# giuliojiang/pbrt-v3-IILE

Hardware: AMD Instinct MI355X
Metric: Mray/s on killeroo-simple 1080p (path integrator, rays = Scene::Intersect + IntersectP calls) (higher is better)
Workload: dtype f32

## Files before the change

include/iile_gpu.h:

```cpp
#ifndef IILE_GPU_H
#define IILE_GPU_H

#include "iile_scene.h"

#ifdef __cplusplus
extern "C" {
#endif

typedef struct iile_scene iile_scene;

enum {
    IILE_OK = 0,
    IILE_ERR_ARG = 1,
    IILE_ERR_NO_DEVICE = 2,
    IILE_ERR_HIP = 3,
    IILE_ERR_UNSUPPORTED = 4,
    IILE_ERR_TIMEOUT = 5
};

typedef struct iile_render_params {
    int32_t k_begin, k_end;
    int32_t tile_rank, tile_nranks;
    int32_t spp_per_pass;
    int32_t collect_stats;
// ... 5 lines not shown
typedef struct iile_stats {
    uint64_t camera_rays, closest_rays, shadow_rays;
    uint64_t nodes_closest, nodes_any, tri_tests, tri_hits;
    uint64_t sphere_tests;
    uint64_t nee_evals, zero_radiance;
    uint64_t path_length[8];
    double ms_total;
    double ms_generate, ms_extend, ms_shade, ms_connect, ms_film;
    int32_t n_extend_launches, n_connect_launches , n_shade_launches, n_passes;
    uint64_t n_paths;
    uint64_t workspace_bytes;
    uint64_t ext_rays, ext_nodes, ext_tri_tests, ext_sphere_tests;
    uint64_t any_tri_tests;
    double ms_shadow, ms_mis, ms_resolve;
    uint64_t mis_rays_traced;
    uint64_t ext_rays_traced;
} iile_stats;

int iile_device_count(void);
const char *iile_last_error(void);

int iile_device_select(int32_t device);
int iile_device_alloc(uint64_t bytes, void **out_dev);
void iile_device_free(void *dev);
int iile_device_download(void *dst_host, const void *src_dev, uint64_t bytes, void *stream);
int iile_device_upload(void *dst_dev, const void *src_host, uint64_t bytes, void *stream);
int iile_device_zero(void *dev, uint64_t bytes, void *stream);
int iile_stream_create(void **out_stream);
int iile_stream_wait(void *stream);
void iile_stream_destroy(void *stream);

int iile_scene_create(const iile_scene_desc *desc, iile_scene **out);
void iile_scene_destroy(iile_scene *scene);
int iile_scene_set_camera_motion(iile_scene *scene, const iile_camera_motion *motion);

int iile_render(iile_scene *scene, const iile_render_params *params, float *film_xyzw, iile_stats *stats);
int iile_render_status(iile_scene *scene, void *stream);
int iile_render_ao(iile_scene *scene, const iile_ao_params *params, const iile_render_params *render, float *film_xyzw, iile_stats *stats);
int iile_test_patch_capacity(iile_scene *scene, uint32_t capacity);

int iile_trace_closest(iile_scene *scene, int32_t n, const float *o3, const float *d3, const float *tmax,
                       int32_t *prim, float *tb, iile_stats *stats);
#define IILE_SHAPE_HIT_FLOATS 28
int iile_shape_hit_attributes(iile_scene *scene, int32_t n, const float *o3, const float *d3, const int32_t *prim, float *out);
int iile_trace_any(iile_scene *scene, int32_t n, const float *o3, const float *d3, const float *tmax,
                   int32_t *hit, iile_stats *stats);
int iile_halton_samples(iile_scene *scene, int32_t n, const int32_t *px, const int32_t *py, const int32_t *k,
                        int32_t dim0, int32_t ndims, float *out, uint32_t *index_out);
int iile_sample_table_records(iile_scene *scene, int32_t n, const int32_t *px, const int32_t *py, const int32_t *k, const int32_t *bounce,
                              float *out8);
uint64_t iile_sample_table_budget(void);
void iile_test_sample_table_budget(uint64_t bytes);
uint64_t iile_sample_table_bytes(const iile_scene *scene);
int iile_camera_rays(iile_scene *scene, int32_t n, const float *pfilm2, const float *plens2, float *o3, float *d3);
int iile_camera_rays_at(iile_scene *scene, int32_t n, const float *pfilm2, const float *plens2, float time, float *o3, float *d3);
int iile_li_samples(iile_scene *scene, int32_t n, const int32_t *px, const int32_t *py, const int32_t *k,
                    float *L3, int32_t *nrays2);
int iile_ao_array_samples(iile_scene *scene, int32_t n_samples, int32_t n, const int32_t *px, const int32_t *py, const int32_t *k,
                          const int32_t *j, float *out2);
int iile_ao_li_samples(iile_scene *scene, const iile_ao_params *params, int32_t n, const int32_t *px, const int32_t *py, const int32_t *k,
                       float *L1, int32_t *nrays2);
int iile_bsdf_eval(iile_scene *scene, int32_t n, int32_t mat, const float *wo3, const float *wi3, float *out4);
int iile_bsdf_sample(iile_scene *scene, int32_t n, int32_t mat, const float *wo3, const float *u2, float *out7);
int iile_bsdf_eval_ng(iile_scene *scene, int32_t n, int32_t mat, const float *ng3, const float *wo3, const float *wi3, float *out4);
int iile_bsdf_sample_ng(iile_scene *scene, int32_t n, int32_t mat, const float *ng3, const float *wo3, const float *u2, float *out7);
int iile_bsdf_sample_specular(iile_scene *scene, int32_t n, int32_t mat, const float *wo3, const float *u2, float *out9);
int iile_render_probes(iile_scene *scene, int32_t n_probes, const float *pos3, const float *dir3, float *intensity_rgb,
                       float *normals_xyz, float *distance, int32_t outputs_on_device, iile_stats *stats, void *stream);
typedef struct iile_probe_ref_params {
    int32_t max_depth;
    int32_t first_sample;
    int32_t n_samples;
    int32_t spp_total;
    int32_t outputs_on_device;
    void *stream;
} iile_probe_ref_params;
int iile_render_probes_reference(iile_scene *scene, int32_t n_probes, const float *pos3, const float *dir3, const iile_probe_ref_params *params,
                                 float *intensity_rgb, float *weight_sum, float *normals_xyz, float *distance, iile_stats *stats);
int iile_test_probe_ref_group(iile_scene *scene, uint32_t samples_per_group);
int iile_reference_points(iile_scene *scene, int32_t n, const float *pfilm2, uint8_t *valid, float *pos3, float *dir3);
typedef struct iile_direct_params {
    int32_t n_passes, first_pass;
    int32_t accumulate;
    int32_t film_on_device;
    void *stream;
} iile_direct_params;
int iile_render_direct(iile_scene *scene, const iile_direct_params *params, double *film_rgbw);
int iile_iispt_hemi_points(iile_scene *scene, const iile_iispt_task *task, uint8_t *valid, float *pos3, float *dir3);
int iile_iispt_gather(iile_scene *scene, const iile_iispt_task *task, const uint8_t *valid, const float *pos3, const float *dir3,
                      const float *nn_films, int32_t nn_on_device, float *out_rgbw, int32_t out_on_device);
int iile_iispt_hemi_points_batch(iile_scene *scene, const iile_iispt_task *tasks, int32_t n_tasks, uint8_t *valid, float *pos3, float *dir3,
                                 void *stream);
int iile_iispt_gather_batch(iile_scene *scene, const iile_iispt_task *tasks, int32_t n_tasks, const uint8_t *valid, const float *pos3,
                            const float *dir3, const float *nn_films, int32_t nn_on_device, float *out_rgbw, int32_t out_on_device, void *stream);
int iile_iispt_film_add(iile_scene *scene, const iile_iispt_task *tasks, int32_t n_tasks, const float *out_rgbw_dev, double *film_rgbw_dev,
                        int32_t film_w, int32_t film_h, void *stream);
int iile_iispt_film_merge(const double *direct_rgbw_dev, const double *indirect_rgbw_dev, int64_t n_pixels, float *rgb_dev, void *stream);
typedef struct iile_iispt_net iile_iispt_net;
typedef struct iile_iispt_net_weights {
    const float *conv_weight[15], *conv_bias[15];
    const float *bn_weight[5], *bn_bias[5], *bn_mean[5], *bn_var[5];
    float bn_eps;
} iile_iispt_net_weights;
int iile_iispt_net_create(const iile_iispt_net_weights *weights, iile_iispt_net **out);
int iile_iispt_net_load(const char *path, iile_iispt_net **out);
int iile_iispt_net_forward(iile_iispt_net *net, const float *in_dev, float *out_dev, int32_t n, int32_t max_batch, void *stream,
// ... 28 lines not shown
```

pbrt-v3-iile_amd/binding.py:

```python
import ctypes
import os

import numpy as np

_HERE = os.path.dirname(os.path.abspath(__file__))
LIB_DIR = os.path.join(_HERE, "lib")
REPO_ROOT = os.path.dirname(_HERE)
DEFAULT_SCENE = os.path.join(REPO_ROOT, "scenes", "killeroo-simple.pbrt")

c_i32, c_u32, c_u64, c_f32, c_f64 = (ctypes.c_int32, ctypes.c_uint32, ctypes.c_uint64, ctypes.c_float,
                                     ctypes.c_double)
c_vp = ctypes.c_void_p


class HostOverrides(ctypes.Structure):
    _fields_ = [("xres", c_i32), ("yres", c_i32), ("spp", c_i32), ("max_depth", c_i32), ("sampler", c_i32),
                ("accel_split", c_i32), ("bvh_build", c_vp), ("quick_render", c_i32)]


SAMPLERS = {None: 0, "": 0, "halton": 1, "sobol": 2}
SPLITS = {None: 0, "": 0, "sah": 1, "hlbvh": 2, "middle": 3, "equal": 4}


class HostSceneInfo(ctypes.Structure):
# ... 142 lines not shown

class Disney(ctypes.Structure):
    _fields_ = [(n, c_f32) for n in ("metallic specular_tint anisotropic sheen sheen_tint clearcoat clearcoat_gloss spec_trans "
                                     "flatness diff_trans").split()] + [("thin", c_i32), ("pad_", c_i32)]
QUADRIC_DISK, QUADRIC_CYLINDER = 0, 1
PRIM_SPHERE, PRIM_FLIP, PRIM_QUADRIC = 1, 8, 32
LIGHT_AREA_QUADRIC = 6


class GpuStats(ctypes.Structure):
    _fields_ = [(n, c_u64) for n in ("camera_rays closest_rays shadow_rays nodes_closest nodes_any tri_tests "
                                     "tri_hits sphere_tests nee_evals zero_radiance").split()] + [
        ("path_length", c_u64 * 8),
        ("ms_total", c_f64), ("ms_generate", c_f64), ("ms_extend", c_f64), ("ms_shade", c_f64),
        ("ms_connect", c_f64), ("ms_film", c_f64),
        ("n_extend_launches", c_i32), ("n_connect_launches", c_i32), ("n_shade_launches", c_i32),
        ("n_passes", c_i32), ("n_paths", c_u64), ("workspace_bytes", c_u64),
        ("ext_rays", c_u64), ("ext_nodes", c_u64), ("ext_tri_tests", c_u64), ("ext_sphere_tests", c_u64),
        ("any_tri_tests", c_u64), ("ms_shadow", c_f64), ("ms_mis", c_f64), ("ms_resolve", c_f64),
        ("mis_rays_traced", c_u64), ("ext_rays_traced", c_u64)]

    def as_dict(self):
        d = {}
        for name, _ in self._fields_:
            v = getattr(self, name)
            d[name] = list(v) if name == "path_length" else v
        return d


HOST_SYMBOLS = ["iile_host_load_pbrt", "iile_host_scene_desc", "iile_host_scene_film", "iile_host_scene_get_info",
                "iile_host_scene_free", "iile_host_film_to_rgb", "iile_host_write_pfm", "iile_host_last_error", "iile_host_read_image",
                "iile_host_scene_texture", "iile_host_scene_texture_level", "iile_host_scene_filter_table",
                "iile_host_sobol_matrices", "iile_host_sobol_vdc", "iile_host_write_exr", "iile_host_write_image",
                "iile_host_scene_film_filename", "iile_host_scene_light", "iile_host_scene_quadric_count", "iile_host_scene_quadric",
                "iile_host_scene_material", "iile_host_scene_camera", "iile_host_scene_ao", "iile_host_scene_camera_motion"]
class NetWeights(ctypes.Structure):
    _fields_ = [("conv_weight", c_vp * 15), ("conv_bias", c_vp * 15), ("bn_weight", c_vp * 5), ("bn_bias", c_vp * 5),
                ("bn_mean", c_vp * 5), ("bn_var", c_vp * 5), ("bn_eps", c_f32)]


class ProbeRefParams(ctypes.Structure):
    _fields_ = [("max_depth", c_i32), ("first_sample", c_i32), ("n_samples", c_i32), ("spp_total", c_i32), ("outputs_on_device", c_i32),
                ("stream", c_vp)]


class DirectParams(ctypes.Structure):
    _fields_ = [("n_passes", ctypes.c_int32), ("first_pass", ctypes.c_int32), ("accumulate", ctypes.c_int32), ("film_on_device", ctypes.c_int32),
                ("stream", ctypes.c_void_p)]


GPU_SYMBOLS = ["iile_device_count", "iile_last_error", "iile_scene_create", "iile_scene_destroy", "iile_render",
               "iile_scene_set_camera_motion", "iile_camera_rays_at",
               "iile_render_ao", "iile_ao_array_samples", "iile_ao_li_samples",
               "iile_trace_closest", "iile_trace_any", "iile_shape_hit_attributes", "iile_halton_samples", "iile_sample_table_records", "iile_sample_table_budget", "iile_test_sample_table_budget", "iile_sample_table_bytes", "iile_camera_rays", "iile_li_samples",
               "iile_bsdf_eval", "iile_bsdf_sample", "iile_bsdf_eval_ng", "iile_bsdf_sample_ng", "iile_bsdf_sample_specular", "iile_trig_probe", "iile_texture_eval", "iile_texture_eval_p", "iile_light_sample_li", "iile_light_sample_at", "iile_light_pdf_at", "iile_light_le", "iile_light_choose", "iile_render_probes",
               "iile_render_probes_reference", "iile_test_probe_ref_group", "iile_reference_points",
               "iile_device_select", "iile_device_alloc", "iile_device_free", "iile_device_download", "iile_device_upload", "iile_device_zero",
               "iile_stream_create", "iile_stream_wait", "iile_stream_destroy",
               "iile_iispt_film_add", "iile_iispt_film_merge",
               "iile_iispt_hemi_points", "iile_iispt_gather", "iile_iispt_hemi_points_batch", "iile_iispt_gather_batch", "iile_bvh_build_hlbvh", "iile_bvh_pack_probe", "iile_render_direct",
               "iile_wide_ref_shift", "iile_traversal_limits", "iile_render_status", "iile_test_patch_capacity", "iile_iispt_net_create", "iile_iispt_net_load", "iile_iispt_net_forward", "iile_iispt_net_predict", "iile_iispt_net_destroy"]
DIST_SYMBOLS = ["iile_dist_unique_id", "iile_dist_create", "iile_dist_create_deadline", "iile_dist_abort", "iile_dist_wait", "iile_dist_destroy", "iile_dist_rank", "iile_dist_size", "iile_dist_ranks_seen",
                "iile_dist_film_reduce", "iile_dist_monitor_reduce", "iile_dist_barrier", "iile_dist_sum_u64", "iile_dist_max_f64",
                "iile_dist_rendezvous_file", "iile_dist_rendezvous_file_token", "iile_dist_rendezvous_done", "iile_dist_all_ok",
                "iile_dist_last_error"]
DIST_ID_BYTES = 128

_host = None
_gpu = None
_dist = None


def host_lib():
    global _host
    if _host is None:
        path = os.path.join(LIB_DIR, "libiile_host.so")
        if not os.path.exists(path):
            raise RuntimeError(f"{path} is missing: run __graft_entry__.build() (make -C pbrt-v3-iile_amd/csrc host)")
        lib = ctypes.CDLL(path)
        lib.iile_host_last_error.restype = ctypes.c_char_p
        lib.iile_host_load_pbrt.argtypes = [ctypes.c_char_p, ctypes.POINTER(HostOverrides), ctypes.POINTER(c_vp)]
        lib.iile_host_scene_desc.restype = c_vp
        lib.iile_host_scene_desc.argtypes = [c_vp]
        lib.iile_host_scene_film.restype = ctypes.POINTER(FilmDesc)
        lib.iile_host_scene_film.argtypes = [c_vp]
        lib.iile_host_scene_get_info.argtypes = [c_vp, ctypes.POINTER(HostSceneInfo)]
        lib.iile_host_scene_ao.argtypes = [c_vp, ctypes.POINTER(AoParams)]
        lib.iile_host_scene_free.argtypes = [c_vp]
        lib.iile_host_scene_free.restype = None
        lib.iile_host_scene_quadric_count.argtypes = [c_vp]
        lib.iile_host_scene_quadric_count.restype = c_i32
        lib.iile_host_scene_quadric.argtypes = [c_vp, c_i32, ctypes.POINTER(Quadric)]
        lib.iile_host_scene_material.argtypes = [c_vp, c_i32, ctypes.POINTER(Material)]
        lib.iile_host_scene_camera.argtypes = [c_vp, ctypes.POINTER(Camera)]
        lib.iile_host_scene_camera_motion.argtypes = [c_vp, ctypes.POINTER(CameraMotion)]
        lib.iile_host_film_to_rgb.argtypes = [ctypes.POINTER(FilmDesc), c_vp, c_vp]
        lib.iile_host_write_pfm.argtypes = [ctypes.c_char_p, c_vp, c_i32, c_i32]
        lib.iile_host_read_image.argtypes = [ctypes.c_char_p, ctypes.POINTER(c_i32), ctypes.POINTER(c_i32), c_vp]
        lib.iile_host_write_exr.argtypes = [ctypes.c_char_p, c_vp, c_i32, c_i32, c_i32, c_i32, c_i32, c_i32]
        lib.iile_host_write_image.argtypes = [ctypes.c_char_p, ctypes.POINTER(FilmDesc), c_vp]
        lib.iile_host_scene_film_filename.argtypes = [c_vp]
        lib.iile_host_scene_film_filename.restype = ctypes.c_char_p
        lib.iile_host_scene_texture.argtypes = [c_vp, c_i32, ctypes.POINTER(Texture)]
        lib.iile_host_scene_texture_level.argtypes = [c_vp, c_i32, c_i32, c_vp]
        lib.iile_host_scene_filter_table.argtypes = [c_vp, c_vp]
        lib.iile_host_sobol_matrices.argtypes = [c_i32, c_vp, c_vp]
        lib.iile_host_sobol_vdc.argtypes = [c_i32, c_vp, c_vp]
# ... 44 lines not shown
        if not os.path.exists(path):
            raise RuntimeError(f"{path} is missing: the HIP extension was not built; there is no CPU fallback "
                               "(run __graft_entry__.build())")
        lib = ctypes.CDLL(path)
        lib.iile_last_error.restype = ctypes.c_char_p
        lib.iile_scene_create.argtypes = [c_vp, ctypes.POINTER(c_vp)]
        lib.iile_scene_destroy.argtypes = [c_vp]
        lib.iile_scene_destroy.restype = None
        lib.iile_render.argtypes = [c_vp, ctypes.POINTER(RenderParams), c_vp, ctypes.POINTER(GpuStats)]
        lib.iile_render_ao.argtypes = [c_vp, ctypes.POINTER(AoParams), ctypes.POINTER(RenderParams), c_vp, ctypes.POINTER(GpuStats)]
        lib.iile_ao_array_samples.argtypes = [c_vp, c_i32, c_i32, c_vp, c_vp, c_vp, c_vp, c_vp]
        lib.iile_ao_li_samples.argtypes = [c_vp, ctypes.POINTER(AoParams), c_i32, c_vp, c_vp, c_vp, c_vp, c_vp]
        lib.iile_trace_closest.argtypes = [c_vp, c_i32, c_vp, c_vp, c_vp, c_vp, c_vp, ctypes.POINTER(GpuStats)]
        lib.iile_trace_any.argtypes = [c_vp, c_i32, c_vp, c_vp, c_vp, c_vp, ctypes.POINTER(GpuStats)]
        lib.iile_halton_samples.argtypes = [c_vp, c_i32, c_vp, c_vp, c_vp, c_i32, c_i32, c_vp, c_vp]
        lib.iile_camera_rays.argtypes = [c_vp, c_i32, c_vp, c_vp, c_vp, c_vp]
        lib.iile_camera_rays_at.argtypes = [c_vp, c_i32, c_vp, c_vp, c_f32, c_vp, c_vp]
        lib.iile_scene_set_camera_motion.argtypes = [c_vp, ctypes.POINTER(CameraMotion)]
        lib.iile_li_samples.argtypes = [c_vp, c_i32, c_vp, c_vp, c_vp, c_vp, c_vp]
        lib.iile_bsdf_eval.argtypes = [c_vp, c_i32, c_i32, c_vp, c_vp, c_vp]
        lib.iile_texture_eval.argtypes = [c_vp, c_i32, c_i32, c_vp, c_vp, c_vp]
        lib.iile_light_sample_li.argtypes = [c_vp, c_i32, c_i32, c_vp, c_vp]
        lib.iile_light_sample_at.argtypes = [c_vp, c_i32, c_i32, c_vp, c_vp, c_vp, c_vp]
        lib.iile_light_pdf_at.argtypes = [c_vp, c_i32, c_i32, c_vp, c_vp, c_vp, c_vp]
        lib.iile_light_le.argtypes = [c_vp, c_i32, c_i32, c_vp, c_vp]
        lib.iile_light_choose.argtypes = [c_vp, c_i32, c_vp, c_vp, c_vp, c_vp, c_vp]
        lib.iile_texture_eval_p.argtypes = [c_vp, c_i32, c_i32, c_vp, c_vp, c_vp, c_vp]
        lib.iile_render_probes.argtypes = [c_vp, c_i32, c_vp, c_vp, c_vp, c_vp, c_vp, c_i32, ctypes.POINTER(GpuStats), c_vp]
        lib.iile_render_probes_reference.argtypes = [c_vp, c_i32, c_vp, c_vp, ctypes.POINTER(ProbeRefParams), c_vp, c_vp, c_vp, c_vp,
                                                     ctypes.POINTER(GpuStats)]
        lib.iile_test_probe_ref_group.argtypes = [c_vp, c_u32]
        lib.iile_reference_points.argtypes = [c_vp, c_i32, c_vp, c_vp, c_vp, c_vp]
        lib.iile_bsdf_sample.argtypes = [c_vp, c_i32, c_i32, c_vp, c_vp, c_vp]
        lib.iile_bsdf_eval_ng.argtypes = [c_vp, c_i32, c_i32, c_vp, c_vp, c_vp, c_vp]
        lib.iile_bsdf_sample_ng.argtypes = [c_vp, c_i32, c_i32, c_vp, c_vp, c_vp, c_vp]
        lib.iile_bsdf_sample_specular.argtypes = [c_vp, c_i32, c_i32, c_vp, c_vp, c_vp]
        lib.iile_trig_probe.argtypes = [c_i32, c_vp, c_vp]
        lib.iile_iispt_hemi_points.argtypes = [c_vp, ctypes.POINTER(IisptTask), c_vp, c_vp, c_vp]
        lib.iile_iispt_gather.argtypes = [c_vp, ctypes.POINTER(IisptTask), c_vp, c_vp, c_vp, c_vp, c_i32, c_vp, c_i32]
        lib.iile_iispt_hemi_points_batch.argtypes = [c_vp, ctypes.POINTER(IisptTask), c_i32, c_vp, c_vp, c_vp, c_vp]
        lib.iile_iispt_gather_batch.argtypes = [c_vp, ctypes.POINTER(IisptTask), c_i32, c_vp, c_vp, c_vp, c_vp, c_i32, c_vp, c_i32, c_vp]
        lib.iile_bvh_build_hlbvh.argtypes = [c_i32, c_vp, c_i32, c_vp, ctypes.POINTER(c_i32), c_vp, ctypes.POINTER(BvhBuildStats)]
        lib.iile_bvh_pack_probe.argtypes = [c_i32, c_vp, c_i32, c_vp, c_vp, ctypes.POINTER(c_i32)]
        lib.iile_render_status.argtypes = [c_vp, c_vp]
        lib.iile_traversal_limits.argtypes = [ctypes.POINTER(c_i32)]
        lib.iile_traversal_limits.restype = None
        lib.iile_test_patch_capacity.argtypes = [c_vp, c_u32]
        lib.iile_sample_table_budget.argtypes = []
        lib.iile_sample_table_budget.restype = c_u64
        lib.iile_test_sample_table_budget.argtypes = [c_u64]
        lib.iile_test_sample_table_budget.restype = None
        lib.iile_sample_table_bytes.argtypes = [c_vp]
        lib.iile_sample_table_bytes.restype = c_u64
        lib.iile_iispt_net_create.argtypes = [ctypes.POINTER(NetWeights), ctypes.POINTER(c_vp)]
        lib.iile_iispt_net_load.argtypes = [ctypes.c_char_p, ctypes.POINTER(c_vp)]
        lib.iile_iispt_net_forward.argtypes = [c_vp, c_vp, c_vp, c_i32, c_i32, c_vp, c_vp, c_i32]
        lib.iile_iispt_net_predict.argtypes = [c_vp, c_vp, c_vp, c_vp, c_vp, c_vp, c_i32, c_i32, c_i32, c_vp]
        lib.iile_iispt_film_add.argtypes = [c_vp, ctypes.POINTER(IisptTask), c_i32, c_vp, c_vp, c_i32, c_i32, c_vp]
        lib.iile_iispt_film_merge.argtypes = [c_vp, c_vp, ctypes.c_int64, c_vp, c_vp]
        lib.iile_device_upload.argtypes = [c_vp, c_vp, ctypes.c_uint64, c_vp]
        lib.iile_device_zero.argtypes = [c_vp, ctypes.c_uint64, c_vp]
        lib.iile_iispt_net_destroy.argtypes = [c_vp]
        lib.iile_iispt_net_destroy.restype = None
        _gpu = lib
    return _gpu


def dist_lib():
    global _dist
    if _dist is None:
        path = os.path.join(LIB_DIR, "libiile_dist.so")
        if not os.path.exists(path):
            raise RuntimeError(f"{path} is missing: run __graft_entry__.build() (make -C pbrt-v3-iile_amd/csrc dist)")
        lib = ctypes.CDLL(path)
        lib.iile_dist_last_error.restype = ctypes.c_char_p
        lib.iile_dist_unique_id.argtypes = [c_vp]
        lib.iile_dist_create.argtypes = [c_vp, c_i32, c_i32, ctypes.POINTER(c_vp)]
        lib.iile_dist_create_deadline.argtypes = [c_vp, c_i32, c_i32, ctypes.c_double, ctypes.POINTER(c_vp)]
        lib.iile_dist_wait.argtypes = [c_vp, c_vp]
        lib.iile_dist_abort.argtypes = [c_vp]
        lib.iile_dist_abort.restype = None
        lib.iile_dist_destroy.argtypes = [c_vp]
        lib.iile_dist_destroy.restype = None
        lib.iile_dist_rank.argtypes = [c_vp]
        lib.iile_dist_size.argtypes = [c_vp]
        lib.iile_dist_film_reduce.argtypes = [c_vp, c_vp, ctypes.c_int64, c_i32, c_vp]
        lib.iile_dist_barrier.argtypes = [c_vp, c_vp]
        lib.iile_dist_sum_u64.argtypes = [c_vp, c_vp, c_i32]
        lib.iile_dist_max_f64.argtypes = [c_vp, c_vp, c_i32]
        lib.iile_dist_rendezvous_file.argtypes = [ctypes.c_char_p, c_i32, c_vp, c_i32]
        lib.iile_dist_rendezvous_file_token.argtypes = [ctypes.c_char_p, c_i32, ctypes.c_uint64, c_vp, c_i32]
        lib.iile_dist_rendezvous_done.argtypes = [c_vp, ctypes.c_char_p]
        lib.iile_dist_all_ok.argtypes = [c_vp, c_i32, ctypes.POINTER(c_i32)]
        _dist = lib
    return _dist


class Dist:

    @staticmethod
    def unique_id():
        buf = (ctypes.c_uint8 * DIST_ID_BYTES)()
        lib = dist_lib()
        if lib.iile_dist_unique_id(buf) != 0:
            raise RuntimeError(f"iile_dist_unique_id failed: {lib.iile_dist_last_error().decode()}")
        return bytes(buf)
# ... 239 lines not shown
            self.close()
        except Exception:
            pass


def sample_table_budget():
    return int(gpu_lib().iile_sample_table_budget())


def set_test_sample_table_budget(nbytes):
    gpu_lib().iile_test_sample_table_budget(int(nbytes))


class GpuScene:

    def __init__(self, host_scene):
        lib = gpu_lib()
        self.host = host_scene
        self._s = c_vp()
        rc = lib.iile_scene_create(host_scene.desc, ctypes.byref(self._s))
        if rc != 0:
            raise RuntimeError(f"iile_scene_create failed ({rc}): {lib.iile_last_error().decode()}")
        motion = getattr(host_scene, "camera_motion", None)
        if motion is not None:
            rc = lib.iile_scene_set_camera_motion(self._s, ctypes.byref(motion))
            if rc != 0:
                msg = lib.iile_last_error().decode()
                lib.iile_scene_destroy(self._s)
                self._s = c_vp()
                raise RuntimeError(f"iile_scene_set_camera_motion failed ({rc}): {msg}")

    def _check(self, rc, what):
        if rc != 0:
            raise RuntimeError(f"{what} failed ({rc}): {gpu_lib().iile_last_error().decode()}")

    def render(self, k_begin=0, k_end=0, tile_rank=0, tile_nranks=1, spp_per_pass=0, collect_stats=False,
               time_kernels=False, film_device_ptr=None, stream=None, want_stats=True):
        prm = RenderParams(int(k_begin), int(k_end), int(tile_rank), int(tile_nranks), int(spp_per_pass),
                           int(bool(collect_stats)), int(time_kernels), int(film_device_ptr is not None),
                           c_vp(stream) if stream else None)
        st = GpuStats()
        if film_device_ptr is not None:
            film, ptr = None, c_vp(int(film_device_ptr))
        else:
            h, w = self.host.film_shape
            film = np.zeros((h, w, 4), np.float32)
            ptr = film.ctypes.data
        rc = gpu_lib().iile_render(self._s, ctypes.byref(prm), ptr, ctypes.byref(st) if want_stats else None)
        self._check(rc, "iile_render")
        if not want_stats:
            return film, None
        d = st.as_dict()
        d["sample_table_bytes"] = int(gpu_lib().iile_sample_table_bytes(self._s))
        return film, d

    def _ao_params(self, nsamples, cossample):
        ao = self.host.ao or {"nsamples": 64, "cossample": True}
        return AoParams(int(ao["nsamples"] if nsamples is None else nsamples), int(bool(ao["cossample"] if cossample is None else cossample)))

    def render_ao(self, nsamples=None, cossample=None, k_begin=0, k_end=0, tile_rank=0, tile_nranks=1, spp_per_pass=0, collect_stats=False,
                  film_device_ptr=None, stream=None, want_stats=True):
        ao = self._ao_params(nsamples, cossample)
        prm = RenderParams(int(k_begin), int(k_end), int(tile_rank), int(tile_nranks), int(spp_per_pass), int(bool(collect_stats)), 0,
                           int(film_device_ptr is not None), c_vp(stream) if stream else None)
        st = GpuStats()
        if film_device_ptr is not None:
            film, ptr = None, c_vp(int(film_device_ptr))
        else:
            h, w = self.host.film_shape
            film = np.zeros((h, w, 4), np.float32)
            ptr = film.ctypes.data
        rc = gpu_lib().iile_render_ao(self._s, ctypes.byref(ao), ctypes.byref(prm), ptr, ctypes.byref(st) if want_stats else None)
        self._check(rc, "iile_render_ao")
        return film, (st.as_dict() if want_stats else None)

    def ao_array_samples(self, nsamples, px, py, k, j):
        px, py, k, j = _i32(px), _i32(py), _i32(k), _i32(j)
        out = np.empty((len(px), 2), np.float32)
        self._check(gpu_lib().iile_ao_array_samples(self._s, int(nsamples), len(px), px.ctypes.data, py.ctypes.data, k.ctypes.data, j.ctypes.data,
                                                    out.ctypes.data), "iile_ao_array_samples")
        return out

    def ao_li_samples(self, px, py, k, nsamples=None, cossample=None):
        ao = self._ao_params(nsamples, cossample)
        px, py, k = _i32(px), _i32(py), _i32(k)
        n = len(px)
        L = np.empty(n, np.float32)
        nr = np.empty((n, 2), np.int32)
        self._check(gpu_lib().iile_ao_li_samples(self._s, ctypes.byref(ao), n, px.ctypes.data, py.ctypes.data, k.ctypes.data, L.ctypes.data,
                                                 nr.ctypes.data), "iile_ao_li_samples")
        return L, nr

    def render_status(self, stream=None):
        self._check(gpu_lib().iile_render_status(self._s, c_vp(stream) if stream else None), "iile_render_status")

    def test_patch_capacity(self, capacity):
        self._check(gpu_lib().iile_test_patch_capacity(self._s, int(capacity)), "iile_test_patch_capacity")

    def trace_closest(self, o, d, tmax, instrumented=True):
        o, d, tmax = _f32(o), _f32(d), _f32(tmax)
        n = len(tmax)
        prim = np.empty(n, np.int32)
        tb = np.empty((n, 4), np.float32)
        st = GpuStats()
        self._check(gpu_lib().iile_trace_closest(self._s, n, o.ctypes.data, d.ctypes.data, tmax.ctypes.data,
                                                 prim.ctypes.data, tb.ctypes.data,
                                                 ctypes.byref(st) if instrumented else None), "iile_trace_closest")
        return prim, tb, st.as_dict()

    def shape_hit_attributes(self, o, d, prim):
        o, d, prim = _f32(o).reshape(-1, 3), _f32(d).reshape(-1, 3), _i32(prim)
        out = np.empty((len(prim), 28), np.float32)
        f = gpu_lib().iile_shape_hit_attributes
        f.argtypes = [c_vp, c_i32, c_vp, c_vp, c_vp, c_vp]
        self._check(f(self._s, len(prim), o.ctypes.data, d.ctypes.data, prim.ctypes.data, out.ctypes.data), "iile_shape_hit_attributes")
        r = {k: out[:, 3 * i:3 * i + 3] for i, k in enumerate(("p", "n", "sn", "dpdu", "dpdv", "dndu", "dndv", "wo"))}
        r.update(u=out[:, 24], v=out[:, 25], flip=out[:, 26] != 0)
        return r

    def trace_any(self, o, d, tmax, instrumented=True):
        o, d, tmax = _f32(o), _f32(d), _f32(tmax)
        n = len(tmax)
        hit = np.empty(n, np.int32)
        st = GpuStats()
        self._check(gpu_lib().iile_trace_any(self._s, n, o.ctypes.data, d.ctypes.data, tmax.ctypes.data,
                                             hit.ctypes.data, ctypes.byref(st) if instrumented else None),
                    "iile_trace_any")
        return hit, st.as_dict()

    def halton_samples(self, px, py, k, dim0, ndims):
        px, py, k = _i32(px), _i32(py), _i32(k)
        n = len(px)
        out = np.empty((n, ndims), np.float32)
        idx = np.empty(n, np.uint32)
        self._check(gpu_lib().iile_halton_samples(self._s, n, px.ctypes.data, py.ctypes.data, k.ctypes.data, dim0,
                                                  ndims, out.ctypes.data, idx.ctypes.data), "iile_halton_samples")
        return out, idx

    def sample_table_records(self, px, py, k, bounce):
        px, py, k, bounce = _i32(px), _i32(py), _i32(k), _i32(bounce)
        out = np.empty((len(px), 8), np.float32)
        f = gpu_lib().iile_sample_table_records
        f.argtypes = [c_vp, c_i32, c_vp, c_vp, c_vp, c_vp, c_vp]
        self._check(f(self._s, len(px), px.ctypes.data, py.ctypes.data, k.ctypes.data, bounce.ctypes.data, out.ctypes.data),
                    "iile_sample_table_records")
        return out

    def camera_rays(self, pfilm, plens=None):
        pfilm = _f32(pfilm)
        n = len(pfilm)
        o = np.empty((n, 3), np.float32)
        d = np.empty((n, 3), np.float32)
        pl = _f32(plens) if plens is not None else None
        self._check(gpu_lib().iile_camera_rays(self._s, n, pfilm.ctypes.data, pl.ctypes.data if pl is not None else None,
                                               o.ctypes.data, d.ctypes.data), "iile_camera_rays")
        return o, d

    def camera_rays_at(self, pfilm, time, plens=None):
        pfilm = _f32(pfilm)
        n = len(pfilm)
        o = np.empty((n, 3), np.float32)
        d = np.empty((n, 3), np.float32)
        pl = _f32(plens) if plens is not None else None
        self._check(gpu_lib().iile_camera_rays_at(self._s, n, pfilm.ctypes.data, pl.ctypes.data if pl is not None else None,
                                                  c_f32(time), o.ctypes.data, d.ctypes.data), "iile_camera_rays_at")
        return o, d

    def set_camera_motion(self, motion):
        return gpu_lib().iile_scene_set_camera_motion(self._s, ctypes.byref(motion) if motion is not None else None)

    def li_samples(self, px, py, k):
        px, py, k = _i32(px), _i32(py), _i32(k)
        n = len(px)
        L = np.empty((n, 3), np.float32)
        nr = np.empty((n, 2), np.int32)
        self._check(gpu_lib().iile_li_samples(self._s, n, px.ctypes.data, py.ctypes.data, k.ctypes.data, L.ctypes.data,
                                              nr.ctypes.data), "iile_li_samples")
        return L, nr

    def bsdf_eval(self, mat, wo, wi):
        wo, wi = _f32(wo), _f32(wi)
        out = np.empty((len(wo), 4), np.float32)
        self._check(gpu_lib().iile_bsdf_eval(self._s, len(wo), mat, wo.ctypes.data, wi.ctypes.data, out.ctypes.data),
                    "iile_bsdf_eval")
        return out

    def light_sample_li(self, light, p):
        p = _f32(p).reshape(-1, 3)
        out = np.empty((len(p), 7), np.float32)
        self._check(gpu_lib().iile_light_sample_li(self._s, int(light), len(p), p.ctypes.data, out.ctypes.data), "iile_light_sample_li")
        return out

    def light_sample_at(self, light, ref_p, ref_n, u):
        ref_p, ref_n, u = _f32(ref_p).reshape(-1, 3), _f32(ref_n).reshape(-1, 3), _f32(u).reshape(-1, 2)
        assert len(ref_p) == len(ref_n) == len(u)
        out = np.empty((len(ref_p), 13), np.float32)
        self._check(gpu_lib().iile_light_sample_at(self._s, int(light), len(ref_p), ref_p.ctypes.data, ref_n.ctypes.data, u.ctypes.data,
                                                   out.ctypes.data), "iile_light_sample_at")
# ... 238 lines not shown
        if rc != 0:
            raise RuntimeError(f"iile_iispt_net_forward failed ({rc}): {self._lib.iile_last_error().decode()}")

    def predict(self, intensity_ptr, normals_ptr, distance_ptr, pred_ptr, n, film_rows=False, max_batch=0, stream=None, slot_ptr=None):
        rc = self._lib.iile_iispt_net_predict(self._h, intensity_ptr, normals_ptr, distance_ptr, pred_ptr, slot_ptr, int(n), int(bool(film_rows)),
                                              int(max_batch), stream)
        if rc != 0:
            raise RuntimeError(f"iile_iispt_net_predict failed ({rc}): {self._lib.iile_last_error().decode()}")

    def close(self):
        if self._h:
            self._lib.iile_iispt_net_destroy(self._h)
            self._h = c_vp()

    def __del__(self):
        try:
            self.close()
        except Exception:
            pass


def bvh_build_hlbvh(bounds6, max_prims_in_node=4):
    b = _f32(bounds6).reshape(-1, 6)
    n = len(b)
    nodes = np.zeros(max(2 * n, 1), dtype=BVH_NODE)
    order = np.zeros(max(n, 1), dtype=np.int32)
    n_nodes = c_i32(0)
    st = BvhBuildStats()
    rc = gpu_lib().iile_bvh_build_hlbvh(n, b.ctypes.data, int(max_prims_in_node), nodes.ctypes.data, ctypes.byref(n_nodes), order.ctypes.data,
                                        ctypes.byref(st))
    if rc != 0:
        raise RuntimeError(f"iile_bvh_build_hlbvh failed ({rc}): {gpu_lib().iile_last_error().decode()}")
    return nodes[:n_nodes.value].copy(), order[:n].copy(), {k: getattr(st, k) for k, _ in BvhBuildStats._fields_}


def bvh_pack_probe(nodes):
    nodes = np.ascontiguousarray(nodes, dtype=BVH_NODE)
    ni = int((nodes["nprims"] == 0).sum())
    wide = np.zeros((max(ni, 1), 16), np.float32)
    wide4 = np.zeros((max(ni, 1), 32), np.float32)
    nested = c_i32(0)
    rc = gpu_lib().iile_bvh_pack_probe(len(nodes), nodes.ctypes.data, ni, wide.ctypes.data, wide4.ctypes.data, ctypes.byref(nested))
    if rc != 0:
        raise RuntimeError(f"iile_bvh_pack_probe failed ({rc}): {gpu_lib().iile_last_error().decode()}")
    return wide[:ni], wide4[:ni], bool(nested.value)


def traversal_limits():
    out = (c_i32 * 3)()
    gpu_lib().iile_traversal_limits(out)
    return {"lds_stack": int(out[0]), "top_records": int(out[1]), "max_bvh_depth": int(out[2])}


def trig_probe(x):
    x = _f32(x)
    out = np.empty((len(x), 3), np.float32)
    rc = gpu_lib().iile_trig_probe(len(x), x.ctypes.data, out.ctypes.data)
    if rc != 0:
        raise RuntimeError(f"iile_trig_probe failed ({rc}): {gpu_lib().iile_last_error().decode()}")
    return out


def device_count():
    return int(gpu_lib().iile_device_count())
```

pbrt-v3-iile_amd/csrc/device/api_common.h:

```cpp
#pragma once
#include <algorithm>
#include <cstdint>
#include <string>
#include <vector>

#include "../../../include/iile_gpu.h"
#include "kernels.h"

#define HIP_TRY(expr)                                                                                        \
    do {                                                                                                     \
        hipError_t e_ = (expr);                                                                              \
        if (e_ != hipSuccess)                                                                                \
            return ::iile::api_fail(IILE_ERR_HIP, std::string(#expr) + ": " + hipGetErrorString(e_));       \
    } while (0)

namespace iile {

int ensure_device();

template <typename T>
struct DevBuf {
    T *p = nullptr;
    ~DevBuf() {
        if (p) (void)hipFree(p);
// ... 34 lines not shown
        const size_t want = std::max<size_t>(std::max(bytes, grown), 1);
        const hipError_t e = hipMalloc(&p, want);
        if (e != hipSuccess) {
            p = nullptr;
            return api_fail(IILE_ERR_HIP, oom ? std::string(oom) : "hipMalloc of a device block: " + std::string(hipGetErrorString(e)));
        }
        cap = want;
        return IILE_OK;
    }
};

struct Carver {
    char *base;
    size_t used = 0;
    explicit Carver(void *block = nullptr) : base(static_cast<char *>(block)) {}
    template <typename T>
    T *take(size_t n) {
        T *r = base ? reinterpret_cast<T *>(base + used) : nullptr;
        used += (std::max<size_t>(n, 1) * sizeof(T) + 255) & ~size_t(255);
        return r;
    }
};

struct EventPair {
    hipEvent_t a, b;
    int kind;
};

constexpr uint64_t kMaxPassPaths = 200000000ull;
static_assert(kMaxPassPaths < (uint64_t(1) << kSlotBits), "queue slots must fit kSlotBits");

}

struct iile_scene {
    iile::DScene ds;
    std::vector<void *> allocs;
    std::vector<uint8_t> prim_is_shape;
    int n_cus = 256;
    int max_depth = 5;
    int spp = 1;
    std::vector<int> light_samples;
    std::vector<int> light_types;
    uint32_t ws_paths = 0;
    iile::PassBuffers pb;
    iile::DevBlock ws_block;
    uint32_t film_tiles = 0, film_pixels = 0;
    iile::FilmBuffers fb;
    iile::DevBlock film_block, wide_block;
    uint64_t film_wide = 0;
    iile_probe_setup probe;
    const uint32_t *probe_pixel_offsets = nullptr;
    const float *probe_filter_table = nullptr;
    uint64_t sample_table_bytes = 0;
    void *stab_block = nullptr;
    bool camera_moves = false;
    float shutter[2] = {0.f, 1.f};
    uint32_t *flag_count = nullptr;
    float *flag_rec = nullptr;
    iile::DevBlock probe_block;
    int *spill = nullptr;
    hipStream_t nee_stream = nullptr;
    int *spill_nee = nullptr;
    hipEvent_t ev_shade[16] = {}, ev_nee[16] = {};
    std::vector<iile::EventPair> events;
    size_t events_used = 0;
    hipEvent_t ev_begin = nullptr, ev_end = nullptr;
    std::vector<int> tile_of_slot, slot_of_tile;
    iile::DevBlock tile_tables;
    int map_key[4] = {0, 0, 0, 0};
    iile::PatchDev patch{};
    iile::DevBlock patch_block;
    iile::DevBlock film_add_block;
    uint32_t patch_cap_override = 0;
    uint32_t probe_ref_group_override = 0;
    bool overflow_unchecked = false;
    hipStream_t overflow_stream = nullptr;
    iile::DevBlock scratch;
    iile::DevBlock ao_block;
};

namespace iile {
int ensure_workspace(iile_scene *sc, uint32_t n_paths);
int ensure_film(iile_scene *sc, uint32_t n_tiles, uint32_t n_pixels, uint64_t n_wide = 0);
int frame_pass(iile_scene *sc, const DScene &S, int rank, int nranks, hipStream_t stream, PassDesc *P);
uint64_t path_budget(double bytes_per_path);
constexpr uint64_t kSampleTableBudget = uint64_t(4) << 30;
uint64_t sample_table_budget();
void set_sample_table_budget(uint64_t bytes);
int run_pass(iile_scene *sc, const DScene &S, int max_depth, const PassDesc &P_in, const LaunchCfg &cfg, bool timed, bool one_stream = false);
void copy_counters(const DCounters &c, iile_stats *st);
struct FrameIntegrator {
    double bytes_per_path;
    uint64_t max_pass_paths;
    const char *too_many;
    int (*reserve)(iile_scene *sc, uint32_t n_paths, void *ctx);
    int (*run)(iile_scene *sc, const DScene &S, const PassDesc &P, const LaunchCfg &cfg, bool timed, bool one_stream, void *ctx);
    void *ctx;
};
int render_frame(iile_scene *sc, const iile_render_params *prm, float *film_xyzw, iile_stats *stats, const FrameIntegrator &fi);
}
```

pbrt-v3-iile_amd/csrc/device/api_probes.hip:

```cpp
#include <cstring>

#include "api_common.h"

using namespace iile;

namespace {
LaunchCfg probe_cfg(const iile_scene *sc, bool count_stats = false) {
    LaunchCfg cfg{sc->n_cus, nullptr, count_stats};
    cfg.camera_moves = sc->camera_moves;
    return cfg;
}
template <typename T>
int finish(DevBuf<T> &dev, T *host, size_t n) {
    HIP_TRY(hipGetLastError());
    HIP_TRY(hipDeviceSynchronize());
    return dev.get(host, n);
}

int trace_common(iile_scene *sc, int32_t n, const float *o3, const float *d3, const float *tmax, int any,
                 std::vector<float4> *hits, iile_stats *stats) {
    if (!sc || n < 0 || !o3 || !d3 || !tmax) return api_fail(IILE_ERR_ARG, "iile_trace: bad argument");
    int rc = ensure_device();
    if (rc) return rc;
    std::vector<float4> ro(n), rd(n);
// ... 54 lines not shown
    return IILE_OK;
}

int iile_trace_any(iile_scene *sc, int32_t n, const float *o3, const float *d3, const float *tmax, int32_t *hit,
                   iile_stats *stats) {
    if (!hit) return api_fail(IILE_ERR_ARG, "iile_trace_any: null output");
    std::vector<float4> hits;
    int rc = trace_common(sc, n, o3, d3, tmax, 1, &hits, stats);
    if (rc) return rc;
    for (int i = 0; i < n; ++i) {
        uint32_t u;
        std::memcpy(&u, &hits[2 * i].x, 4);
        hit[i] = int32_t(u);
    }
    return IILE_OK;
}

int iile_halton_samples(iile_scene *sc, int32_t n, const int32_t *px, const int32_t *py, const int32_t *k,
                        int32_t dim0, int32_t ndims, float *out, uint32_t *index_out) {
    if (!sc || n < 0 || !px || !py || !k || !out || ndims <= 0 || dim0 < 0 || dim0 + ndims > (sc->ds.sobol ? sc->ds.sobol_dims : sc->ds.n_hdims))
        return api_fail(IILE_ERR_ARG, "iile_halton_samples: bad argument");
    int rc = ensure_device();
    if (rc) return rc;
    DevBuf<int> dx, dy, dk;
    DevBuf<float> dout;
    DevBuf<uint32_t> dindex;
    if ((rc = dx.put(px, n)) || (rc = dy.put(py, n)) || (rc = dk.put(k, n)) || (rc = dout.alloc(size_t(n) * ndims)) ||
        (rc = dindex.alloc(n)))
        return rc;
    if (n) launch_halton(sc->ds, n, dx.p, dy.p, dk.p, dim0, ndims, dout.p, dindex.p, probe_cfg(sc));
    if ((rc = finish(dout, out, size_t(n) * ndims))) return rc;
    if (index_out && (rc = dindex.get(index_out, n))) return rc;
    return IILE_OK;
}

int iile_sample_table_records(iile_scene *sc, int32_t n, const int32_t *px, const int32_t *py, const int32_t *k, const int32_t *bounce,
                              float *out8) {
    if (!sc || n < 0 || !px || !py || !k || !bounce || !out8) return api_fail(IILE_ERR_ARG, "iile_sample_table_records: bad argument");
    if (!sc->ds.stab_shade) return api_fail(IILE_ERR_ARG, "iile_sample_table_records: the scene has no sample table");
    for (int i = 0; i < n; ++i)
        if (k[i] < 0 || uint32_t(k[i]) >= sc->ds.stab_spp || bounce[i] >= sc->ds.max_depth)
            return api_fail(IILE_ERR_ARG, "iile_sample_table_records: sample or bounce outside the table");
    int rc = ensure_device();
    if (rc) return rc;
    DevBuf<int> dx, dy, dk, db;
    DevBuf<float> dout;
    if ((rc = dx.put(px, n)) || (rc = dy.put(py, n)) || (rc = dk.put(k, n)) || (rc = db.put(bounce, n)) || (rc = dout.alloc(size_t(n) * 8))) return rc;
    if (n) launch_sample_table_read(sc->ds, n, dx.p, dy.p, dk.p, db.p, dout.p, probe_cfg(sc));
    return finish(dout, out8, size_t(n) * 8);
}
uint64_t iile_sample_table_budget(void) { return sample_table_budget(); }
void iile_test_sample_table_budget(uint64_t bytes) { set_sample_table_budget(bytes); }
uint64_t iile_sample_table_bytes(const iile_scene *sc) { return sc ? sc->sample_table_bytes : 0; }

int iile_camera_rays(iile_scene *sc, int32_t n, const float *pfilm2, const float *plens2, float *o3, float *d3) {
    if (!sc || n < 0 || !pfilm2 || !o3 || !d3) return api_fail(IILE_ERR_ARG, "iile_camera_rays: bad argument");
    return iile_camera_rays_at(sc, n, pfilm2, plens2, 0.f, o3, d3);
}
int iile_camera_rays_at(iile_scene *sc, int32_t n, const float *pfilm2, const float *plens2, float time, float *o3, float *d3) {
    if (!sc || n < 0 || !pfilm2 || !o3 || !d3) return api_fail(IILE_ERR_ARG, "iile_camera_rays_at: bad argument");
    if (!(time == time)) return api_fail(IILE_ERR_ARG, "iile_camera_rays_at: the time is not a number");
    int rc = ensure_device();
    if (rc) return rc;
    DevBuf<float> df, dl, dox, ddx;
    if ((rc = df.put(pfilm2, 2 * size_t(n))) || (rc = dox.alloc(3 * size_t(n))) || (rc = ddx.alloc(3 * size_t(n))))
        return rc;
    if (plens2 && (rc = dl.put(plens2, 2 * size_t(n)))) return rc;
    if (n) launch_camera(sc->ds, n, df.p, plens2 ? dl.p : nullptr, time, dox.p, ddx.p, probe_cfg(sc));
    if ((rc = finish(dox, o3, 3 * size_t(n))) || (rc = ddx.get(d3, 3 * size_t(n)))) return rc;
    return IILE_OK;
}

int iile_bsdf_eval(iile_scene *sc, int32_t n, int32_t mat, const float *wo3, const float *wi3, float *out4) {
    return bsdf_probe(sc, n, mat, wo3, wi3, 3, 0, out4, 4);
}
int iile_bsdf_sample(iile_scene *sc, int32_t n, int32_t mat, const float *wo3, const float *u2, float *out7) {
    return bsdf_probe(sc, n, mat, wo3, u2, 2, 1, out7, 7);
}
int iile_bsdf_eval_ng(iile_scene *sc, int32_t n, int32_t mat, const float *ng3, const float *wo3, const float *wi3, float *out4) {
    if (!ng3) return api_fail(IILE_ERR_ARG, "iile_bsdf_eval_ng: null normal");
    return bsdf_probe(sc, n, mat, wo3, wi3, 3, 0, out4, 4, ng3);
}
int iile_bsdf_sample_ng(iile_scene *sc, int32_t n, int32_t mat, const float *ng3, const float *wo3, const float *u2, float *out7) {
    if (!ng3) return api_fail(IILE_ERR_ARG, "iile_bsdf_sample_ng: null normal");
    return bsdf_probe(sc, n, mat, wo3, u2, 2, 1, out7, 7, ng3);
}

int iile_bsdf_sample_specular(iile_scene *sc, int32_t n, int32_t mat, const float *wo3, const float *u2, float *out9) {
    return bsdf_probe(sc, n, mat, wo3, u2, 2, 2, out9, 9);
}

int iile_light_sample_li(iile_scene *sc, int32_t light, int32_t n, const float *p3, float *out7) {
    if (!sc || n < 0 || !p3 || !out7 || light < 0 || light >= sc->ds.n_lights)
        return api_fail(IILE_ERR_ARG, "iile_light_sample_li: bad argument");
    if (!iile_light_is_delta(sc->light_types[size_t(light)])) return api_fail(IILE_ERR_ARG, "iile_light_sample_li: not a delta light");
    int rc = ensure_device();
    if (rc) return rc;
    DevBuf<float> dp, dout;
    if ((rc = dp.put(p3, 3 * size_t(n))) || (rc = dout.alloc(7 * size_t(n)))) return rc;
    if (n) launch_light_probe(sc->ds, n, light, dp.p, dout.p, probe_cfg(sc));
    return finish(dout, out7, 7 * size_t(n));
}

static bool light_is_sampled(int type) {
    return type == IILE_LIGHT_DIFFUSE_AREA || type == IILE_LIGHT_AREA_TRIANGLE || type == IILE_LIGHT_AREA_QUADRIC || type == IILE_LIGHT_INFINITE;
}
// ... 114 lines not shown
```

pbrt-v3-iile_amd/csrc/device/api_render.hip:

```cpp
#include <chrono>
#include <cmath>
#include <cstdio>
#include <cstdlib>
#include <cstring>

#include "api_common.h"

using namespace iile;

namespace {

int get_events(iile_scene *sc, int kind, EventPair **out) {
    if (sc->events_used == sc->events.size()) {
        EventPair ep;
        HIP_TRY(hipEventCreate(&ep.a));
        HIP_TRY(hipEventCreate(&ep.b));
        sc->events.push_back(ep);
    }
    *out = &sc->events[sc->events_used++];
    (*out)->kind = kind;
    return IILE_OK;
}

template <typename Fn>
// ... 171 lines not shown
        sc->fb.tile_rgbw = c.take<float4>(2 * size_t(n_tiles) * 256);
        sc->fb.film_xyzw = c.take<float4>(n_pixels);
        return c.used;
    };
    if (const int rc = sc->film_block.reserve(film(Carver()))) return rc;
    film(Carver(sc->film_block.p));
    sc->fb.k0_rgbv = sc->fb.tile_rgbw + size_t(n_tiles) * 256;
    sc->film_tiles = n_tiles;
    sc->film_pixels = n_pixels;
    return IILE_OK;
}

int frame_pass(iile_scene *sc, const DScene &S, int rank, int nranks, hipStream_t stream, PassDesc *P) {
    std::memset(P, 0, sizeof(*P));
    P->n_tiles_x = (S.samp_x1 - S.samp_x0 + 15) / 16;
    P->n_tiles_y = (S.samp_y1 - S.samp_y0 + 15) / 16;
    P->tile_rank = rank, P->tile_nranks = nranks;
    return ensure_tile_map(sc, P, stream);
}

uint64_t path_budget(double bytes_per_path) {
    double budget_mb = 65536;
    if (const char *e = std::getenv("IILE_WORKSPACE_MB")) budget_mb = std::max(64.0, atof(e));
    return std::min<uint64_t>(uint64_t(budget_mb * 1048576.0 / bytes_per_path), kMaxPassPaths);
}

void copy_counters(const DCounters &c, iile_stats *st) {
    st->camera_rays = c.camera_rays;
    st->closest_rays = c.closest_rays;
    st->shadow_rays = c.shadow_rays;
    st->nodes_closest = c.nodes_closest;
    st->nodes_any = c.nodes_any;
    st->tri_tests = c.tri_tests;
    st->tri_hits = c.tri_hits;
    st->sphere_tests = c.sphere_tests;
    st->nee_evals = c.nee_evals;
    st->zero_radiance = c.zero_radiance;
    for (int i = 0; i < 8; ++i) st->path_length[i] = c.path_length[i];
    st->ext_rays = c.ext_rays;
    st->ext_nodes = c.ext_nodes;
    st->ext_tri_tests = c.ext_tri_tests;
    st->ext_sphere_tests = c.ext_sphere_tests;
    st->any_tri_tests = c.any_tri_tests;
    st->mis_rays_traced = c.mis_traced;
    st->ext_rays_traced = c.ext_traced;
}

int run_pass(iile_scene *sc, const DScene &S_in, int max_depth, const PassDesc &P_in, const LaunchCfg &cfg, bool timed, bool one_stream) {
    PassBuffers &B = sc->pb;
    PassDesc P = P_in;
    DScene S = S_in;
    if (cfg.count_stats || P.list_px || S.probe_mode || P.k0 < 0 || uint64_t(P.k0) + uint64_t(P.kc) > uint64_t(S.stab_spp) || max_depth > S.max_depth)
        clear_sample_table(&S);
    P.gen_fused = !cfg.count_stats && !P.list_px && !S.has_infinite && !S.probe_mode && !B.nray_out && !S.env_camera && !cfg.camera_moves;
    HIP_TRY(hipMemsetAsync(B.counts, 0, kCntWords * sizeof(uint32_t), cfg.stream));
    auto timed_launch_on = [&](hipStream_t stream, int kind, auto &&fn) -> int { return timed_step(sc, timed, stream, kind, fn); };
    auto timed_launch = [&](int kind, auto &&fn) -> int { return timed_launch_on(cfg.stream, kind, fn); };
    const bool two_streams = sc->nee_stream && !one_stream && !cfg.count_stats && !S.has_infinite && max_depth < 15;
    const bool nee_doubled = two_streams && !S.has_specular && B.nee_alt;
    LaunchCfg cfg_nee = cfg;
    if (two_streams) cfg_nee.stream = sc->nee_stream;
    auto buffers_of = [&](int bounce, bool nee_side) {
        PassBuffers X = B;
        if (nee_doubled && (bounce & 1)) X.nee = B.nee_alt, X.mis_hit = B.mis_hit_alt, X.nee_mis = B.nee_mis_alt;
        if (two_streams && nee_side) X.spill = sc->spill_nee;
        return X;
    };
    int rc = IILE_OK;
    if (P.gen_fused) {
        HIP_TRY(hipMemsetD32Async(reinterpret_cast<hipDeviceptr_t>(&B.counts[0]), int(P.n_paths), 1, cfg.stream));
    } else {
        rc = timed_launch(0, [&] { launch_generate(S, P, B, cfg); });
        if (rc) return rc;
    }
    P.skip_last_bounce = 0;
    if (!cfg.count_stats && max_depth >= 1 && !S.probe_mode && !B.nray_out)
        P.skip_last_bounce = S.has_specular ? 1 : 2;
    const int last_bounce = (P.skip_last_bounce == 2) ? max_depth - 1 : max_depth;
    for (int b = 0; b <= last_bounce; ++b) {
        rc = timed_launch(1, [&] { launch_extend(S, P, B, b, B.queue_cap, cfg); });
        if (rc) return rc;
        if (S.has_infinite) {
            rc = timed_launch(6, [&] { launch_miss(S, B, b, B.queue_cap, cfg); });
            if (rc) return rc;
        }
        if (two_streams && !nee_doubled && b > 0) HIP_TRY(hipStreamWaitEvent(cfg.stream, sc->ev_nee[b - 1], 0));
        if (nee_doubled && b > 1) HIP_TRY(hipStreamWaitEvent(cfg.stream, sc->ev_nee[b - 2], 0));
        const PassBuffers B_shade = buffers_of(b, false), B_nee = buffers_of(b, true);
        rc = timed_launch(2, [&] { launch_shade(S, P, B_shade, b, B.queue_cap, cfg); });
        if (rc) return rc;
        if (b < max_depth) {
            if (two_streams) {
                HIP_TRY(hipEventRecord(sc->ev_shade[b], cfg.stream));
                HIP_TRY(hipStreamWaitEvent(cfg_nee.stream, sc->ev_shade[b], 0));
            }
            rc = timed_launch_on(cfg_nee.stream, 5, [&] { launch_mis(S, B_nee, b, B.queue_cap, cfg_nee); });
            if (rc) return rc;
            rc = timed_launch_on(cfg_nee.stream, 6, [&] { launch_mis_lit(S, B_nee, b, B.queue_cap, cfg_nee); });
            if (rc) return rc;
            rc = timed_launch_on(cfg_nee.stream, 3, [&] { launch_shadow(S, B_nee, b, B.queue_cap, cfg_nee); });
            if (rc) return rc;
            if (two_streams) HIP_TRY(hipEventRecord(sc->ev_nee[b], cfg_nee.stream));
        }
    }
    if (two_streams && max_depth > 0) HIP_TRY(hipStreamWaitEvent(cfg.stream, sc->ev_nee[max_depth - 1], 0));
    HIP_TRY(hipGetLastError());
    return IILE_OK;
}

int render_frame(iile_scene *sc, const iile_render_params *prm, float *film_xyzw, iile_stats *stats, const FrameIntegrator &fi) {
    int rc = check_pending_overflow(sc);
    if (rc) return rc;
    const DScene &S = sc->ds;
    int k_begin = prm->k_begin, k_end = prm->k_end;
    if (k_end <= 0) {
        k_begin = 0;
        k_end = sc->spp;
    }
    if (k_begin < 0 || k_begin >= k_end) return api_fail(IILE_ERR_ARG, "iile_render: empty sample range");
    int rank = prm->tile_rank, nranks = prm->tile_nranks;
    if (nranks <= 0) {
        rank = 0;
        nranks = 1;
    }
    if (rank < 0 || rank >= nranks) return api_fail(IILE_ERR_ARG, "iile_render: tile_rank out of range");
    hipStream_t stream = static_cast<hipStream_t>(prm->stream);
    LaunchCfg cfg{sc->n_cus, stream, prm->collect_stats != 0};
    cfg.camera_moves = sc->camera_moves;
    const bool timed = prm->time_kernels != 0;

    PassDesc P;
    rc = frame_pass(sc, S, rank, nranks, stream, &P);
    if (rc) return rc;
    const uint64_t pix_slots = uint64_t(P.n_owned_tiles) * 256;
    const int n_samples = k_end - k_begin;
    uint64_t max_paths = std::min<uint64_t>(path_budget(fi.bytes_per_path), fi.max_pass_paths);
    if (prm->spp_per_pass > 0) max_paths = std::min<uint64_t>(max_paths, std::max<uint64_t>(1, pix_slots * uint64_t(prm->spp_per_pass)));
    const uint64_t paths_per_tile = uint64_t(256) * uint64_t(n_samples);
    if (paths_per_tile > kMaxPassPaths) return api_fail(IILE_ERR_UNSUPPORTED, "more than 781 250 samples per pixel in one render: split the sample range");
    if (paths_per_tile > fi.max_pass_paths) return api_fail(IILE_ERR_UNSUPPORTED, fi.too_many);
    const int tiles_per_pass = int(std::max<uint64_t>(1, std::min<uint64_t>(uint64_t(std::max(P.n_owned_tiles, 1)), max_paths / paths_per_tile)));
    const uint32_t fw = uint32_t(S.crop_x1 - S.crop_x0), fh = uint32_t(S.crop_y1 - S.crop_y0);
// ... 186 lines not shown
```

pbrt-v3-iile_amd/csrc/device/api_scene.hip:

```cpp
#include <array>
#include <chrono>
#include <cmath>
#include <cstddef>
#include <cstdio>
#include <cstdlib>
#include <cstring>
#include <limits>
#include <map>

#include "api_common.h"

using namespace iile;

namespace {
thread_local std::string g_err;
}
namespace iile {
int api_fail(int code, const std::string &msg) {
    g_err = msg;
    return code;
}
int ensure_device() {
    int n = 0;
    hipError_t e = hipGetDeviceCount(&n);
// ... 635 lines not shown
    const int n = d.n_lights;
    const size_t stride = light_record_floats(n);
    if (n > 1 && d.integrator.light_strategy != IILE_LIGHTS_SPATIAL) {
        std::vector<float> tab(stride, 0.f);
        const float *power = n > IILE_MAX_LIGHTS ? d.light_power_all : d.integrator.light_power;
        float *func = tab.data(), *cdf = tab.data() + n;
        for (int i = 0; i < n; ++i) func[i] = d.integrator.light_strategy == IILE_LIGHTS_UNIFORM ? 1.f : power[i];
        cdf[0] = 0;
        for (int i = 1; i < n + 1; ++i) cdf[i] = cdf[i - 1] + func[i - 1] / n;
        const float func_int = cdf[n];
        if (func_int == 0)
            for (int i = 1; i < n + 1; ++i) cdf[i] = float(i) / float(n);
        else
            for (int i = 1; i < n + 1; ++i) cdf[i] /= func_int;
        tab[2 * size_t(n) + 1] = func_int;
        return upload(sc, tab.data(), tab.size(), &S.light_dist);
    }
    if (!spatial_table(d)) return IILE_OK;
    light_grid(d, S.light_nv);
    std::vector<float> samples(128 * 5);
    const int bases[5] = {2, 3, 5, 7, 11};
    for (int i = 0; i < 128; ++i)
        for (int b = 0; b < 5; ++b) {
            if (b == 0) {
                uint64_t v = uint64_t(i), r = 0;
                for (int k = 0; k < 64; ++k) r |= ((v >> k) & 1ull) << (63 - k);
                samples[5 * i] = float(double(r) * 0x1p-64);
                continue;
            }
            const float inv_base = 1.f / float(bases[b]);
            uint64_t a = uint64_t(i), rev = 0;
            float inv_base_n = 1;
            while (a) {
                const uint64_t next = a / uint64_t(bases[b]);
                rev = rev * uint64_t(bases[b]) + (a - next * uint64_t(bases[b]));
                inv_base_n *= inv_base;
                a = next;
            }
            samples[5 * i + b] = std::min(float(rev) * inv_base_n, 0x1.fffffep-1f);
        }
    const float *dsamples = nullptr;
    float *dist = nullptr;
    const size_t n_vox = size_t(S.light_nv[0]) * S.light_nv[1] * S.light_nv[2];
    int rc = upload(sc, samples.data(), samples.size(), &dsamples);
    if (!rc) rc = scene_alloc(sc, n_vox * stride * sizeof(float), &dist, "hipMalloc(light distributions) failed");
    if (rc) return rc;
    S.light_dist = dist;
    LaunchCfg cfg{sc->n_cus, nullptr, false};
    launch_light_distributions(S, dsamples, dist, cfg);
    if (hipDeviceSynchronize() != hipSuccess || hipGetLastError() != hipSuccess) return api_fail(IILE_ERR_HIP, "light distribution kernel failed");
    return IILE_OK;
}

int build_sample_table(iile_scene *sc, const iile_scene_desc &d) {
    DScene &S = sc->ds;
    clear_sample_table(&S);
    sc->sample_table_bytes = 0;
    const int64_t spp = d.halton.spp;
    if (S.sobol || S.max_depth <= 0 || spp <= 0 || S.sample_stride <= 0 || std::getenv("IILE_NO_SAMPLE_TABLE")) return IILE_OK;
    if (5 + 7 * int64_t(S.max_depth) >= int64_t(S.n_hdims)) return IILE_OK;
    const bool lens = S.lens_radius > 0;
    const uint64_t per_slot = uint64_t(32) * uint64_t(S.max_depth) + (lens ? 16 : 8);
    if (uint64_t(spp) > sample_table_budget() / (uint64_t(16384) * per_slot)) return IILE_OK;
    const uint64_t slots = uint64_t(16384) * uint64_t(spp);
    if (slots >= (uint64_t(1) << 32)) return IILE_OK;
    const auto t0 = std::chrono::steady_clock::now();
    S.stab_slots = uint32_t(slots), S.stab_spp = uint32_t(spp);
    if (spp > 1) {
        int l = 0;
        while ((uint64_t(1) << l) < uint64_t(spp)) ++l;
        S.stab_spp_magic = uint32_t((((uint64_t(1) << l) - uint64_t(spp)) << 32) / uint64_t(spp) + 1);
        S.stab_spp_shift = uint32_t(l - 1);
    }
    float2 *cam = nullptr, *lens_part = nullptr;
    float4 *shade = nullptr;
    auto layout = [&](Carver c) {
        cam = c.take<float2>(slots);
        if (lens) lens_part = c.take<float2>(slots);
        shade = c.take<float4>(slots * uint64_t(S.max_depth) * 2);
        return c.used;
    };
    void *block = nullptr;
    if (hipMalloc(&block, layout(Carver())) != hipSuccess) {
        (void)hipGetLastError();
        clear_sample_table(&S);
        return IILE_OK;
    }
    sc->allocs.push_back(block);
    sc->stab_block = block;
    layout(Carver(block));
    launch_sample_table(S, cam, lens_part, shade, LaunchCfg{sc->n_cus, nullptr, false});
    if (hipDeviceSynchronize() != hipSuccess || hipGetLastError() != hipSuccess) return api_fail(IILE_ERR_HIP, "sample table kernel failed");
    S.stab_cam = cam, S.stab_lens = lens_part, S.stab_shade = shade;
    sc->sample_table_bytes = slots * per_slot;
    if (std::getenv("IILE_TIMING"))
        fprintf(stderr, "iile timing: sample table of %.1f MiB built in %.3f s\n", double(sc->sample_table_bytes) / 1048576.0,
                std::chrono::duration<double>(std::chrono::steady_clock::now() - t0).count());
    return IILE_OK;
}

}

namespace iile {
namespace {
uint64_t g_table_budget_override = 0;
}
uint64_t sample_table_budget() { return g_table_budget_override ? g_table_budget_override : kSampleTableBudget; }
void set_sample_table_budget(uint64_t bytes) { g_table_budget_override = bytes; }
}

extern "C" {

const char *iile_last_error(void) { return g_err.c_str(); }

int iile_device_count(void) {
    int n = 0;
    if (hipGetDeviceCount(&n) != hipSuccess) return 0;
    return n;
}

int iile_device_select(int32_t device) {
    int rc = ensure_device();
    if (rc) return rc;
    HIP_TRY(hipSetDevice(device));
    return IILE_OK;
}
int iile_device_alloc(uint64_t bytes, void **out_dev) {
    if (!out_dev) return api_fail(IILE_ERR_ARG, "iile_device_alloc: null argument");
    int rc = ensure_device();
    if (rc) return rc;
    HIP_TRY(hipMalloc(out_dev, std::max<size_t>(size_t(bytes), 1)));
    return IILE_OK;
}
void iile_device_free(void *dev) {
    if (dev) (void)hipFree(dev);
}
int iile_device_download(void *dst_host, const void *src_dev, uint64_t bytes, void *stream) {
    if (!dst_host || !src_dev) return api_fail(IILE_ERR_ARG, "iile_device_download: null argument");
    hipStream_t s = static_cast<hipStream_t>(stream);
    HIP_TRY(hipMemcpyAsync(dst_host, src_dev, size_t(bytes), hipMemcpyDeviceToHost, s));
    HIP_TRY(hipStreamSynchronize(s));
    return IILE_OK;
}

int iile_device_upload(void *dst_dev, const void *src_host, uint64_t bytes, void *stream) {
    if (!dst_dev || !src_host) return api_fail(IILE_ERR_ARG, "iile_device_upload: null argument");
    hipStream_t s = static_cast<hipStream_t>(stream);
    HIP_TRY(hipMemcpyAsync(dst_dev, src_host, size_t(bytes), hipMemcpyHostToDevice, s));
    HIP_TRY(hipStreamSynchronize(s));
    return IILE_OK;
// ... 39 lines not shown
              "texture kinds");
int iile_scene_create(const iile_scene_desc *d, iile_scene **out) {
    if (!d || !out) return api_fail(IILE_ERR_ARG, "iile_scene_create: null argument");
    int rc = check_scene_desc(*d);
    if (!rc) rc = ensure_device();
    if (rc) return rc;
    iile_scene *sc = new iile_scene;
    std::memset(&sc->ds, 0, sizeof(sc->ds));
    std::memset(&sc->pb, 0, sizeof(sc->pb));
    std::memset(&sc->fb, 0, sizeof(sc->fb));
    hipDeviceProp_t prop;
    int dev = 0;
    if (hipGetDevice(&dev) == hipSuccess && hipGetDeviceProperties(&prop, dev) == hipSuccess)
        sc->n_cus = prop.multiProcessorCount;
    set_kernel_flags(*d, sc->ds);
    for (auto build : {build_bvh, build_top4, build_prims, build_shapes, build_materials, build_textures, build_lights, build_halton,
                       build_sobol, build_camera_film, build_runtime, build_light_distribution, build_sample_table}) {
        rc = build(sc, *d);
        if (rc) {
            iile_scene_destroy(sc);
            return rc;
        }
    }
    *out = sc;
    return IILE_OK;
}

int iile_scene_set_camera_motion(iile_scene *sc, const iile_camera_motion *mo) {
    if (!sc || !mo) return api_fail(IILE_ERR_ARG, "iile_scene_set_camera_motion: null argument");
    if (sc->camera_moves) return api_fail(IILE_ERR_ARG, "iile_scene_set_camera_motion: the scene's camera has a motion already");
    auto finite = [](const float *v, size_t n) {
        for (size_t i = 0; i < n; ++i)
            if (!std::isfinite(v[i])) return false;
        return true;
    };
    if (!finite(&mo->start_time, 1) || !finite(&mo->end_time, 1) || !finite(mo->camera_to_world_end, 16) || !finite(&mo->T[0][0], 6) ||
        !finite(&mo->R[0][0], 8) || !finite(&mo->S[0][0], 32))
        return api_fail(IILE_ERR_ARG, "iile_scene_set_camera_motion: a non-finite entry in the camera motion");
    if (mo->end_time < mo->start_time) return api_fail(IILE_ERR_ARG, "iile_scene_set_camera_motion: the motion ends before it starts (TransformTimes)");
    int rc = ensure_device();
    if (rc) return rc;
    DScene &S = sc->ds;
    DCameraMotion dm;
    std::memset(&dm, 0, sizeof(dm));
    dm.c2w_start = S.camera_to_world;
    std::memcpy(dm.c2w_end.m, mo->camera_to_world_end, 64);
    dm.start_time = mo->start_time, dm.end_time = mo->end_time;
    dm.shutter_open = sc->shutter[0], dm.shutter_close = sc->shutter[1];
    std::memcpy(dm.T, mo->T, sizeof(dm.T));
    std::memcpy(dm.R, mo->R, sizeof(dm.R));
    for (int k = 0; k < 2; ++k)
        for (int i = 0; i < 3; ++i)
            for (int j = 0; j < 3; ++j) dm.S[k][3 * i + j] = mo->S[k][4 * i + j];
    if (S.stab_cam) {
        const uint64_t slots = S.stab_slots;
        void *time = nullptr;
        if (sc->sample_table_bytes + 4 * slots <= sample_table_budget() && hipMalloc(&time, size_t(slots) * sizeof(float)) != hipSuccess) {
            (void)hipGetLastError();
            time = nullptr;
        }
        if (!time) {
            for (void *&p : sc->allocs)
                if (p == sc->stab_block) p = nullptr;
            HIP_TRY(hipFree(sc->stab_block));
            sc->stab_block = nullptr;
            clear_sample_table(&S);
            sc->sample_table_bytes = 0;
        } else {
            sc->allocs.push_back(time);
            launch_sample_table_time(S, static_cast<float *>(time), LaunchCfg{sc->n_cus, nullptr, false});
            if (hipDeviceSynchronize() != hipSuccess || hipGetLastError() != hipSuccess) return api_fail(IILE_ERR_HIP, "sample table time kernel failed");
            dm.stab_time = static_cast<float *>(time);
            sc->sample_table_bytes += 4 * slots;
        }
    }
    HIP_TRY(hipMemcpy(const_cast<DCameraMotion *>(camera_motion(S)), &dm, sizeof(dm), hipMemcpyHostToDevice));
    sc->camera_moves = true;
    return IILE_OK;
}

void iile_scene_destroy(iile_scene *sc) {
    if (!sc) return;
    for (void *p : sc->allocs) (void)hipFree(p);
    if (sc->nee_stream) (void)hipStreamDestroy(sc->nee_stream);
    for (int i = 0; i < 16; ++i) {
        if (sc->ev_shade[i]) (void)hipEventDestroy(sc->ev_shade[i]);
        if (sc->ev_nee[i]) (void)hipEventDestroy(sc->ev_nee[i]);
    }
    for (EventPair &e : sc->events) {
        (void)hipEventDestroy(e.a);
        (void)hipEventDestroy(e.b);
    }
    if (sc->ev_begin) (void)hipEventDestroy(sc->ev_begin);
    if (sc->ev_end) (void)hipEventDestroy(sc->ev_end);
    delete sc;
}
}
```

pbrt-v3-iile_amd/csrc/device/dbsdf.h:

```cpp
#pragma once
enum Lobe : int { kLobePassThrough, kLobeLambert, kLobeLambertTrans, kLobeMicro, kLobeMicroTrans, kLobeBlend, kLobeSpecular, kLobeSpecTrans };
DEV bool lobe_is_specular(Lobe l) { return l == kLobePassThrough || l == kLobeSpecular || l == kLobeSpecTrans; }
struct Bsdf {
    F3 ns, ng, ss, ts;
    F3 kd;
    union { F3 micro_r, ks; };
    union { F3 kr, ltrans_t, cond_eta; };
    union { F3 kt, mtrans_t, cond_k; };
    float alpha, eta;
    float alpha_y;
    F3 t0;
    bool has_t0, has_t1;
    float path_eta;
    bool has_mtrans;
    int n_lobes;
    float on_a, on_b;
    bool oren_nayar;
    int mtype;
    bool has_lambert, has_micro, has_spec;
    bool has_blend;
    bool has_ltrans;
};
DEV int n_nonspec(const Bsdf &b) {
    return (b.has_lambert ? 1 : 0) + (b.has_ltrans ? 1 : 0) + (b.has_micro ? 1 : 0) + (b.has_mtrans ? 1 : 0) + (b.has_blend ? 1 : 0);
// ... 314 lines not shown
    const float eta = wo.z > 0 ? (eta_b / eta_a) : (eta_a / eta_b);
    F3 wh = normalize(wo + wi * eta);
    if (wh.z < 0) wh = -wh;
    const float F = fr_dielectric(dot(wo, wh), eta_a, eta_b);
    const float sqrt_denom = dot(wo, wh) + eta * dot(wi, wh);
    const float factor = 1 / eta;
    const float omf = 1.f - F;
    return F3{omf, omf, omf} * b.mtrans_t *
           fabsf(tr_d(wh, b.alpha, b.alpha_y) * tr_g(wo, wi, b.alpha, b.alpha_y) * eta * eta * absdot(wi, wh) * absdot(wo, wh) * factor * factor /
                 (cos_i * cos_o * sqrt_denom * sqrt_denom));
}
DEV float mtrans_pdf(const Bsdf &b, F3 wo, F3 wi) {
    if (same_hemisphere(wo, wi)) return 0;
    const float eta_a = 1.f, eta_b = b.eta;
    const float eta = wo.z > 0 ? (eta_b / eta_a) : (eta_a / eta_b);
    const F3 wh = normalize(wo + wi * eta);
    const float sqrt_denom = dot(wo, wh) + eta * dot(wi, wh);
    const float dwh_dwi = fabsf((eta * eta * dot(wi, wh)) / (sqrt_denom * sqrt_denom));
    return tr_pdf(wo, wh, b.alpha, b.alpha_y) * dwh_dwi;
}
DEV F3 lobes_f(const Bsdf &b, F3 wo, F3 wi) {
    F3 f = F3{0, 0, 0};
    if (b.has_lambert) f = f + diffuse_f(b, wo, wi);
    if (b.has_micro) f = f + micro_f(b, wo, wi);
    if (b.has_blend) f = f + blend_f(b, wo, wi);
    return f;
}
DEV F3 trans_lobes_f(const Bsdf &b, F3 wo, F3 wi) {
    F3 f = F3{0, 0, 0};
    if (b.has_ltrans) f = f + ltrans_f(b);
    if (b.has_mtrans) f = f + mtrans_f(b, wo, wi);
    return f;
}
DEV F3 bsdf_f(const Bsdf &b, F3 woW, F3 wiW) {
    F3 wi = to_local(b, wiW), wo = to_local(b, woW);
    if (wo.z == 0) return F3{0, 0, 0};
    bool reflect = dot(wiW, b.ng) * dot(woW, b.ng) > 0;
    if (reflect) return lobes_f(b, wo, wi);
    return trans_lobes_f(b, wo, wi);
}
DEV float bsdf_pdf(const Bsdf &b, F3 woW, F3 wiW) {
    if (b.n_lobes == 0) return 0.f;
    F3 wo = to_local(b, woW), wi = to_local(b, wiW);
    if (wo.z == 0) return 0.f;
    float pdf = 0.f;
    if (b.has_lambert) pdf += lambert_pdf(wo, wi);
    if (b.has_ltrans) pdf += ltrans_pdf(wo, wi);
    if (b.has_micro) pdf += micro_pdf(b, wo, wi);
    if (b.has_mtrans) pdf += mtrans_pdf(b, wo, wi);
    if (b.has_blend) pdf += blend_pdf(b, wo, wi);
    const int matching = n_nonspec(b);
    return matching > 0 ? pdf / matching : 0.f;
}
DEV F3 bsdf_sample_f(const Bsdf &b, F3 woW, F3 *wiW, float u0, float u1, float *pdf, const bool allow_specular = false,
                     bool *sampled_specular = nullptr, bool *sampled_transmission = nullptr) {
    if (sampled_specular) *sampled_specular = false;
    if (sampled_transmission) *sampled_transmission = false;
    const int matching = allow_specular ? b.n_lobes : n_nonspec(b);
    if (matching == 0) {
        *pdf = 0;
        return F3{0, 0, 0};
    }
    int comp = int(floorf(u0 * matching));
    if (comp > matching - 1) comp = matching - 1;
    Lobe pick;
    int count = comp;
    if (allow_specular && b.has_t0 && count-- == 0)
        pick = kLobePassThrough;
    else if (b.has_lambert && count-- == 0)
        pick = kLobeLambert;
    else if (b.has_ltrans && count-- == 0)
        pick = kLobeLambertTrans;
    else if (b.has_micro && count-- == 0)
        pick = kLobeMicro;
    else if (b.has_mtrans && count-- == 0)
        pick = kLobeMicroTrans;
    else if (b.has_blend && count-- == 0)
        pick = kLobeBlend;
    else if (!(allow_specular && b.has_t1) || (b.has_spec && count-- == 0))
        pick = kLobeSpecular;
    else
        pick = kLobeSpecTrans;
    if (pick == kLobeSpecular && !b.has_spec) __builtin_unreachable();
    const float ur0 = mn(u0 * matching - comp, kOneMinusEpsilon);
    F3 wo = to_local(b, woW);
    if (wo.z == 0) return F3{0, 0, 0};
    *pdf = 0;
    F3 wi = F3{0, 0, 0}, f;
    if (pick == kLobeLambert) {
        wi = cosine_sample_hemisphere(ur0, u1);
        if (wo.z < 0) wi.z *= -1;
        *pdf = lambert_pdf(wo, wi);
        f = diffuse_f(b, wo, wi);
    } else if (pick == kLobeLambertTrans) {
        wi = cosine_sample_hemisphere(ur0, u1);
        if (wo.z > 0) wi.z *= -1;
        *pdf = ltrans_pdf(wo, wi);
        f = ltrans_f(b);
    } else if (pick == kLobeMicro) {
        F3 wh = tr_sample_wh(wo, ur0, u1, b.alpha, b.alpha_y);
        wi = -wo + 2 * dot(wo, wh) * wh;
        if (!same_hemisphere(wo, wi))
            f = F3{0, 0, 0};
        else {
            *pdf = tr_pdf(wo, wh, b.alpha, b.alpha_y) / (4 * dot(wo, wh));
            f = micro_f(b, wo, wi);
        }
    } else if (pick == kLobeBlend) {
        float ua = ur0;
        if (ua < .5f) {
            ua = mn(2 * ua, kOneMinusEpsilon);
            wi = cosine_sample_hemisphere(ua, u1);
            if (wo.z < 0) wi.z *= -1;
        } else {
            ua = mn(2 * (ua - .5f), kOneMinusEpsilon);
            const F3 wh = tr_sample_wh(wo, ua, u1, b.alpha, b.alpha_y);
            wi = -wo + 2 * dot(wo, wh) * wh;
            if (!same_hemisphere(wo, wi)) return F3{0, 0, 0};
        }
        *pdf = blend_pdf(b, wo, wi);
        f = blend_f(b, wo, wi);
    } else if (pick == kLobeMicroTrans) {
        const F3 wh = tr_sample_wh(wo, ur0, u1, b.alpha, b.alpha_y);
        const float eta_a = 1.f, eta_b = b.eta;
        const float eta = wo.z > 0 ? (eta_a / eta_b) : (eta_b / eta_a);
        if (!refract_dir(wo, wh, eta, &wi)) return F3{0, 0, 0};
        *pdf = mtrans_pdf(b, wo, wi);
        f = mtrans_f(b, wo, wi);
    } else if (pick == kLobePassThrough || pick == kLobeSpecTrans) {
        const float eta_a = 1.f, eta_b = pick == kLobePassThrough ? 1.f : b.eta;
        float scale;
        if (!specular_refract(wo, eta_a, eta_b, &wi, &scale)) return F3{0, 0, 0};
        *pdf = 1;
        const F3 ft = (pick == kLobePassThrough ? b.t0 : b.kt) * (1.f - fr_dielectric(wi.z, eta_a, eta_b));
        f = sdiv(ft * scale, fabsf(wi.z));
        if (sampled_specular) *sampled_specular = true;
        if (sampled_transmission) *sampled_transmission = true;
    } else if (b.mtype == kMatGlass) {
        const float eta_a = 1.f, eta_b = b.eta;
        const float F = fr_dielectric(wo.z, eta_a, eta_b);
        if (ur0 < F) {
            wi = F3{-wo.x, -wo.y, wo.z};
            *pdf = F;
// ... 272 lines not shown
    switch (l) {
    case kDzDiffuse:
    case kDzRetro: return b.dz_diffuse;
    case kDzFakeSS: return b.dz_diffuse && b.dz_thin;
    case kDzSheen: return b.dz_sheen;
    case kDzMicro: return true;
    case kDzCoat: return b.dz_coat;
    case kDzMicroTrans: return b.has_mtrans;
    default: return b.has_ltrans;
    }
}
DEV F3 dz_lobes_f(const DisneyBsdf &b, bool reflect, F3 wo, F3 wi) {
    F3 f = F3{0, 0, 0};
    if (reflect) {
        if (b.dz_diffuse) {
            f = f + dz_diffuse_f(b.r_diffuse, wo, wi);
            if (b.dz_thin) f = f + dz_fakess_f(b.r_ss, b.rough, wo, wi);
            f = f + dz_retro_f(b.r_retro, b.rough, wo, wi);
            if (b.dz_sheen) f = f + dz_sheen_f(b.r_sheen, wo, wi);
        }
        f = f + dz_micro_f(b, wo, wi);
        if (b.dz_coat) f = f + dz_coat_f(b, wo, wi);
    } else {
        if (b.has_mtrans) f = f + dz_mtrans_f(b, wo, wi);
        if (b.has_ltrans) f = f + ltrans_f(b);
    }
    return f;
}
DEV float dz_lobes_pdf(const DisneyBsdf &b, int skip, F3 wo, F3 wi, float pdf) {
    const float cosine = lambert_pdf(wo, wi);
#pragma unroll
    for (int l = kDzDiffuse; l <= kDzSheen; ++l)
        if (l != skip && dz_has(b, DisneyLobe(l))) pdf += cosine;
    if (skip != kDzMicro) pdf += micro_pdf(b, wo, wi);
    if (skip != kDzCoat && b.dz_coat) pdf += dz_coat_pdf(b, wo, wi);
    if (skip != kDzMicroTrans && b.has_mtrans) pdf += dz_mtrans_pdf(b, wo, wi);
    if (skip != kDzLambertTrans && b.has_ltrans) pdf += ltrans_pdf(wo, wi);
    return pdf;
}
DEV F3 bsdf_f(const DisneyBsdf &b, F3 woW, F3 wiW) {
    if (!b.disney) return bsdf_f(static_cast<const Bsdf &>(b), woW, wiW);
    const F3 wi = to_local(b, wiW), wo = to_local(b, woW);
    if (wo.z == 0) return F3{0, 0, 0};
    const bool reflect = dot(wiW, b.ng) * dot(woW, b.ng) > 0;
    return dz_lobes_f(b, reflect, wo, wi);
}
DEV float bsdf_pdf(const DisneyBsdf &b, F3 woW, F3 wiW) {
    if (!b.disney) return bsdf_pdf(static_cast<const Bsdf &>(b), woW, wiW);
    const F3 wo = to_local(b, woW), wi = to_local(b, wiW);
    if (wo.z == 0) return 0.f;
    return dz_lobes_pdf(b, -1, wo, wi, 0.f) / b.n_lobes;
}
DEV F3 bsdf_sample_f(const DisneyBsdf &b, F3 woW, F3 *wiW, float u0, float u1, float *pdf, const bool allow_specular = false,
                     bool *sampled_specular = nullptr, bool *sampled_transmission = nullptr) {
    if (!b.disney) return bsdf_sample_f(static_cast<const Bsdf &>(b), woW, wiW, u0, u1, pdf, allow_specular, sampled_specular, sampled_transmission);
    if (sampled_specular) *sampled_specular = false;
    if (sampled_transmission) *sampled_transmission = false;
    const int matching = b.n_lobes;
    int comp = int(floorf(u0 * matching));
    if (comp > matching - 1) comp = matching - 1;
    int pick = kDzLambertTrans, count = comp;
    bool found = false;
#pragma unroll
    for (int l = kDzDiffuse; l <= kDzLambertTrans; ++l)
        if (!found && dz_has(b, DisneyLobe(l)) && count-- == 0) pick = l, found = true;
    const float ur0 = mn(u0 * matching - comp, kOneMinusEpsilon);
    const F3 wo = to_local(b, woW);
    if (wo.z == 0) return F3{0, 0, 0};
    *pdf = 0;
    F3 wi = F3{0, 0, 0}, f;
    if (pick <= kDzSheen) {
        wi = cosine_sample_hemisphere(ur0, u1);
        if (wo.z < 0) wi.z *= -1;
        *pdf = lambert_pdf(wo, wi);
        f = dz_lobe_f(b, DisneyLobe(pick), wo, wi);
    } else if (pick == kDzMicro) {
        const F3 wh = tr_sample_wh(wo, ur0, u1, b.alpha, b.alpha_y);
        wi = -wo + 2 * dot(wo, wh) * wh;
        if (!same_hemisphere(wo, wi))
            f = F3{0, 0, 0};
        else {
            *pdf = tr_pdf(wo, wh, b.alpha, b.alpha_y) / (4 * dot(wo, wh));
            f = dz_micro_f(b, wo, wi);
        }
    } else if (pick == kDzCoat) {
        const float alpha2 = .25f * .25f;
        const float cos_t = sqrtf(mx(0.f, (1 - powf(alpha2, 1 - ur0)) / (1 - alpha2)));
        const float sin_t = sqrtf(mx(0.f, 1 - cos_t * cos_t));
        const float phi = 2 * kPi * u1;
        float sp, cp;
        sincos_f(phi, &sp, &cp);
        F3 wh = F3{sin_t * cp, sin_t * sp, cos_t};
        if (!same_hemisphere(wo, wh)) wh = -wh;
        wi = -wo + 2 * dot(wo, wh) * wh;
        if (!same_hemisphere(wo, wi))
            f = F3{0, 0, 0};
        else {
            *pdf = dz_coat_pdf(b, wo, wi);
            f = dz_coat_f(b, wo, wi);
        }
    } else if (pick == kDzMicroTrans) {
        const F3 wh = tr_sample_wh(wo, ur0, u1, b.t_ax, b.t_ay);
        const float eta_a = 1.f, eta_b = b.eta;
        const float eta = wo.z > 0 ? (eta_a / eta_b) : (eta_b / eta_a);
        if (!refract_dir(wo, wh, eta, &wi)) return F3{0, 0, 0};
        *pdf = dz_mtrans_pdf(b, wo, wi);
        f = dz_mtrans_f(b, wo, wi);
// ... 18 lines not shown
```

pbrt-v3-iile_amd/csrc/device/dlight.h:

```cpp
#pragma once
#include "dtex.h"
struct LightSample {
    F3 p, perr, n;
};
DEV float sphere_area(const DSphere &sp) { return sp.phi_max * sp.radius * (sp.zmax - sp.zmin); }
DEV LightSample sphere_sample_area(const DSphere &sp, float u0, float u1, float *pdf) {
    float z = 1 - 2 * u0;
    float r = sqrtf(mx(0.f, 1.f - z * z));
    float phi = 2 * kPi * u1;
    float s, c;
    sincos_f(phi, &s, &c);
    F3 us = F3{r * c, r * s, z};
    F3 pobj = F3{0, 0, 0} + sp.radius * us;
    LightSample it;
    it.n = normalize(xf_normal(sp.o2w_inv, pobj));
    if (sp.reverse_orientation) it.n = it.n * -1.f;
    float scale = sp.radius / length(pobj);
    pobj = F3{pobj.x * scale, pobj.y * scale, pobj.z * scale};
    F3 pobj_err = kGamma5 * vabs(pobj);
    it.p = xf_point_err2(sp.o2w, pobj, pobj_err, &it.perr);
    *pdf = 1 / sphere_area(sp);
    return it;
}
DEV LightSample sphere_sample(const DSphere &sp, const Isect &ref, float u0, float u1, float *pdf) {
    const F3 pc = F3{sp.center[0], sp.center[1], sp.center[2]};
    F3 porigin = offset_ray_origin(ref.p, ref.perr, ref.n, pc - ref.p);
    if (length_sq(porigin - pc) <= sp.radius * sp.radius) {
        LightSample intr = sphere_sample_area(sp, u0, u1, pdf);
        F3 wi = intr.p - ref.p;
        if (length_sq(wi) == 0)
            *pdf = 0;
        else {
            wi = normalize(wi);
            *pdf *= length_sq(ref.p - intr.p) / absdot(intr.n, -wi);
        }
        if (is_inf(*pdf)) *pdf = 0.f;
        return intr;
    }
    F3 wc = normalize(pc - ref.p);
    F3 wcx, wcy;
    coordinate_system(wc, &wcx, &wcy);
    float sin_tmax2 = sp.radius * sp.radius / length_sq(ref.p - pc);
    float cos_tmax = sqrtf(mx(0.f, 1 - sin_tmax2));
    float cos_t = (1 - u0) + u0 * cos_tmax;
    float sin_t = sqrtf(mx(0.f, 1 - cos_t * cos_t));
    float phi = u1 * 2 * kPi;
    float dc = length(ref.p - pc);
    float ds = dc * cos_t - sqrtf(mx(0.f, sp.radius * sp.radius - dc * dc * sin_t * sin_t));
    float cos_a = (dc * dc + sp.radius * sp.radius - ds * ds) / (2 * dc * sp.radius);
    float sin_a = sqrtf(mx(0.f, 1 - cos_a * cos_a));
    float sphi, cphi;
    sincos_f(phi, &sphi, &cphi);
    F3 nw = sin_a * cphi * (-wcx) + sin_a * sphi * (-wcy) + cos_a * (-wc);
    F3 pw = pc + sp.radius * nw;
    LightSample it;
    it.p = pw;
    it.perr = kGamma5 * vabs(pw);
    it.n = nw;
    if (sp.reverse_orientation) it.n = it.n * -1.f;
    *pdf = 1 / (2 * kPi * (1 - cos_tmax));
    return it;
}
DEV float sphere_pdf(const DSphere &sp, const Isect &ref, F3 wi) {
    const F3 pc = F3{sp.center[0], sp.center[1], sp.center[2]};
    F3 porigin = offset_ray_origin(ref.p, ref.perr, ref.n, pc - ref.p);
    if (length_sq(porigin - pc) <= sp.radius * sp.radius) {
        F3 ro = offset_ray_origin(ref.p, ref.perr, ref.n, wi);
        float t;
        F3 od, ph;
        if (!sphere_test(sp, ro, wi, IILE_INF, &t, &od, &ph)) return 0;
        Isect li;
        sphere_interaction(sp, od, ph, &li);
        float pdf = length_sq(ref.p - li.p) / (absdot(li.n, -wi) * sphere_area(sp));
        if (is_inf(pdf)) pdf = 0.f;
        return pdf;
    }
    float sin_tmax2 = sp.radius * sp.radius / length_sq(ref.p - pc);
    float cos_tmax = sqrtf(mx(0.f, 1 - sin_tmax2));
    return 1 / (2 * kPi * (1 - cos_tmax));
}
DEV float quadric_area(const DQuadric &q) {
    if (q.kind == kQuadricDisk) return float(double(q.phi_max) * 0.5 * double(q.radius * q.radius - q.inner_radius * q.inner_radius));
    return (q.zmax - q.zmin) * q.radius * q.phi_max;
}
DEV LightSample quadric_sample_area(const DQuadric &q, float u0, float u1, float *pdf) {
    LightSample it;
    if (q.kind == kQuadricDisk) {
        float px, py;
        concentric_sample_disk(u0, u1, &px, &py);
        const F3 pobj = F3{px * q.radius, py * q.radius, q.height};
        it.n = normalize(xf_normal(q.o2w_inv, F3{0, 0, 1}));
        if (q.reverse_orientation) it.n = it.n * -1.f;
        it.p = xf_point_err2(q.o2w, pobj, F3{0, 0, 0}, &it.perr);
    } else {
        const float z = (1 - u0) * q.zmin + u0 * q.zmax;
        const float phi = u1 * q.phi_max;
        float s, c;
        sincos_f(phi, &s, &c);
        F3 pobj = F3{q.radius * c, q.radius * s, z};
        it.n = normalize(xf_normal(q.o2w_inv, F3{pobj.x, pobj.y, 0}));
        if (q.reverse_orientation) it.n = it.n * -1.f;
        const float hit_rad = sqrtf(pobj.x * pobj.x + pobj.y * pobj.y);
        pobj.x *= q.radius / hit_rad;
        pobj.y *= q.radius / hit_rad;
        const F3 pobj_err = kGamma3 * vabs(F3{pobj.x, pobj.y, 0});
// ... 77 lines not shown
    sincos_f(phi, &sin_phi, &cos_phi);
    const F3 wl = F3{sin_theta * cos_phi, sin_theta * sin_phi, cos_theta};
    *wi = F3{lt.l2w[0] * wl.x + lt.l2w[1] * wl.y + lt.l2w[2] * wl.z, lt.l2w[3] * wl.x + lt.l2w[4] * wl.y + lt.l2w[5] * wl.z,
             lt.l2w[6] * wl.x + lt.l2w[7] * wl.y + lt.l2w[8] * wl.z};
    *pdf = map_pdf / (2 * kPi * kPi * sin_theta);
    if (sin_theta == 0) *pdf = 0;
    *target = ref_p + *wi * (2 * lt.world_radius);
    return inf_lookup(S, lt, d0, d1);
}
DEV float inf_pdf_li(const DScene &S, const DLight &lt, F3 w) {
    const F3 wi = inf_w2l(lt, w);
    const float theta = spherical_theta(wi), phi = spherical_phi(wi);
    float sin_theta, cos_theta;
    sincos_f(theta, &sin_theta, &cos_theta);
    if (sin_theta <= 0) return 0;
    const float func_int = inf_cond(S, lt, lt.dist_h)[2 * lt.dist_h + 1];
    if (!(func_int > 0)) return 0;
    const float p0 = phi * kInv2Pi, p1 = theta * kInvPi;
    int iu = int(p0 * float(lt.dist_w)), iv = int(p1 * float(lt.dist_h));
    iu = iu < 0 ? 0 : (iu > lt.dist_w - 1 ? lt.dist_w - 1 : iu);
    iv = iv < 0 ? 0 : (iv > lt.dist_h - 1 ? lt.dist_h - 1 : iv);
    const float func = inf_cond(S, lt, iv)[iu];
    return (func / func_int) / (2 * kPi * kPi * sin_theta);
}

DEV float triangle_area(const DScene &S, int prim) {
    const float4 v0 = S.tri_verts[3 * size_t(prim)], v1 = S.tri_verts[3 * size_t(prim) + 1],
                 v2 = S.tri_verts[3 * size_t(prim) + 2];
    const F3 p0 = F3{v0.x, v0.y, v0.z}, p1 = F3{v1.x, v1.y, v1.z}, p2 = F3{v2.x, v2.y, v2.z};
    return float(0.5 * double(length(cross(p1 - p0, p2 - p0))));
}
DEV LightSample triangle_sample_area(const DScene &S, int prim, float u0, float u1, float *pdf) {
    const float su0 = sqrtf(u0);
    const float b0 = 1 - su0, b1 = u1 * su0;
    const float4 v0 = S.tri_verts[3 * size_t(prim)], v1 = S.tri_verts[3 * size_t(prim) + 1],
                 v2 = S.tri_verts[3 * size_t(prim) + 2];
    const F3 p0 = F3{v0.x, v0.y, v0.z}, p1 = F3{v1.x, v1.y, v1.z}, p2 = F3{v2.x, v2.y, v2.z};
    const uint32_t flags = f2b(v0.w);
    LightSample it;
    it.p = b0 * p0 + b1 * p1 + (1 - b0 - b1) * p2;
    it.n = normalize(cross(p1 - p0, p2 - p0));
    if (flags & 2u) {
        const float4 a = S.tri_norms[3 * size_t(prim)], b = S.tri_norms[3 * size_t(prim) + 1],
                     c = S.tri_norms[3 * size_t(prim) + 2];
        const F3 ns = b0 * F3{a.x, a.y, a.z} + b1 * F3{b.x, b.y, b.z} + (1 - b0 - b1) * F3{c.x, c.y, c.z};
        it.n = faceforward(it.n, ns);
    } else if (flags & 8u)
        it.n = it.n * -1.f;
    const F3 abs_sum = vabs(b0 * p0) + vabs(b1 * p1) + vabs((1 - b0 - b1) * p2);
    it.perr = kGamma6 * abs_sum;
    *pdf = 1 / triangle_area(S, prim);
    return it;
}
DEV LightSample shape_sample(const DScene &S, const DLight &lt, const Isect &ref, float u0, float u1, float *pdf) {
    if (lt.type == kLightDiffuseArea) return sphere_sample(S.spheres[lt.sphere], ref, u0, u1, pdf);
    if (lt.type == kLightAreaQuadric) return quadric_sample(S.quadrics[lt.quadric], ref, u0, u1, pdf);
    LightSample intr = triangle_sample_area(S, lt.prim, u0, u1, pdf);
    F3 wi = intr.p - ref.p;
    if (length_sq(wi) == 0)
        *pdf = 0;
    else {
        wi = normalize(wi);
        *pdf *= length_sq(ref.p - intr.p) / absdot(intr.n, -wi);
        if (is_inf(*pdf)) *pdf = 0.f;
    }
    return intr;
}
DEV float shape_pdf(const DScene &S, const DLight &lt, const Isect &ref, F3 wi, unsigned long long *n_tests,
                    unsigned long long *n_hits) {
    if (lt.type == kLightDiffuseArea) return sphere_pdf(S.spheres[lt.sphere], ref, wi);
    if (lt.type == kLightAreaQuadric) return quadric_pdf(S.quadrics[lt.quadric], ref, wi);
    const F3 o = offset_ray_origin(ref.p, ref.perr, ref.n, wi);
    const RayCtx rc = make_ray_ctx(o, wi);
    const int prim = lt.prim;
    const float4 v0 = S.tri_verts[3 * size_t(prim)], v1 = S.tri_verts[3 * size_t(prim) + 1],
                 v2 = S.tri_verts[3 * size_t(prim) + 2];
    const F3 p0 = F3{v0.x, v0.y, v0.z}, p1 = F3{v1.x, v1.y, v1.z}, p2 = F3{v2.x, v2.y, v2.z};
    float t, b0, b1, b2;
    ++*n_tests;
    if (!triangle_test(rc, IILE_INF, p0, p1, p2, &t, &b0, &b1, &b2)) return 0;
    ++*n_hits;
    Isect li;
    triangle_interaction(S, prim, f2b(v0.w), p0, p1, p2, wi, b0, b1, b2, &li);
    float pdf = length_sq(ref.p - li.p) / (absdot(li.n, -wi) * triangle_area(S, prim));
    if (is_inf(pdf)) pdf = 0.f;
    return pdf;
}
DEV float power_heuristic(float fpdf, float gpdf) {
    float f = 1 * fpdf, g = 1 * gpdf;
    return (f * f) / (f * f + g * g);
}

DEV F3 area_light_L(const DLight &lt, F3 n, F3 w) {
    return (lt.two_sided || dot(n, w) > 0) ? F3{lt.lemit[0], lt.lemit[1], lt.lemit[2]} : F3{0, 0, 0};
}
DEV F3 projection_light_projection(const DScene &S, const DLight &lt, F3 w) {
    const F3 wl = inf_w2l(lt, w);
    if (wl.z < lt.l2w[IILE_PROJ_HITHER]) return F3{0, 0, 0};
    float xp = lt.l2w[IILE_PROJ_M00] * wl.x;
    float yp = lt.l2w[IILE_PROJ_M11] * wl.y;
    const float wp = wl.z;
    if (wp != 1) {
        const float inv = 1.f / wp;
        xp = inv * xp;
        yp = inv * yp;
    }
    const float *sb = lt.l2w + IILE_PROJ_BOUNDS;
    const float x0 = sb[0], y0 = sb[1], x1 = sb[2], y1 = sb[3];
// ... 72 lines not shown
```

pbrt-v3-iile_amd/csrc/device/dpath.h:

```cpp
#pragma once
#include "dscene.h"

namespace iile {

DEV uint32_t div_magic(uint32_t a, uint32_t magic, uint32_t shift) {
    uint32_t t = __umulhi(magic, a);
    return (t + ((a - t) >> 1)) >> shift;
}

DEV uint32_t halton_index(const DScene &S, int px, int py, uint32_t k) {
    int pmx = px - (px / 128) * 128, pmy = py - (py / 128) * 128;
    if (pmx < 0) pmx += 128;
    if (pmy < 0) pmy += 128;
    return S.pixel_offsets[pmy * 128 + pmx] + k * uint32_t(S.sample_stride);
}

DEV float radical_inverse_base2(uint32_t a) {
    unsigned long long rev = (unsigned long long)__brev(a) << 32;
    return float(double(rev) * 0x1p-64);
}
DEV float radical_inverse_base3(uint32_t a0) {
    const float inv_base = 1.f / 3.f;
    double a = double(a0), reversed = 0;
    float inv_base_n = 1;
// ... 135 lines not shown
DEV void sample_dimensions_n(const DScene &S, PermPtr perms, int dim0, bool dim_uniform, int dim_lane, uint32_t index, float *out) {
    if (dim_lane < 2) __builtin_unreachable();
    if (S.sobol) {
#pragma unroll
        for (int i = 0; i < N; ++i) out[i] = sobol_sample_dimension(S, perms, index, dim_lane + i, 0, 0);
    } else if (dim_uniform) {
        scrambled_radical_inverse_n<N>(S, perms, dim0, index, out);
    } else {
        for (int i = 0; i < N; ++i) out[i] = sample_dimension_hi(S, perms, index, dim_lane + i);
    }
}

DEV uint32_t sample_slot(const DScene &S, int px, int py, uint32_t k) {
    int pmx = px - (px / 128) * 128, pmy = py - (py / 128) * 128;
    if (pmx < 0) pmx += 128;
    if (pmy < 0) pmy += 128;
    return uint32_t(pmy * 128 + pmx) * S.stab_spp + k;
}
DEV uint32_t slot_halton_index(const DScene &S, uint32_t slot) {
    const uint32_t cls = S.stab_spp > 1 ? div_magic(slot, S.stab_spp_magic, S.stab_spp_shift) : slot;
    return S.pixel_offsets[cls] + (slot - cls * S.stab_spp) * uint32_t(S.sample_stride);
}
DEV void record_continuation(const float4 &ra, const float4 &rb, int off, float *u0, float *u1, float *ur) {
    *u0 = off == 5 ? rb.y : (off == 1 ? ra.y : ra.x);
    *u1 = off == 5 ? rb.z : (off == 1 ? ra.z : ra.y);
    *ur = off == 5 ? rb.w : (off == 1 ? ra.w : ra.z);
}

DEV void concentric_sample_disk(float u0, float u1, float *dx, float *dy) {
    float ox = 2.f * u0 - 1, oy = 2.f * u1 - 1;
    if (ox == 0 && oy == 0) {
        *dx = 0;
        *dy = 0;
        return;
    }
    float theta, r;
    if (fabsf(ox) > fabsf(oy)) {
        r = ox;
        theta = kPiOver4 * (oy / ox);
    } else {
        r = oy;
        theta = kPiOver2 - kPiOver4 * (ox / oy);
    }
    float s, c;
    sincos_f(theta, &s, &c);
    *dx = r * c;
    *dy = r * s;
}
DEV F3 cosine_sample_hemisphere(float u0, float u1) {
    float dx, dy;
    concentric_sample_disk(u0, u1, &dx, &dy);
    float z = sqrtf(mx(0.f, 1 - dx * dx - dy * dy));
    return F3{dx, dy, z};
}

DEV float opaque_zero() {
    float z = 0.f;
    asm volatile("" : "+v"(z));
    return z;
}
static __device__ __attribute__((noinline)) F3 env_camera_direction(float pfx, float pfy, int xres, int yres) {
    const float theta = kPi * pfy / float(yres);
    const float phi = 2 * kPi * pfx / float(xres);
    float st, ct, sp, cp;
    sincos_f(theta, &st, &ct);
    sincos_f(phi, &sp, &cp);
    return F3{st * cp, ct, st * sp};
}
static __device__ __attribute__((noinline)) M44 camera_to_world_motion(const DCameraMotion *mo, float time) {
    if (time <= mo->start_time) return mo->c2w_start;
    if (time >= mo->end_time) return mo->c2w_end;
    const float dt = (time - mo->start_time) / (mo->end_time - mo->start_time);
    const float *T0 = mo->T[0], *T1 = mo->T[1], *q1 = mo->R[0], *q2 = mo->R[1];
    const float tx = (1 - dt) * T0[0] + dt * T1[0], ty = (1 - dt) * T0[1] + dt * T1[1], tz = (1 - dt) * T0[2] + dt * T1[2];
    float q[4];
    const float cos_theta = (q1[0] * q2[0] + q1[1] * q2[1] + q1[2] * q2[2]) + q1[3] * q2[3];
    if (cos_theta > .9995f) {
        for (int i = 0; i < 4; ++i) q[i] = (1 - dt) * q1[i] + dt * q2[i];
        const float len = sqrtf((q[0] * q[0] + q[1] * q[1] + q[2] * q[2]) + q[3] * q[3]), inv = 1.f / len;
        q[0] *= inv, q[1] *= inv, q[2] *= inv, q[3] = q[3] / len;
    } else {
        const float theta = acos_f(mn(mx(cos_theta, -1.f), 1.f));
        const float thetap = theta * dt;
        float qp[4];
        for (int i = 0; i < 4; ++i) qp[i] = q2[i] - q1[i] * cos_theta;
        const float len = sqrtf((qp[0] * qp[0] + qp[1] * qp[1] + qp[2] * qp[2]) + qp[3] * qp[3]), inv = 1.f / len;
        qp[0] *= inv, qp[1] *= inv, qp[2] *= inv, qp[3] = qp[3] / len;
        float st, ct;
        sincos_f(thetap, &st, &ct);
        for (int i = 0; i < 4; ++i) q[i] = q1[i] * ct + qp[i] * st;
    }
    const float xx = q[0] * q[0], yy = q[1] * q[1], zz = q[2] * q[2];
    const float xy = q[0] * q[1], xz = q[0] * q[2], yz = q[1] * q[2];
    const float wx = q[0] * q[3], wy = q[1] * q[3], wz = q[2] * q[3];
    float R[16] = {1 - 2 * (yy + zz), 2 * (xy - wz), 2 * (xz + wy), 0,
                   2 * (xy + wz), 1 - 2 * (xx + zz), 2 * (yz - wx), 0,
                   2 * (xz - wy), 2 * (yz + wx), 1 - 2 * (xx + yy), 0,
                   0, 0, 0, 1};
    float Tm[16] = {1, 0, 0, tx, 0, 1, 0, ty, 0, 0, 1, tz, 0, 0, 0, 1};
    float Sm[16] = {0, 0, 0, 0, 0, 0, 0, 0, 0, 0, 0, 0, 0, 0, 0, 1};
    for (int i = 0; i < 3; ++i)
        for (int j = 0; j < 3; ++j) Sm[4 * i + j] = (1 - dt) * mo->S[0][3 * i + j] + dt * mo->S[1][3 * i + j];
    float TR[16];
    M44 out;
    for (int i = 0; i < 4; ++i)
        for (int j = 0; j < 4; ++j)
// ... 536 lines not shown
    is->u = b0 * uv00 + b1 * uv10 + b2 * uv20;
    is->v = b0 * uv01 + b1 * uv11 + b2 * uv21;
    is->dpdu = dpdu;
    is->dpdv = dpdv;
    is->wo = normalize(-ray_d);
    F3 n = normalize(cross(dp02, dp12));
    const bool flip = (flags & 8u) != 0;
    if (flags & 2u) {
        const float4 *nn = S.tri_norms + 3 * size_t(prim);
        float4 a = nn[0], b = nn[1], c = nn[2];
        F3 n0 = F3{a.x, a.y, a.z}, n1 = F3{b.x, b.y, b.z}, n2 = F3{c.x, c.y, c.z};
        F3 ns = (b0 * n0 + b1 * n1 + b2 * n2);
        if (length_sq(ns) > 0)
            ns = normalize(ns);
        else
            ns = n;
        F3 ss = normalize(dpdu);
        F3 ts = cross(ss, ns);
        if (length_sq(ts) > 0.f) {
            ts = normalize(ts);
            ss = cross(ts, ns);
        } else
            coordinate_system(ns, &ss, &ts);
        const F3 dn1 = n0 - n2, dn2 = n1 - n2;
        if (double(fabsf(determinant)) < 1e-8) {
            is->dndu = is->dndv = F3{0, 0, 0};
        } else {
            const float inv_det = 1 / determinant;
            is->dndu = (duv12y * dn1 - duv02y * dn2) * inv_det;
            is->dndv = (-duv12x * dn1 + duv02x * dn2) * inv_det;
        }
        F3 sn = normalize(cross(ss, ts));
        if (flip) sn = -sn;
        n = faceforward(n, sn);
        is->sn = sn;
        is->sdpdu = ss;
        is->sdpdv = ts;
    } else {
        if (flip) n = -n;
        is->sn = n;
        is->sdpdu = dpdu;
        is->sdpdv = dpdv;
        is->dndu = is->dndv = F3{0, 0, 0};
    }
    is->flip = flip;
    is->n = n;
}

#include "dtrav.h"
#include "dtex.h"
#include "dbsdf.h"
#include "dlight.h"

template <bool EXT, bool COUNT, class BSDF>
DEV uint32_t estimate_direct_request(const DScene &S, const DLight &lt, const DSphere *lsp, const Isect &is, const BSDF &bsdf, float ul0,
                                     float ul1, float us0, float us1, F3 &so, F3 &sd, F3 &A, F3 &mo, F3 &md, F3 &Bc,
                                     unsigned long long *n_pdf_tests, unsigned long long *n_pdf_hits) {
    uint32_t nee_flags = 0;
    if (EXT && lt.type == kLightInfinite) {
        float light_pdf = 0, scattering_pdf = 0;
        F3 wi = F3{0, 0, 0}, target = F3{0, 0, 0};
        const F3 Li = inf_sample_li(S, lt, is.p, ul0, ul1, &wi, &light_pdf, &target);
        if (light_pdf > 0 && !is_black(Li)) {
            const F3 f = bsdf_f(bsdf, is.wo, wi) * absdot(wi, is.sn);
            scattering_pdf = bsdf_pdf(bsdf, is.wo, wi);
            if (!is_black(f)) {
                so = offset_ray_origin(is.p, is.perr, is.n, target - is.p);
                sd = target - so;
                A = sdiv(f * Li * power_heuristic(light_pdf, scattering_pdf), light_pdf);
                nee_flags |= NEE_HAS_SHADOW;
            }
        }
        F3 f2 = bsdf_sample_f(bsdf, is.wo, &wi, us0, us1, &scattering_pdf);
        f2 = f2 * absdot(wi, is.sn);
        if (!is_black(f2) && scattering_pdf > 0) {
            const float lp = inf_pdf_li(S, lt, wi);
            if (lp != 0) {
                mo = offset_ray_origin(is.p, is.perr, is.n, wi);
                md = wi;
                Bc = sdiv(f2 * inf_le(S, lt, wi) * power_heuristic(scattering_pdf, lp), scattering_pdf);
                nee_flags |= NEE_HAS_MIS;
            }
        }
    } else if (EXT && iile_light_is_delta(lt.type)) {
        F3 wi, target;
        const F3 Li = delta_light_li(S, lt, is.p, &wi, &target);
        if (!is_black(Li)) {
            const F3 f = bsdf_f(bsdf, is.wo, wi) * absdot(wi, is.sn);
            if (!is_black(f)) {
                so = offset_ray_origin(is.p, is.perr, is.n, target - is.p);
                sd = target - so;
                A = sdiv(f * Li, 1.f);
                nee_flags |= NEE_HAS_SHADOW;
            }
        }
    } else {
        float light_pdf = 0, scattering_pdf = 0;
        F3 wi = F3{0, 0, 0}, Li = F3{0, 0, 0};
        const LightSample ps = EXT ? shape_sample(S, lt, is, ul0, ul1, &light_pdf) : sphere_sample(*lsp, is, ul0, ul1, &light_pdf);
        if (light_pdf == 0 || length_sq(ps.p - is.p) == 0) {
            light_pdf = 0;
        } else {
            wi = normalize(ps.p - is.p);
            Li = area_light_L(lt, ps.n, -wi);
        }
        if (light_pdf > 0 && !is_black(Li)) {
            const F3 f = bsdf_f(bsdf, is.wo, wi) * absdot(wi, is.sn);
            scattering_pdf = bsdf_pdf(bsdf, is.wo, wi);
            if (!is_black(f)) {
                so = offset_ray_origin(is.p, is.perr, is.n, ps.p - is.p);
                const F3 target = offset_ray_origin(ps.p, ps.perr, ps.n, so - ps.p);
                sd = target - so;
                A = sdiv(f * Li * power_heuristic(light_pdf, scattering_pdf), light_pdf);
                nee_flags |= NEE_HAS_SHADOW;
            }
        }
        F3 f2 = bsdf_sample_f(bsdf, is.wo, &wi, us0, us1, &scattering_pdf);
        f2 = f2 * absdot(wi, is.sn);
        if (!is_black(f2) && scattering_pdf > 0) {
            const F3 m_o = offset_ray_origin(is.p, is.perr, is.n, wi);
            bool can_reach = true;
            if (!COUNT && lt.type == kLightDiffuseArea) {
                float t_l;
                F3 od_l, ph_l;
                can_reach = sphere_test(lsp ? *lsp : S.spheres[lt.sphere], m_o, wi, IILE_INF, &t_l, &od_l, &ph_l);
            } else if (EXT && !COUNT && lt.type == kLightAreaQuadric) {
                float t_l;
                F3 od_l, ph_l;
                can_reach = quadric_test(S.quadrics[lt.quadric], m_o, wi, IILE_INF, &t_l, &od_l, &ph_l);
            }
            if (can_reach) {
                const float lp = EXT ? shape_pdf(S, lt, is, wi, n_pdf_tests, n_pdf_hits) : sphere_pdf(*lsp, is, wi);
                if (lp != 0) {
                    mo = m_o;
                    md = wi;
                    Bc = sdiv(f2 * F3{lt.lemit[0], lt.lemit[1], lt.lemit[2]} * power_heuristic(scattering_pdf, lp), scattering_pdf);
                    nee_flags |= NEE_HAS_MIS;
                }
            }
        }
    }
    return nee_flags;
}

DEV bool mis_ray_lit(const DScene &S, int li, int prim, float b0, float b1, float b2, F3 mo, F3 md) {
    const DLight &lt = S.lights[li];
    Isect lis;
    if (lt.type == kLightAreaTriangle) {
        const float4 v0 = S.tri_verts[3 * size_t(prim)], v1 = S.tri_verts[3 * size_t(prim) + 1], v2 = S.tri_verts[3 * size_t(prim) + 2];
        triangle_interaction(S, prim, f2b(v0.w), F3{v0.x, v0.y, v0.z}, F3{v1.x, v1.y, v1.z}, F3{v2.x, v2.y, v2.z}, md, b0, b1, b2, &lis);
    } else {
        shape_hit_interaction(S, lt.type == kLightAreaQuadric ? ~lt.quadric : lt.sphere, mo, md, &lis);
    }
    return lt.two_sided || dot(lis.n, -md) > 0;
}

}
```

pbrt-v3-iile_amd/csrc/device/dscene.h:

```cpp
#pragma once
#include "../../../include/iile_scene.h"
#include "dmath.h"

namespace iile {

struct DSphere {
    M44 o2w, o2w_inv;
    float radius, zmin, zmax, theta_min, theta_max, phi_max;
    int reverse_orientation, swaps_handedness;
    float center[3];
    float pad_;
};
enum { kQuadricDisk = 0, kQuadricCylinder = 1 };
struct DQuadric {
    M44 o2w, o2w_inv;
    int kind;
    float radius, inner_radius, height, zmin, zmax, phi_max;
    int reverse_orientation, swaps_handedness;
};
enum { kMatMatte = 0, kMatPlastic = 1, kMatUber = 2, kMatMirror = 3, kMatGlass = 4, kMatMetal = 5, kMatSubstrate = 6,
       kMatTranslucent = 8, kMatDisney = 10 };
struct alignas(16) DMaterial {
    int type;
    float kd[3];
// ... 113 lines not shown
    int light_nv[3];
    int has_infinite;
    int extended_features;
    int all_lights_infinite;
    int has_glass;
    int has_uber_trans;
    int has_specular;
    int has_alpha;
    int rare_prims;
    int boxes_nested;
    M44 raster_to_camera, camera_to_world;
    float lens_radius, focal_distance;
    float dx_camera[3], dy_camera[3];
    int env_camera;
    float diff_scale;
    int xres, yres;
    int crop_x0, crop_y0, crop_x1, crop_y1;
    int samp_x0, samp_y0, samp_x1, samp_y1;
    int pb_x0, pb_y0, pb_x1, pb_y1;
    int pb_set;
    float filter_rx, filter_ry, max_sample_luminance;
    int probe_mode;
    int filter_wide;
    const float *filter_table;
    int base_scale0, base_scale1, base_exp0, base_exp1, sample_stride, mult_inv0, mult_inv1;
    int sample_center;
    const float2 *stab_cam;
    const float2 *stab_lens;
    const float4 *stab_shade;
    uint32_t stab_slots;
    uint32_t stab_spp;
    uint32_t stab_spp_magic, stab_spp_shift;
    int sobol, sobol_log2res, sobol_res, sobol_dims;
    const uint32_t *sobol_mat;
    const uint32_t *sobol_vdc;
    const uint32_t *sobol_bt;
    const uint32_t *sobol_vdc_bt;
    int max_depth;
    float rr_threshold;
};
static_assert(sizeof(DScene) == 672, "DScene keeps its size: the kernels take it by value, and their register allocation follows its layout");
constexpr int kPixelOffsets = 128 * 128;
inline __host__ __device__ const DCameraMotion *camera_motion(const DScene &S) {
    return reinterpret_cast<const DCameraMotion *>(S.pixel_offsets + kPixelOffsets);
}
inline __host__ __device__ const iile_disney *disney_table(const DScene &S) {
    return reinterpret_cast<const iile_disney *>(S.materials + S.n_materials);
}
inline void clear_sample_table(DScene *S) {
    S->stab_cam = S->stab_lens = nullptr;
    S->stab_shade = nullptr;
    S->stab_slots = S->stab_spp = S->stab_spp_magic = S->stab_spp_shift = 0;
}

enum { NEE_HAS_SHADOW = 1, NEE_HAS_MIS = 2 };

struct DCounters {
    unsigned long long camera_rays, closest_rays, shadow_rays;
    unsigned long long nodes_closest, nodes_any, tri_tests, tri_hits, sphere_tests;
    unsigned long long nee_evals, zero_radiance;
    unsigned long long path_length[8];
    unsigned long long ext_rays, ext_nodes, ext_tri_tests, ext_sphere_tests;
    unsigned long long any_tri_tests;
    unsigned long long mis_traced;
    unsigned long long ext_traced;
};

}
```

pbrt-v3-iile_amd/csrc/device/kernels.h:

```cpp
#pragma once
#include <string>

#include "../../../include/iile_scene.h"
#include "dscene.h"

namespace iile {

struct PassDesc {
    int n_tiles_x, n_tiles_y, tile_rank, tile_nranks, n_owned_tiles;
    const int *tile_of_slot, *slot_of_tile;
    int slot0, n_pass_tiles;
    int k0, kc;
    uint32_t n_paths;
    const int *list_px, *list_py, *list_k;
    int probe_mode, probe_tiles, probe_stx;
    const DProbeCam *probe_cams;
    int gen_fused;
    int skip_last_bounce;
    uint32_t direct_seed;
    int direct_arrays;
    const unsigned long long *direct_jump;
    const int *direct_nsamples;
    int direct_total_samples;
    int direct_levels;
// ... 6 lines not shown
    float4 *L;
    float4 *beta;
    uint32_t *hindex;
    float *eta_scale;
    float4 *ray_o[2];
    float4 *ray_d[2];
    float4 *ray_s[2];
    float4 *hits;
    float4 *mis_hit;
    float4 *nee_alt, *mis_hit_alt;
    uint8_t *nee_mis_alt;
    float4 *nee;
    uint8_t *nee_mis;
    uint32_t *shade_q;
    uint32_t *counts;
    DCounters *counters;
    uint32_t *nray_out;
    int *spill;
    float4 *aux;
    uint32_t *flag_count;
    float *flag_rec;
    float4 *dir_E, *dir_F;
    float4 *dir_RD;
    uint32_t dir_paths;
};
constexpr uint32_t kMaxFlagged = 1u << 20;

struct FilmBuffers {
    float4 *tile_rgbw;
    float4 *k0_rgbv;
    float4 *film_xyzw;
    float4 *wide_L;
    float2 *wide_pf;
};

struct PatchDev {
    uint32_t *counters;
    uint4 *hits;
    uint32_t *keys;
    uint32_t *heads;
    uint32_t table_mask;
    uint4 *ent_a;
    float4 *ent_b;
    uint32_t cap_hits, cap_entries;
};
constexpr uint32_t kPatchNil = 0xffffffffu;

struct LaunchCfg {
    int n_cus;
    hipStream_t stream;
    bool count_stats;
    int trav_blocks_per_cu = 0;
    bool camera_moves = false;
};

int api_fail(int code, const std::string &msg);
int check_bvh_nodes(const iile_bvh_node *nodes, int n_nodes, int64_t max_prims, const char *prefix, int *n_interior);
int pack_wide_records(const iile_bvh_node *d_nodes, int n_nodes, int n_interior, float4 *d_wide, float4 *d_wide4, int *nested_out,
                      const int *d_remap = nullptr);

uint32_t queue_capacity(uint32_t n_paths, int n_cus);
void launch_generate(const DScene &S, const PassDesc &P, const PassBuffers &B, const LaunchCfg &cfg);
void launch_extend(const DScene &S, const PassDesc &P, const PassBuffers &B, int bounce, uint32_t max_rays, const LaunchCfg &cfg);
void launch_shade(const DScene &S, const PassDesc &P, const PassBuffers &B, int bounce, uint32_t max_rays, const LaunchCfg &cfg);
void launch_shade_motion(const DScene &S, const PassDesc &P, const PassBuffers &B, int bounce, uint32_t max_rays, const LaunchCfg &cfg);
void launch_shadow(const DScene &S, const PassBuffers &B, int bounce, uint32_t max_rays, const LaunchCfg &cfg);
void launch_mis(const DScene &S, const PassBuffers &B, int bounce, uint32_t max_rays, const LaunchCfg &cfg);
void launch_light_distributions(const DScene &S, const float *samples, float *out, const LaunchCfg &cfg);
void launch_sample_table(const DScene &S, float2 *cam, float2 *lens, float4 *shade, const LaunchCfg &cfg);
void launch_sample_table_time(const DScene &S, float *time, const LaunchCfg &cfg);
void launch_sample_table_read(const DScene &S, int n, const int *px, const int *py, const int *k, const int *bounce, float *out, const LaunchCfg &cfg);
void launch_miss(const DScene &S, const PassBuffers &B, int bounce, uint32_t max_rays, const LaunchCfg &cfg);
void launch_mis_lit(const DScene &S, const PassBuffers &B, int bounce, uint32_t max_rays, const LaunchCfg &cfg);
void launch_direct_generate(const DScene &S, const PassDesc &P, const PassBuffers &B, const LaunchCfg &cfg);
void launch_direct_shade(const DScene &S, const PassDesc &P, const PassBuffers &B, int depth, uint32_t max_rays, const LaunchCfg &cfg);
void launch_direct_tree(const DScene &S, const PassDesc &P, const PassBuffers &B, double *film_rgbw, const LaunchCfg &cfg);
void launch_direct_miss(const DScene &S, const PassBuffers &B, int depth, uint32_t max_rays, const LaunchCfg &cfg);
void launch_direct_fold(const DScene &S, const PassDesc &P, const PassBuffers &B, double *film_rgbw, const LaunchCfg &cfg);

void launch_film_accumulate(const DScene &S, const PassDesc &P, const PassBuffers &B, const FilmBuffers &F, const LaunchCfg &cfg);
void launch_film_resolve(const DScene &S, const PassDesc &P, const FilmBuffers &F, const LaunchCfg &cfg);
void launch_patch_pass(const DScene &S, const PassDesc &P, const PassBuffers &B, const FilmBuffers &F, const PatchDev &D, const LaunchCfg &cfg);
void launch_patch_merge(const DScene &S, const PassDesc &P, const FilmBuffers &F, const PatchDev &D, const LaunchCfg &cfg);
void launch_film_store(const DScene &S, const PassDesc &P, const PassBuffers &B, const FilmBuffers &F, int k_begin, int n_samples, const LaunchCfg &cfg);
void launch_film_gather(const DScene &S, const PassDesc &P, const FilmBuffers &F, int n_samples, const LaunchCfg &cfg);
void launch_probe_finish(const DScene &S, const PassDesc &P, const PassBuffers &B, const FilmBuffers &F, int n_probes, float *intensity, float *normals,
                         float *distance, const LaunchCfg &cfg);
bool launch_probe_film(const DScene &S, const PassDesc &P, const PassBuffers &B, int n_probes, float *intensity, float *normals, float *distance,
                       const LaunchCfg &cfg);
int probe_film_tiles(const DScene &S);
void launch_probe_film_add(const DScene &S, const PassDesc &P, const PassBuffers &B, int n_probes, float4 *acc, int n_ord, float *normals, float *distance,
                           const LaunchCfg &cfg);
void launch_probe_film_resolve(const DScene &S, const PassDesc &P, int n_probes, float4 *acc, int n_ord, float *intensity, float *weight_sum, const LaunchCfg &cfg);

struct AoBuffers {
    float4 *ray_o, *ray_d;
    float *term;
    uint8_t *vis;
    uint32_t *hit_pid;
    int n_samples, cos_sample;
};
constexpr int kCntAoHits = 16, kCntAoHead = 64;
void launch_ao_rays(const DScene &S, const PassDesc &P, const PassBuffers &B, const AoBuffers &A, const LaunchCfg &cfg);
void launch_ao_occlude(const DScene &S, const PassBuffers &B, const AoBuffers &A, uint32_t max_rays, const LaunchCfg &cfg);
void launch_ao_fold(const PassDesc &P, const PassBuffers &B, const AoBuffers &A, const LaunchCfg &cfg);
void launch_ao_array_probe(const DScene &S, int n_samples, int n, const int *px, const int *py, const int *k, const int *j, float *out2, const LaunchCfg &cfg);

struct DHemiCam {
    M44 c2w;
    float w2c[9];
    float look[3], origin[3];
    int valid;
};
struct IisptItems {
    float4 *ro, *rd, *beta, *hit, *pf;
    uint32_t *idx;
    uint32_t *n_active;
    int n_items, n_hemi, nx;
};
struct IisptJob {
    iile_iispt_task T;
    IisptItems I;
    int ny;
    uint8_t *valid;
// ... 42 lines not shown
```

pbrt-v3-iile_amd/csrc/device/kernels_shade.hip:

```cpp
#include <cstdlib>
#include <type_traits>

#include "kcommon.h"

namespace iile {

DEV F3 sample_li_plain(const DScene &S, const DLight &lt, F3 po, float u0, float u1, float *pdf) {
    *pdf = 1;
    if (lt.type == kLightInfinite) {
        F3 wi, target;
        return inf_sample_li(S, lt, po, u0, u1, &wi, pdf, &target);
    }
    if (iile_light_is_delta(lt.type)) {
        F3 wi, target;
        return delta_light_li(S, lt, po, &wi, &target);
    }
    Isect ref;
    ref.p = po;
    ref.perr = F3{0, 0, 0};
    ref.n = F3{0, 0, 0};
    const LightSample ps = shape_sample(S, lt, ref, u0, u1, pdf);
    if (*pdf == 0 || length_sq(ps.p - po) == 0) {
        *pdf = 0;
        return F3{0, 0, 0};
// ... 38 lines not shown
    for (int j = 0; j < n; ++j) {
        const float f = mx(d[j], min_contrib);
        d[j] = f;
        cdf = cdf + f / float(n);
        d[n + 1 + j] = cdf;
    }
    const float func_int = cdf;
    d[2 * n + 1] = func_int;
    for (int i = 1; i < n + 1; ++i) {
        if (func_int == 0)
            d[n + i] = float(i) / float(n);
        else
            d[n + i] = d[n + i] / func_int;
    }
}

__global__ __launch_bounds__(256) void k_sample_table(DScene S, float2 *cam, float2 *lens, float4 *shade) {
    const uint32_t slot = blockIdx.x * blockDim.x + threadIdx.x;
    if (slot >= S.stab_slots) return;
    const uint32_t idx = slot_halton_index(S, slot);
    if (blockIdx.y == 0) {
        cam[slot] = make_float2(sample_dimension(S, idx, 0), sample_dimension(S, idx, 1));
        if (lens) lens[slot] = make_float2(sample_dimension(S, idx, 3), sample_dimension(S, idx, 4));
        return;
    }
    const int b = int(blockIdx.y) - 1, d0 = 5 + 7 * b;
    float r[8];
    for (int i = 0; i < 8; ++i) r[i] = sample_dimension_hi(S, S.perms, idx, d0 + i);
    float4 *rec = shade + (size_t(b) * S.stab_slots + slot) * 2;
    rec[0] = make_float4(r[0], r[1], r[2], r[3]);
    rec[1] = make_float4(r[4], r[5], r[6], r[7]);
}
__global__ __launch_bounds__(256) void k_sample_table_time(DScene S, float *time) {
    const uint32_t slot = blockIdx.x * blockDim.x + threadIdx.x;
    if (slot >= S.stab_slots) return;
    time[slot] = sample_dimension(S, slot_halton_index(S, slot), 2);
}
__global__ void k_sample_table_read(DScene S, int n, const int *px, const int *py, const int *k, const int *bounce, float *out) {
    const int i = blockIdx.x * blockDim.x + threadIdx.x;
    if (i >= n) return;
    const uint32_t slot = sample_slot(S, px[i], py[i], uint32_t(k[i]));
    float4 a = make_float4(0, 0, 0, 0), b = make_float4(0, 0, 0, 0);
    if (bounce[i] < 0) {
        const float2 c = S.stab_cam[slot];
        a.x = c.x, a.y = c.y;
        if (S.stab_lens) a.z = S.stab_lens[slot].x, a.w = S.stab_lens[slot].y;
    } else {
        const float4 *rec = S.stab_shade + (size_t(bounce[i]) * S.stab_slots + slot) * 2;
        a = rec[0], b = rec[1];
    }
    reinterpret_cast<float4 *>(out)[2 * size_t(i)] = a;
    reinterpret_cast<float4 *>(out)[2 * size_t(i) + 1] = b;
}
#endif

#ifndef IILE_SHADE_WAVES
#define IILE_SHADE_WAVES 4
#endif
#ifndef IILE_SHADE_WAVES_TEX
#define IILE_SHADE_WAVES_TEX 3
#endif
#ifndef IILE_SHADE_WAVES_DISNEY
#define IILE_SHADE_WAVES_DISNEY 2
#endif
constexpr int shade_waves(bool tex, bool disney = false) { return disney ? IILE_SHADE_WAVES_DISNEY : (tex ? IILE_SHADE_WAVES_TEX : IILE_SHADE_WAVES); }
#ifndef IILE_SHADE_TAB_REREAD
#define IILE_SHADE_TAB_REREAD 0
#endif
template <bool COUNT, bool EXT, bool TEX, bool TAB = false, bool DIS = false, bool MOT = false>
__global__ __launch_bounds__(kBlock, shade_waves(TEX, DIS)) void k_shade(DScene S, PassDesc P, PassBuffers B, int bounce, uint32_t plane) {
    static_assert(!(TAB && COUNT), "the instrumented build keeps the digit chains");
    static_assert(!DIS || (EXT && TEX && !COUNT), "the Disney builds are textured ones");
    static_assert(!MOT || (TEX && (DIS || COUNT)), "the moving camera's builds are the instrumented one and the Disney builds");
    constexpr bool DZ = DIS || COUNT;
    typename std::conditional<TAB, const uint16_t *, lds_u16 *>::type s_perms;
    if constexpr (TAB) {
        s_perms = S.perms;
    } else {
        extern __shared__ __attribute__((aligned(16))) uint16_t s_perms_raw[];
        if (S.sobol) {
        } else {
            for (int i = threadIdx.x; i < S.n_perms; i += kBlock) s_perms_raw[i] = S.perms[i];
        }
        __syncthreads();
        s_perms = (lds_u16 *)s_perms_raw;
    }
    const uint32_t count = B.counts[kCntShade + bounce];
    const float4 *ro = B.ray_o[bounce & 1], *rd = B.ray_d[bounce & 1];
    float4 *no = B.ray_o[(bounce + 1) & 1], *nd = B.ray_d[(bounce + 1) & 1];
    const float4 *rs = B.ray_s[bounce & 1];
    float4 *ns = B.ray_s[(bounce + 1) & 1];
    unsigned long long n_nee = 0, n_term = 0, n_pdf_tests = 0, n_pdf_hits = 0;
    DiagSums<IILE_SWITCH(IILE_SHADE_STAMPS) && !COUNT, 8> stamps;
    WaveOut ray_out{0, 0}, nee_out{0, 0}, mis_out{0, 0};
    auto pad_ray = [&](uint32_t sl) { no[sl] = make_float4(0, 0, 0, b2f(kInvalid)); };
    auto pad_nee = [&](uint32_t sl) { B.nee[plane + sl] = B.nee[4 * plane + sl] = make_float4(0, 0, 0, b2f(kInvalid)); };
    auto pad_mis = [&](uint32_t sl) { B.nee[2 * plane + sl] = make_float4(0, 0, 0, b2f(kInvalid)); };
    __shared__ uint32_t s_entry[kWavesPerBlock][kShadeChunk];
    const int lane = threadIdx.x & 63, wave = threadIdx.x >> 6;
    uint32_t *const head = &B.counts[kCntShdHead + bounce];
    for (;;) {
        uint32_t base = 0;
        if (lane == 0) base = atomicAdd(head, uint32_t(kShadeChunk));
        base = __builtin_amdgcn_readfirstlane(base);
        if (base >= count) break;
        uint32_t ent[kShadeChunk / 64];
#pragma unroll
        for (int j = 0; j < kShadeChunk / 64; ++j) {
            const uint32_t qi = base + uint32_t(j) * 64u + uint32_t(lane);
            ent[j] = qi < count ? B.shade_q[qi] : kInvalid;
        }
        uint32_t run = 0;
        for (uint32_t c = 0; c < 8; ++c) {
#pragma unroll
            for (int j = 0; j < kShadeChunk / 64; ++j) {
                const bool is_c = (ent[j] == kInvalid ? 7u : ent[j] >> kSlotBits) == c;
                const uint64_t m = __ballot(is_c);
                if (is_c)
                    s_entry[wave][run + __builtin_amdgcn_mbcnt_hi(uint32_t(m >> 32), __builtin_amdgcn_mbcnt_lo(uint32_t(m), 0u))] = ent[j];
                run += uint32_t(__popcll(m));
            }
        }
        __builtin_amdgcn_fence(__ATOMIC_ACQ_REL, "wavefront");
        __builtin_amdgcn_wave_barrier();
        stamps.mark(0);
      for (int round = 0; round < kShadeChunk / 64; ++round) {
        const uint32_t mine = s_entry[wave][round * 64 + lane];
        const bool valid = mine != kInvalid;
        if (__ballot(valid) == 0) break;
        const uint32_t slot = mine & ((1u << kSlotBits) - 1u);
        bool surface = false;
        bool alive = false, returned_early = false;
        uint32_t pid = 0, hidx = 0;
        int dim = 0;
        bool tab_wave = false;
        float4 rec_a = make_float4(0, 0, 0, 0), rec_b = make_float4(0, 0, 0, 0);
        auto chain_index = [&]() { return TAB ? slot_halton_index(S, hidx) : hidx; };
        Isect is;
        typename bsdf_of<DZ>::type bsdf;
        F3 beta = F3{0, 0, 0}, ray_d = F3{0, 0, 1};
        uint32_t state_next = 0;
        {
            bool emit_nee = false;
            F3 so = F3{0, 0, 0}, sd = F3{0, 0, 1}, mo = F3{0, 0, 0}, md = F3{0, 0, 1};
            F3 A = F3{0, 0, 0}, Bc = F3{0, 0, 0};
            uint32_t nee_flags = 0, nee_light = 0;
            float light_sel_pdf = 1.f;
            if (valid) {
                float4 o4, d4;
                uint32_t fused_hidx = 0;
                const float4 h4 = B.hits[slot];
                if (bounce == 0 && P.gen_fused) {
                    const float4 cpf = B.beta[slot];
                    fused_hidx = f2b(cpf.z);
                    float cl0 = 0, cl1 = 0;
                    if (S.lens_radius > 0) {
                        if (TAB) {
                            const float2 cl = S.stab_lens[fused_hidx];
                            cl0 = cl.x, cl1 = cl.y;
                        } else {
                            cl0 = sample_dimension(S, s_perms, fused_hidx, 3);
                            cl1 = sample_dimension(S, s_perms, fused_hidx, 4);
                        }
                    }
                    F3 co, cd;
                    float ctm;
                    camera_ray<false>(S, cpf.x, cpf.y, cl0, cl1, &co, &cd, &ctm, opaque_zero());
                    o4 = make_float4(co.x, co.y, co.z, b2f(slot));
                    d4 = make_float4(cd.x, cd.y, cd.z, ctm);
                } else {
                    o4 = ro[slot];
                    d4 = rd[slot];
                }
                pid = f2b(o4.w);
                const float4 beta4 = bounce == 0 ? make_float4(1, 1, 1, 0) : rs[slot];
                const uint32_t state_w = bounce == 0 ? 5u : f2b(d4.w);
                beta = F3{beta4.x, beta4.y, beta4.z};
                dim = int(state_w & 0xffffu);
                const bool prev_specular = EXT && (state_w >> 16) != 0;
                hidx = bounce == 0 ? ((P.gen_fused) ? fused_hidx : B.hindex[pid]) : f2b(beta4.w);
                float u_nee[4] = {0, 0, 0, 0};
                if (bounce < S.max_depth) {
                    const int dim_u = __builtin_amdgcn_readfirstlane(dim);
                    const bool dim_uniform = __ballot(dim != dim_u) == 0;
                    if (TAB) {
                        tab_wave = dim_uniform && dim_u == 5 + 7 * bounce;
                        if (tab_wave) {
                            const float4 *rec = S.stab_shade + (size_t(bounce) * S.stab_slots + hidx) * 2;
                            rec_a = rec[0];
                            rec_b = rec[1];
                            u_nee[0] = rec_a.y, u_nee[1] = rec_a.z, u_nee[2] = rec_a.w, u_nee[3] = rec_b.x;
                        } else {
                            sample_dimensions_n<4>(S, s_perms, dim_u + 1, false, dim + 1, chain_index(), u_nee);
                        }
                    } else {
                        sample_dimensions_n<4>(S, s_perms, dim_u + 1, dim_uniform, dim + 1, hidx, u_nee);
                    }
                }
                stamps.mark(1);
                const int prim = int(f2b(h4.x));
                const F3 ray_o = F3{o4.x, o4.y, o4.z};
                ray_d = F3{d4.x, d4.y, d4.z};
                float4 v0 = S.tri_verts[3 * size_t(prim)];
                float4 v1 = S.tri_verts[3 * size_t(prim) + 1];
                float4 v2 = S.tri_verts[3 * size_t(prim) + 2];
                keep_whole(v0, v1, v2);
                const uint32_t flags = f2b(v0.w);
                const int material = int(f2b(v1.w)), light = int(f2b(v2.w));
                if (flags & 1u) {
                    shape_hit_interaction<TEX, EXT>(S, S.prim_shape[prim], ray_o, ray_d, &is);
                } else {
                    triangle_interaction(S, prim, flags, F3{v0.x, v0.y, v0.z}, F3{v1.x, v1.y, v1.z},
                                         F3{v2.x, v2.y, v2.z}, ray_d, h4.y, h4.z, h4.w, &is);
                }
                if (EXT && S.probe_mode && bounce == 0) {
                    const F3 cv = is.p - ray_o;
                    const DProbeCam &cam = P.probe_cams[(pid / uint32_t(P.kc)) / (256u * uint32_t(P.probe_tiles))];
                    B.aux[pid] = make_float4(cam.nrm[0] * is.n.x + cam.nrm[1] * is.n.y + cam.nrm[2] * is.n.z,
                                             cam.nrm[3] * is.n.x + cam.nrm[4] * is.n.y + cam.nrm[5] * is.n.z,
                                             cam.nrm[6] * is.n.x + cam.nrm[7] * is.n.y + cam.nrm[8] * is.n.z, sqrtf(dot(cv, cv)));
                }
                if (((bounce == 0 && !(EXT && S.probe_mode)) || prev_specular) && light >= 0) {
                    const float4 L4 = B.L[pid];
                    const F3 L = F3{L4.x, L4.y, L4.z} + beta * area_light_L(S.lights[light], is.n, -ray_d);
                    B.L[pid] = make_float4(L.x, L.y, L.z, 0);
                }
                if (bounce < S.max_depth) {
                    surface = true;
                    if (TEX && S.textured_materials) {
                        const DMaterial &m0 = S.materials[material];
                        if (m0.kd_tex >= 0 || m0.ks_tex >= 0 || m0.kr_tex >= 0 || m0.kt_tex >= 0 || m0.bump_tex >= 0 || m0.rough_tex >= 0 || m0.sigma_tex >= 0 || m0.opacity_tex >= 0 || m0.rough_tex_v >= 0) {
                            TexDiff td = TexDiff{0, 0, 0, 0};
                            F3 dpdx = F3{0, 0, 0}, dpdy = F3{0, 0, 0};
                            if (bounce == 0) {
                                int px = 0, py = 0;
                                uint32_t kk = 0;
                                path_pixel(S, P, pid, &px, &py, &kk);
                                float u0, u1, l0 = 0, l1 = 0, time = 0;
                                if (TAB) {
                                    const float2 cu = S.stab_cam[hidx];
                                    u0 = cu.x, u1 = cu.y;
                                    if (S.lens_radius > 0) {
                                        const float2 cl = S.stab_lens[hidx];
                                        l0 = cl.x, l1 = cl.y;
                                    }
                                    if (MOT) time = camera_ray_time(S, camera_motion(S)->stab_time[hidx]);
                                } else {
                                    u0 = sample_dimension(S, s_perms, hidx, 0, px, py), u1 = sample_dimension(S, s_perms, hidx, 1, px, py);
                                    if (S.lens_radius > 0) {
                                        l0 = sample_dimension(S, s_perms, hidx, 3);
                                        l1 = sample_dimension(S, s_perms, hidx, 4);
                                    }
                                    if (MOT) time = camera_ray_time(S, sample_dimension(S, s_perms, hidx, 2));
                                }
                                const RayDiff rdiff =
                                    S.probe_mode ? probe_differentials(S, P.probe_cams[(pid / uint32_t(P.kc)) / (256u * uint32_t(P.probe_tiles))],
                                                                       float(px) + u0, float(py) + u1, ray_o, ray_d)
                                                 : camera_differentials<MOT>(S, float(px) + u0, float(py) + u1, l0, l1, ray_o, ray_d, time);
                                td = compute_differentials(is, rdiff, &dpdx, &dpdy);
                            }
                            if (m0.bump_tex >= 0) bump(S, m0.bump_tex, td, dpdx, dpdy, &is);
                            const DMaterial mm = textured_material(S, m0, is, td, dpdx, dpdy);
                            bsdf = make_bsdf_at<EXT, DZ>(S, material, mm, is);
                        } else {
                            bsdf = make_bsdf_at<EXT, DZ>(S, material, m0, is);
                        }
                    } else {
                        bsdf = make_bsdf_at<EXT, DZ>(S, material, S.materials[material], is);
                    }
                    stamps.mark(2);
                    if (n_nonspec(bsdf) > 0) {
                        ++n_nee;
                        int li = 0;
                        if (EXT && S.n_lights > 1) {
                            float ul;
                            if (TAB && tab_wave)
                                ul = rec_a.x;
                            else
                                ul = sample_dimension_hi(S, s_perms, chain_index(), dim);
                            li = sample_light(S, is.p, ul, &light_sel_pdf);
                        }
                        if (S.n_lights > 0) ++dim;
                        if (S.n_lights > 0 && light_sel_pdf != 0) {
                            DLight lt_u;
                            DSphere lsp_u;
                            if (!EXT) {
                                lt_u = uniform_entry(S.lights, 0);
                                lsp_u = uniform_entry(S.spheres, lt_u.sphere);
                            }
                            const DLight &lt = EXT ? S.lights[li] : lt_u;
                            const DSphere &lsp = EXT ? S.spheres[lt.sphere] : lsp_u;
                            dim += 4;
                            nee_flags = estimate_direct_request<EXT, COUNT>(S, lt, &lsp, is, bsdf, u_nee[0], u_nee[1], u_nee[2], u_nee[3], so, sd,
                                                                            A, mo, md, Bc, &n_pdf_tests, &n_pdf_hits);
                            stamps.mark(3);
                            nee_light = uint32_t(li);
                            emit_nee = COUNT || nee_flags != 0;
                        }
                    }
                }
            }
            stamps.mark(4);
            const uint32_t eslot = out_take(nee_out, &B.counts[kCntNee + bounce], emit_nee, pad_nee);
            const bool emit_mis = emit_nee && (nee_flags & NEE_HAS_MIS) != 0;
            const uint32_t mslot = out_take(mis_out, &B.counts[kCntMis + bounce], emit_mis, pad_mis);
            if (emit_nee) {
                B.nee[eslot] = make_float4(so.x, so.y, so.z, light_sel_pdf);
                B.nee[plane + eslot] = make_float4(sd.x, sd.y, sd.z, b2f(nee_flags));
                if (nee_flags & NEE_HAS_MIS) {
                    B.nee[4 * plane + eslot] = make_float4(A.x, A.y, A.z, b2f(pid));
                    B.nee[5 * plane + eslot] = make_float4(Bc.x, Bc.y, Bc.z, b2f(nee_light));
                    B.nee[6 * plane + eslot] = make_float4(beta.x, beta.y, beta.z, b2f(pid));
                } else {
                    const F3 Ld = F3{0, 0, 0} + A;
                    const F3 pre = (__ballot(light_sel_pdf != 1.f) == 0) ? beta * Ld : beta * sdiv(Ld, light_sel_pdf);
                    B.nee[4 * plane + eslot] = make_float4(pre.x, pre.y, pre.z, b2f(pid));
                }
            }
            if (emit_mis) {
                B.nee[2 * plane + mslot] = make_float4(mo.x, mo.y, mo.z, b2f(eslot));
                B.nee[3 * plane + mslot] = make_float4(md.x, md.y, md.z, b2f(nee_light));
            }
        }
        stamps.mark(5);
        F3 next_o = F3{0, 0, 0}, next_d = F3{0, 0, 1};
        if (P.skip_last_bounce == 2 && bounce + 1 >= S.max_depth) surface = false;
        if (surface) {
            float u_bsdf[2], ur_tab = 0;
            if (TAB && tab_wave) {
                const int off = dim - (5 + 7 * bounce);
                if (IILE_SHADE_TAB_REREAD) {
                    const float *rf = reinterpret_cast<const float *>(S.stab_shade + (size_t(bounce) * S.stab_slots + hidx) * 2) + off;
                    u_bsdf[0] = rf[0], u_bsdf[1] = rf[1];
                    if (bounce > 3) ur_tab = rf[2];
                } else {
                    record_continuation(rec_a, rec_b, off, &u_bsdf[0], &u_bsdf[1], &ur_tab);
                }
            } else {
                const int dim_u = __builtin_amdgcn_readfirstlane(dim);
                sample_dimensions_n<2>(S, s_perms, dim_u, !TAB && __ballot(dim != dim_u) == 0, dim, chain_index(), u_bsdf);
            }
            const float u0 = u_bsdf[0], u1 = u_bsdf[1];
            dim += 2;
            float pdf = 0;
            F3 wi = F3{0, 0, 0};
            bool sampled_specular = false, sampled_transmission = false;
            const F3 f = bsdf_sample_f(bsdf, -ray_d, &wi, u0, u1, &pdf, EXT, &sampled_specular, &sampled_transmission);
            float eta_scale = 1.f;
            if (EXT && S.has_glass && bounce > 0) eta_scale = B.eta_scale[pid];
            if (!(is_black(f) || pdf == 0.f)) {
                beta = beta * sdiv(f * absdot(wi, is.sn), pdf);
                const float by = lum_y(beta);
                if (by < 0.f || is_nan(by)) {
                    returned_early = true;
                } else {
                    next_o = offset_ray_origin(is.p, is.perr, is.n, wi);
                    next_d = wi;
                    alive = true;
                    if (sampled_specular && sampled_transmission) {
                        const float eta = bsdf.path_eta;
                        eta_scale *= (dot(-ray_d, is.n) > 0) ? (eta * eta) : 1 / (eta * eta);
                    }
                    const F3 rr_beta = beta * eta_scale;
                    const float mc = max3(rr_beta.x, rr_beta.y, rr_beta.z);
                    if (mc < S.rr_threshold && bounce > 3) {
                        const float q = mx(.05f, 1 - mc);
                        float ur;
                        if (TAB && tab_wave)
                            ur = ur_tab;
                        else
                            ur = sample_dimension_hi(S, s_perms, chain_index(), dim);
                        ++dim;
                        if (ur < q)
                            alive = false;
                        else
                            beta = sdiv(beta, 1 - q);
                    }
                }
            }
            if (EXT && P.skip_last_bounce == 1 && bounce + 1 >= S.max_depth && !sampled_specular) alive = false;
            if (EXT && alive && S.has_glass) B.eta_scale[pid] = eta_scale;
            state_next = uint32_t(dim) | (sampled_specular ? 0x10000u : 0u);
        }
        if (COUNT && valid && !alive && !returned_early) ++n_term;
        stamps.mark(6);
        const uint32_t nslot = out_take(ray_out, &B.counts[kCntRay + bounce + 1], alive, pad_ray);
        if (alive) {
            no[nslot] = make_float4(next_o.x, next_o.y, next_o.z, b2f(pid));
            nd[nslot] = make_float4(next_d.x, next_d.y, next_d.z, b2f(state_next));
            ns[nslot] = make_float4(beta.x, beta.y, beta.z, b2f(hidx));
        }
        stamps.mark(7);
      }
        __builtin_amdgcn_wave_barrier();
    }
    out_flush(ray_out, pad_ray);
    out_flush(nee_out, pad_nee);
    out_flush(mis_out, pad_mis);
    stamps.flush(B.counters, 0);
    if (COUNT) {
        flush_counter(&B.counters->nee_evals, n_nee);
        flush_counter(&B.counters->path_length[bounce < 7 ? bounce : 7], n_term);
        flush_counter(&B.counters->tri_tests, n_pdf_tests);
        flush_counter(&B.counters->tri_hits, n_pdf_hits);
    }
}


#ifdef IILE_SHADE_MOTION_TU
void launch_shade_motion(const DScene &S, const PassDesc &P, const PassBuffers &B, int bounce, uint32_t max_rays, const LaunchCfg &cfg) {
    const dim3 grid(grid_blocks(max_rays, cfg.n_cus, shade_waves(true, !cfg.count_stats)));
    const size_t perm_bytes = S.sobol ? size_t(16) : (size_t(S.n_perms) * sizeof(uint16_t) + 15) & ~size_t(15);
    if (cfg.count_stats)
        hipLaunchKernelGGL((k_shade<true, true, true, false, false, true>), grid, dim3(kBlock), perm_bytes, cfg.stream, S, P, B, bounce, B.queue_cap);
    else if (S.stab_shade)
        hipLaunchKernelGGL((k_shade<false, true, true, true, true, true>), grid, dim3(kBlock), 0, cfg.stream, S, P, B, bounce, B.queue_cap);
    else
        hipLaunchKernelGGL((k_shade<false, true, true, false, true, true>), grid, dim3(kBlock), perm_bytes, cfg.stream, S, P, B, bounce, B.queue_cap);
}
#else
void launch_shade(const DScene &S, const PassDesc &P, const PassBuffers &B, int bounce, uint32_t max_rays, const LaunchCfg &cfg) {
    const bool tex_build = cfg.count_stats || S.textured_materials || S.probe_mode;
    if (cfg.camera_moves && tex_build && !S.probe_mode) return launch_shade_motion(S, P, B, bounce, max_rays, cfg);
    const bool dis_build = S.disney_build && !cfg.count_stats;
    const dim3 grid(grid_blocks(max_rays, cfg.n_cus, shade_waves(tex_build, dis_build)));
    const size_t perm_bytes = S.sobol ? size_t(16) : (size_t(S.n_perms) * sizeof(uint16_t) + 15) & ~size_t(15);
    if (dis_build) {
        if (S.stab_shade)
            hipLaunchKernelGGL((k_shade<false, true, true, true, true>), grid, dim3(kBlock), 0, cfg.stream, S, P, B, bounce, B.queue_cap);
        else
            hipLaunchKernelGGL((k_shade<false, true, true, false, true>), grid, dim3(kBlock), perm_bytes, cfg.stream, S, P, B, bounce, B.queue_cap);
    } else if (S.stab_shade && !cfg.count_stats) {
        if (S.textured_materials)
            hipLaunchKernelGGL((k_shade<false, true, true, true>), grid, dim3(kBlock), 0, cfg.stream, S, P, B, bounce, B.queue_cap);
        else if (S.extended_features)
            hipLaunchKernelGGL((k_shade<false, true, false, true>), grid, dim3(kBlock), 0, cfg.stream, S, P, B, bounce, B.queue_cap);
        else
            hipLaunchKernelGGL((k_shade<false, false, false, true>), grid, dim3(kBlock), 0, cfg.stream, S, P, B, bounce, B.queue_cap);
    } else if (cfg.count_stats)
        hipLaunchKernelGGL((k_shade<true, true, true>), grid, dim3(kBlock), perm_bytes, cfg.stream, S, P, B, bounce, B.queue_cap);
    else
        if (S.textured_materials || S.probe_mode)
            hipLaunchKernelGGL((k_shade<false, true, true>), grid, dim3(kBlock), perm_bytes, cfg.stream, S, P, B, bounce, B.queue_cap);
        else if (S.extended_features)
            hipLaunchKernelGGL((k_shade<false, true, false>), grid, dim3(kBlock), perm_bytes, cfg.stream, S, P, B, bounce, B.queue_cap);
        else
            hipLaunchKernelGGL((k_shade<false, false, false>), grid, dim3(kBlock), perm_bytes, cfg.stream, S, P, B, bounce, B.queue_cap);
}
void launch_sample_table(const DScene &S, float2 *cam, float2 *lens, float4 *shade, const LaunchCfg &cfg) {
    hipLaunchKernelGGL(k_sample_table, dim3((S.stab_slots + 255) / 256, 1 + S.max_depth), dim3(256), 0, cfg.stream, S, cam, lens, shade);
}
void launch_sample_table_time(const DScene &S, float *time, const LaunchCfg &cfg) {
    hipLaunchKernelGGL(k_sample_table_time, dim3((S.stab_slots + 255) / 256), dim3(256), 0, cfg.stream, S, time);
}
void launch_sample_table_read(const DScene &S, int n, const int *px, const int *py, const int *k, const int *bounce, float *out, const LaunchCfg &cfg) {
    hipLaunchKernelGGL(k_sample_table_read, dim3((n + 127) / 128), dim3(128), 0, cfg.stream, S, n, px, py, k, bounce, out);
}
void launch_light_distributions(const DScene &S, const float *samples, float *out, const LaunchCfg &cfg) {
    const int n = S.light_nv[0] * S.light_nv[1] * S.light_nv[2];
    for (int l0 = 0; l0 < S.n_lights; l0 += 32768) {
        DScene part = S;
        part.lights = S.lights + l0;
        part.n_lights = std::min(S.n_lights - l0, 32768);
        hipLaunchKernelGGL(k_light_contrib, dim3((n + 127) / 128, part.n_lights), dim3(128), 0, cfg.stream, part, samples, out + l0,
                           light_record_floats(S.n_lights));
    }
    hipLaunchKernelGGL(k_light_cdf, dim3((n + 127) / 128), dim3(128), 0, cfg.stream, S, out);
}

#endif

}
```

Before: 12080.

## Precompute warped sample directions into a warp plane beside the sample table

Adds a per-slot, per-bounce warp plane built at scene setup. It stores the cosine-hemisphere directions and the sphere-cone phi sin/cos derived from the sample table's random numbers. The shade kernel gets a WARP variant that reads these precomputed directions for single-lobe Lambert BSDF sampling and NEE light sampling instead of computing the trigonometry per ray. This trades arithmetic for extra memory traffic and doubles the sample-table footprint. It falls back to the old path when the budget is exceeded or the camera moves.

```diff
diff --git a/include/iile_gpu.h b/include/iile_gpu.h
--- a/include/iile_gpu.h
+++ b/include/iile_gpu.h
@@ -81,6 +81,10 @@
 uint64_t iile_sample_table_budget(void);
 void iile_test_sample_table_budget(uint64_t bytes);
 uint64_t iile_sample_table_bytes(const iile_scene *scene);
+uint64_t iile_warp_table_bytes(const iile_scene *scene);
+int iile_warp_table_records(iile_scene *scene, int32_t n, const int32_t *px, const int32_t *py, const int32_t *k, const int32_t *bounce,
+                            float *out8);
+int iile_warp_probe(int32_t n, const float *rec8, float *out8);
 int iile_camera_rays(iile_scene *scene, int32_t n, const float *pfilm2, const float *plens2, float *o3, float *d3);
 int iile_camera_rays_at(iile_scene *scene, int32_t n, const float *pfilm2, const float *plens2, float time, float *o3, float *d3);
 int iile_li_samples(iile_scene *scene, int32_t n, const int32_t *px, const int32_t *py, const int32_t *k,
diff --git a/pbrt-v3-iile_amd/binding.py b/pbrt-v3-iile_amd/binding.py
--- a/pbrt-v3-iile_amd/binding.py
+++ b/pbrt-v3-iile_amd/binding.py
@@ -218,7 +218,7 @@
 GPU_SYMBOLS = ["iile_device_count", "iile_last_error", "iile_scene_create", "iile_scene_destroy", "iile_render",
                "iile_scene_set_camera_motion", "iile_camera_rays_at",
                "iile_render_ao", "iile_ao_array_samples", "iile_ao_li_samples",
-               "iile_trace_closest", "iile_trace_any", "iile_shape_hit_attributes", "iile_halton_samples", "iile_sample_table_records", "iile_sample_table_budget", "iile_test_sample_table_budget", "iile_sample_table_bytes", "iile_camera_rays", "iile_li_samples",
+               "iile_trace_closest", "iile_trace_any", "iile_shape_hit_attributes", "iile_halton_samples", "iile_sample_table_records", "iile_sample_table_budget", "iile_test_sample_table_budget", "iile_sample_table_bytes", "iile_warp_table_bytes", "iile_warp_table_records", "iile_warp_probe", "iile_camera_rays", "iile_li_samples",
                "iile_bsdf_eval", "iile_bsdf_sample", "iile_bsdf_eval_ng", "iile_bsdf_sample_ng", "iile_bsdf_sample_specular", "iile_trig_probe", "iile_texture_eval", "iile_texture_eval_p", "iile_light_sample_li", "iile_light_sample_at", "iile_light_pdf_at", "iile_light_le", "iile_light_choose", "iile_render_probes",
                "iile_render_probes_reference", "iile_test_probe_ref_group", "iile_reference_points",
                "iile_device_select", "iile_device_alloc", "iile_device_free", "iile_device_download", "iile_device_upload", "iile_device_zero",
@@ -369,6 +369,10 @@
         lib.iile_test_sample_table_budget.restype = None
         lib.iile_sample_table_bytes.argtypes = [c_vp]
         lib.iile_sample_table_bytes.restype = c_u64
+        lib.iile_warp_table_bytes.argtypes = [c_vp]
+        lib.iile_warp_table_bytes.restype = c_u64
+        lib.iile_warp_table_records.argtypes = [c_vp, c_i32, c_vp, c_vp, c_vp, c_vp, c_vp]
+        lib.iile_warp_probe.argtypes = [c_i32, c_vp, c_vp]
         lib.iile_iispt_net_create.argtypes = [ctypes.POINTER(NetWeights), ctypes.POINTER(c_vp)]
         lib.iile_iispt_net_load.argtypes = [ctypes.c_char_p, ctypes.POINTER(c_vp)]
         lib.iile_iispt_net_forward.argtypes = [c_vp, c_vp, c_vp, c_i32, c_i32, c_vp, c_vp, c_i32]
@@ -714,6 +718,7 @@
             return film, None
         d = st.as_dict()
         d["sample_table_bytes"] = int(gpu_lib().iile_sample_table_bytes(self._s))
+        d["warp_table_bytes"] = int(gpu_lib().iile_warp_table_bytes(self._s))
         return film, d
 
     def _ao_params(self, nsamples, cossample):
@@ -806,6 +811,13 @@
         f.argtypes = [c_vp, c_i32, c_vp, c_vp, c_vp, c_vp, c_vp]
         self._check(f(self._s, len(px), px.ctypes.data, py.ctypes.data, k.ctypes.data, bounce.ctypes.data, out.ctypes.data),
                     "iile_sample_table_records")
+        return out
+
+    def warp_table_records(self, px, py, k, bounce):
+        px, py, k, bounce = _i32(px), _i32(py), _i32(k), _i32(bounce)
+        out = np.empty((len(px), 8), np.float32)
+        self._check(gpu_lib().iile_warp_table_records(self._s, len(px), px.ctypes.data, py.ctypes.data, k.ctypes.data, bounce.ctypes.data,
+                                                      out.ctypes.data), "iile_warp_table_records")
         return out
 
     def camera_rays(self, pfilm, plens=None):
@@ -1150,6 +1162,15 @@
     return {"lds_stack": int(out[0]), "top_records": int(out[1]), "max_bvh_depth": int(out[2])}
 
 
+def warp_probe(rec8):
+    rec8 = np.ascontiguousarray(rec8, np.float32).reshape(-1, 8)
+    out = np.empty_like(rec8)
+    rc = gpu_lib().iile_warp_probe(len(rec8), rec8.ctypes.data, out.ctypes.data)
+    if rc != 0:
+        raise RuntimeError(f"iile_warp_probe failed ({rc}): {gpu_lib().iile_last_error().decode()}")
+    return out
+
+
 def trig_probe(x):
     x = _f32(x)
     out = np.empty((len(x), 3), np.float32)
diff --git a/pbrt-v3-iile_amd/csrc/device/api_common.h b/pbrt-v3-iile_amd/csrc/device/api_common.h
--- a/pbrt-v3-iile_amd/csrc/device/api_common.h
+++ b/pbrt-v3-iile_amd/csrc/device/api_common.h
@@ -110,6 +110,7 @@
     const uint32_t *probe_pixel_offsets = nullptr;
     const float *probe_filter_table = nullptr;
     uint64_t sample_table_bytes = 0;
+    uint64_t warp_table_bytes = 0;
     void *stab_block = nullptr;
     bool camera_moves = false;
     float shutter[2] = {0.f, 1.f};
diff --git a/pbrt-v3-iile_amd/csrc/device/api_probes.hip b/pbrt-v3-iile_amd/csrc/device/api_probes.hip
--- a/pbrt-v3-iile_amd/csrc/device/api_probes.hip
+++ b/pbrt-v3-iile_amd/csrc/device/api_probes.hip
@@ -130,6 +130,33 @@
 uint64_t iile_sample_table_budget(void) { return sample_table_budget(); }
 void iile_test_sample_table_budget(uint64_t bytes) { set_sample_table_budget(bytes); }
 uint64_t iile_sample_table_bytes(const iile_scene *sc) { return sc ? sc->sample_table_bytes : 0; }
+uint64_t iile_warp_table_bytes(const iile_scene *sc) { return sc ? sc->warp_table_bytes : 0; }
+
+int iile_warp_table_records(iile_scene *sc, int32_t n, const int32_t *px, const int32_t *py, const int32_t *k, const int32_t *bounce,
+                            float *out8) {
+    if (!sc || n < 0 || !px || !py || !k || !bounce || !out8) return api_fail(IILE_ERR_ARG, "iile_warp_table_records: bad argument");
+    if (!sc->ds.stab_shade || !sc->warp_table_bytes) return api_fail(IILE_ERR_ARG, "iile_warp_table_records: the scene has no warp plane");
+    for (int i = 0; i < n; ++i)
+        if (k[i] < 0 || uint32_t(k[i]) >= sc->ds.stab_spp || bounce[i] < 0 || bounce[i] >= sc->ds.max_depth)
+            return api_fail(IILE_ERR_ARG, "iile_warp_table_records: sample or bounce outside the plane");
+    int rc = ensure_device();
+    if (rc) return rc;
+    DevBuf<int> dx, dy, dk, db;
+    DevBuf<float> dout;
+    if ((rc = dx.put(px, n)) || (rc = dy.put(py, n)) || (rc = dk.put(k, n)) || (rc = db.put(bounce, n)) || (rc = dout.alloc(size_t(n) * 8))) return rc;
+    if (n) launch_sample_warp_read(sc->ds, n, dx.p, dy.p, dk.p, db.p, dout.p, probe_cfg(sc));
+    return finish(dout, out8, size_t(n) * 8);
+}
+
+int iile_warp_probe(int32_t n, const float *rec8, float *out8) {
+    if (n < 0 || !rec8 || !out8) return api_fail(IILE_ERR_ARG, "iile_warp_probe: bad argument");
+    int rc = ensure_device();
+    if (rc) return rc;
+    DevBuf<float> din, dout;
+    if ((rc = din.put(rec8, size_t(n) * 8)) || (rc = dout.alloc(size_t(n) * 8))) return rc;
+    if (n) launch_warp_probe(n, din.p, dout.p, LaunchCfg{256, nullptr, false});
+    return finish(dout, out8, size_t(n) * 8);
+}
 
 int iile_camera_rays(iile_scene *sc, int32_t n, const float *pfilm2, const float *plens2, float *o3, float *d3) {
     if (!sc || n < 0 || !pfilm2 || !o3 || !d3) return api_fail(IILE_ERR_ARG, "iile_camera_rays: bad argument");
diff --git a/pbrt-v3-iile_amd/csrc/device/api_render.hip b/pbrt-v3-iile_amd/csrc/device/api_render.hip
--- a/pbrt-v3-iile_amd/csrc/device/api_render.hip
+++ b/pbrt-v3-iile_amd/csrc/device/api_render.hip
@@ -247,6 +247,8 @@
     DScene S = S_in;
     if (cfg.count_stats || P.list_px || S.probe_mode || P.k0 < 0 || uint64_t(P.k0) + uint64_t(P.kc) > uint64_t(S.stab_spp) || max_depth > S.max_depth)
         clear_sample_table(&S);
+    LaunchCfg cfg_shade = cfg;
+    cfg_shade.warp_table = S.stab_shade && sc->warp_table_bytes != 0;
     P.gen_fused = !cfg.count_stats && !P.list_px && !S.has_infinite && !S.probe_mode && !B.nray_out && !S.env_camera && !cfg.camera_moves;
     HIP_TRY(hipMemsetAsync(B.counts, 0, kCntWords * sizeof(uint32_t), cfg.stream));
     auto timed_launch_on = [&](hipStream_t stream, int kind, auto &&fn) -> int { return timed_step(sc, timed, stream, kind, fn); };
@@ -282,7 +284,7 @@
         if (two_streams && !nee_doubled && b > 0) HIP_TRY(hipStreamWaitEvent(cfg.stream, sc->ev_nee[b - 1], 0));
         if (nee_doubled && b > 1) HIP_TRY(hipStreamWaitEvent(cfg.stream, sc->ev_nee[b - 2], 0));
         const PassBuffers B_shade = buffers_of(b, false), B_nee = buffers_of(b, true);
-        rc = timed_launch(2, [&] { launch_shade(S, P, B_shade, b, B.queue_cap, cfg); });
+        rc = timed_launch(2, [&] { launch_shade(S, P, B_shade, b, B.queue_cap, cfg_shade); });
         if (rc) return rc;
         if (b < max_depth) {
             if (two_streams) {
diff --git a/pbrt-v3-iile_amd/csrc/device/api_scene.hip b/pbrt-v3-iile_amd/csrc/device/api_scene.hip
--- a/pbrt-v3-iile_amd/csrc/device/api_scene.hip
+++ b/pbrt-v3-iile_amd/csrc/device/api_scene.hip
@@ -711,11 +711,10 @@
     return IILE_OK;
 }
 
-int build_sample_table(iile_scene *sc, const iile_scene_desc &d) {
+int build_sample_table_of(iile_scene *sc, int64_t spp, bool with_warp) {
     DScene &S = sc->ds;
     clear_sample_table(&S);
-    sc->sample_table_bytes = 0;
-    const int64_t spp = d.halton.spp;
+    sc->sample_table_bytes = sc->warp_table_bytes = 0;
     if (S.sobol || S.max_depth <= 0 || spp <= 0 || S.sample_stride <= 0 || std::getenv("IILE_NO_SAMPLE_TABLE")) return IILE_OK;
     if (5 + 7 * int64_t(S.max_depth) >= int64_t(S.n_hdims)) return IILE_OK;
     const bool lens = S.lens_radius > 0;
@@ -723,6 +722,8 @@
     if (uint64_t(spp) > sample_table_budget() / (uint64_t(16384) * per_slot)) return IILE_OK;
     const uint64_t slots = uint64_t(16384) * uint64_t(spp);
     if (slots >= (uint64_t(1) << 32)) return IILE_OK;
+    const uint64_t warp_bytes = slots * uint64_t(32) * uint64_t(S.max_depth);
+    bool warp_on = with_warp && !std::getenv("IILE_NO_WARP_TABLE") && warp_bytes <= sample_table_budget() - slots * per_slot;
     const auto t0 = std::chrono::steady_clock::now();
     S.stab_slots = uint32_t(slots), S.stab_spp = uint32_t(spp);
     if (spp > 1) {
@@ -736,11 +737,16 @@
     auto layout = [&](Carver c) {
         cam = c.take<float2>(slots);
         if (lens) lens_part = c.take<float2>(slots);
-        shade = c.take<float4>(slots * uint64_t(S.max_depth) * 2);
+        shade = c.take<float4>(slots * uint64_t(S.max_depth) * (warp_on ? 4 : 2));
         return c.used;
     };
     void *block = nullptr;
-    if (hipMalloc(&block, layout(Carver())) != hipSuccess) {
+    if (warp_on && hipMalloc(&block, layout(Carver())) != hipSuccess) {
+        (void)hipGetLastError();
+        block = nullptr;
+        warp_on = false;
+    }
+    if (!block && hipMalloc(&block, layout(Carver())) != hipSuccess) {
         (void)hipGetLastError();
         clear_sample_table(&S);
         return IILE_OK;
@@ -752,9 +758,24 @@
     if (hipDeviceSynchronize() != hipSuccess || hipGetLastError() != hipSuccess) return api_fail(IILE_ERR_HIP, "sample table kernel failed");
     S.stab_cam = cam, S.stab_lens = lens_part, S.stab_shade = shade;
     sc->sample_table_bytes = slots * per_slot;
+    if (warp_on) {
+        launch_sample_warp(S, shade, const_cast<float4 *>(warp_plane(S)), LaunchCfg{sc->n_cus, nullptr, false});
+        if (hipDeviceSynchronize() != hipSuccess || hipGetLastError() != hipSuccess) return api_fail(IILE_ERR_HIP, "warp plane kernel failed");
+        sc->warp_table_bytes = warp_bytes;
+    }
     if (std::getenv("IILE_TIMING"))
-        fprintf(stderr, "iile timing: sample table of %.1f MiB built in %.3f s\n", double(sc->sample_table_bytes) / 1048576.0,
-                std::chrono::duration<double>(std::chrono::steady_clock::now() - t0).count());
+        fprintf(stderr, "iile timing: sample table of %.1f MiB and warp plane of %.1f MiB built in %.3f s\n", double(sc->sample_table_bytes) / 1048576.0,
+                double(sc->warp_table_bytes) / 1048576.0, std::chrono::duration<double>(std::chrono::steady_clock::now() - t0).count());
+    return IILE_OK;
+}
+int build_sample_table(iile_scene *sc, const iile_scene_desc &d) { return build_sample_table_of(sc, d.halton.spp, true); }
+int drop_sample_table(iile_scene *sc) {
+    for (void *&p : sc->allocs)
+        if (p == sc->stab_block) p = nullptr;
+    HIP_TRY(hipFree(sc->stab_block));
+    sc->stab_block = nullptr;
+    clear_sample_table(&sc->ds);
+    sc->sample_table_bytes = sc->warp_table_bytes = 0;
     return IILE_OK;
 }
 
@@ -900,6 +921,10 @@
     for (int k = 0; k < 2; ++k)
         for (int i = 0; i < 3; ++i)
             for (int j = 0; j < 3; ++j) dm.S[k][3 * i + j] = mo->S[k][4 * i + j];
+    if (S.stab_cam && sc->warp_table_bytes && sc->sample_table_bytes + sc->warp_table_bytes + 4 * uint64_t(S.stab_slots) > sample_table_budget()) {
+        const int64_t spp = S.stab_spp;
+        if ((rc = drop_sample_table(sc)) || (rc = build_sample_table_of(sc, spp, false))) return rc;
+    }
     if (S.stab_cam) {
         const uint64_t slots = S.stab_slots;
         void *time = nullptr;
@@ -908,12 +933,7 @@
             time = nullptr;
         }
         if (!time) {
-            for (void *&p : sc->allocs)
-                if (p == sc->stab_block) p = nullptr;
-            HIP_TRY(hipFree(sc->stab_block));
-            sc->stab_block = nullptr;
-            clear_sample_table(&S);
-            sc->sample_table_bytes = 0;
+            if ((rc = drop_sample_table(sc))) return rc;
         } else {
             sc->allocs.push_back(time);
             launch_sample_table_time(S, static_cast<float *>(time), LaunchCfg{sc->n_cus, nullptr, false});
diff --git a/pbrt-v3-iile_amd/csrc/device/dbsdf.h b/pbrt-v3-iile_amd/csrc/device/dbsdf.h
--- a/pbrt-v3-iile_amd/csrc/device/dbsdf.h
+++ b/pbrt-v3-iile_amd/csrc/device/dbsdf.h
@@ -390,8 +390,9 @@
     const int matching = n_nonspec(b);
     return matching > 0 ? pdf / matching : 0.f;
 }
+template <class WARP = NoWarp>
 DEV F3 bsdf_sample_f(const Bsdf &b, F3 woW, F3 *wiW, float u0, float u1, float *pdf, const bool allow_specular = false,
-                     bool *sampled_specular = nullptr, bool *sampled_transmission = nullptr) {
+                     bool *sampled_specular = nullptr, bool *sampled_transmission = nullptr, WARP warp = WARP()) {
     if (sampled_specular) *sampled_specular = false;
     if (sampled_transmission) *sampled_transmission = false;
     const int matching = allow_specular ? b.n_lobes : n_nonspec(b);
@@ -426,7 +427,13 @@
     *pdf = 0;
     F3 wi = F3{0, 0, 0}, f;
     if (pick == kLobeLambert) {
-        wi = cosine_sample_hemisphere(ur0, u1);
+        if constexpr (WARP::on) {
+            LambertWarp lw = warp;
+            lw.use = lw.use && matching == 1;
+            wi = cosine_sample_hemisphere(ur0, u1, lw);
+        } else {
+            wi = cosine_sample_hemisphere(ur0, u1);
+        }
         if (wo.z < 0) wi.z *= -1;
         *pdf = lambert_pdf(wo, wi);
         f = diffuse_f(b, wo, wi);
@@ -805,7 +812,7 @@
     return dz_lobes_pdf(b, -1, wo, wi, 0.f) / b.n_lobes;
 }
 DEV F3 bsdf_sample_f(const DisneyBsdf &b, F3 woW, F3 *wiW, float u0, float u1, float *pdf, const bool allow_specular = false,
-                     bool *sampled_specular = nullptr, bool *sampled_transmission = nullptr) {
+                     bool *sampled_specular = nullptr, bool *sampled_transmission = nullptr, NoWarp = NoWarp()) {
     if (!b.disney) return bsdf_sample_f(static_cast<const Bsdf &>(b), woW, wiW, u0, u1, pdf, allow_specular, sampled_specular, sampled_transmission);
     if (sampled_specular) *sampled_specular = false;
     if (sampled_transmission) *sampled_transmission = false;
diff --git a/pbrt-v3-iile_amd/csrc/device/dlight.h b/pbrt-v3-iile_amd/csrc/device/dlight.h
--- a/pbrt-v3-iile_amd/csrc/device/dlight.h
+++ b/pbrt-v3-iile_amd/csrc/device/dlight.h
@@ -22,7 +22,9 @@
     *pdf = 1 / sphere_area(sp);
     return it;
 }
-DEV LightSample sphere_sample(const DSphere &sp, const Isect &ref, float u0, float u1, float *pdf) {
+DEV float sphere_cone_phi(float u1) { return u1 * 2 * kPi; }
+template <class CONE = NoWarp>
+DEV LightSample sphere_sample(const DSphere &sp, const Isect &ref, float u0, float u1, float *pdf, CONE cone = CONE()) {
     const F3 pc = F3{sp.center[0], sp.center[1], sp.center[2]};
     F3 porigin = offset_ray_origin(ref.p, ref.perr, ref.n, pc - ref.p);
     if (length_sq(porigin - pc) <= sp.radius * sp.radius) {
@@ -44,13 +46,20 @@
     float cos_tmax = sqrtf(mx(0.f, 1 - sin_tmax2));
     float cos_t = (1 - u0) + u0 * cos_tmax;
     float sin_t = sqrtf(mx(0.f, 1 - cos_t * cos_t));
-    float phi = u1 * 2 * kPi;
+    float phi = sphere_cone_phi(u1);
     float dc = length(ref.p - pc);
     float ds = dc * cos_t - sqrtf(mx(0.f, sp.radius * sp.radius - dc * dc * sin_t * sin_t));
     float cos_a = (dc * dc + sp.radius * sp.radius - ds * ds) / (2 * dc * sp.radius);
     float sin_a = sqrtf(mx(0.f, 1 - cos_a * cos_a));
     float sphi, cphi;
-    sincos_f(phi, &sphi, &cphi);
+    if constexpr (CONE::on) {
+        sphi = cone.sin_phi, cphi = cone.cos_phi;
+        if (__ballot(!cone.use) != 0) {
+            if (!cone.use) sincos_f(phi, &sphi, &cphi);
+        }
+    } else {
+        sincos_f(phi, &sphi, &cphi);
+    }
     F3 nw = sin_a * cphi * (-wcx) + sin_a * sphi * (-wcy) + cos_a * (-wc);
     F3 pw = pc + sp.radius * nw;
     LightSample it;
@@ -234,8 +243,9 @@
     *pdf = 1 / triangle_area(S, prim);
     return it;
 }
-DEV LightSample shape_sample(const DScene &S, const DLight &lt, const Isect &ref, float u0, float u1, float *pdf) {
-    if (lt.type == kLightDiffuseArea) return sphere_sample(S.spheres[lt.sphere], ref, u0, u1, pdf);
+template <class CONE = NoWarp>
+DEV LightSample shape_sample(const DScene &S, const DLight &lt, const Isect &ref, float u0, float u1, float *pdf, CONE cone = CONE()) {
+    if (lt.type == kLightDiffuseArea) return sphere_sample(S.spheres[lt.sphere], ref, u0, u1, pdf, cone);
     if (lt.type == kLightAreaQuadric) return quadric_sample(S.quadrics[lt.quadric], ref, u0, u1, pdf);
     LightSample intr = triangle_sample_area(S, lt.prim, u0, u1, pdf);
     F3 wi = intr.p - ref.p;
diff --git a/pbrt-v3-iile_amd/csrc/device/dpath.h b/pbrt-v3-iile_amd/csrc/device/dpath.h
--- a/pbrt-v3-iile_amd/csrc/device/dpath.h
+++ b/pbrt-v3-iile_amd/csrc/device/dpath.h
@@ -211,6 +211,40 @@
     concentric_sample_disk(u0, u1, &dx, &dy);
     float z = sqrtf(mx(0.f, 1 - dx * dx - dy * dy));
     return F3{dx, dy, z};
+}
+struct NoWarp {
+    static constexpr bool on = false;
+};
+struct LambertWarp {
+    static constexpr bool on = true;
+    bool use;
+    F3 w;
+};
+struct ConeWarp {
+    static constexpr bool on = true;
+    bool use;
+    float sin_phi, cos_phi;
+};
+struct DirectWarp {
+    static constexpr bool on = true;
+    LambertWarp mis;
+    ConeWarp cone;
+};
+DEV NoWarp warp_mis(const NoWarp &) { return NoWarp(); }
+DEV NoWarp warp_cone(const NoWarp &) { return NoWarp(); }
+DEV LambertWarp warp_mis(const DirectWarp &w) { return w.mis; }
+DEV ConeWarp warp_cone(const DirectWarp &w) { return w.cone; }
+template <class WARP>
+DEV F3 cosine_sample_hemisphere(float u0, float u1, const WARP &warp) {
+    if constexpr (WARP::on) {
+        F3 w = warp.w;
+        if (__ballot(!warp.use) != 0) {
+            if (!warp.use) w = cosine_sample_hemisphere(u0, u1);
+        }
+        return w;
+    } else {
+        return cosine_sample_hemisphere(u0, u1);
+    }
 }
 
 DEV float opaque_zero() {
@@ -853,10 +887,11 @@
 #include "dbsdf.h"
 #include "dlight.h"
 
-template <bool EXT, bool COUNT, class BSDF>
+template <bool EXT, bool COUNT, class BSDF, class WARP = NoWarp>
 DEV uint32_t estimate_direct_request(const DScene &S, const DLight &lt, const DSphere *lsp, const Isect &is, const BSDF &bsdf, float ul0,
                                      float ul1, float us0, float us1, F3 &so, F3 &sd, F3 &A, F3 &mo, F3 &md, F3 &Bc,
-                                     unsigned long long *n_pdf_tests, unsigned long long *n_pdf_hits) {
+                                     unsigned long long *n_pdf_tests, unsigned long long *n_pdf_hits, WARP warp = WARP()) {
+    static_assert(!WARP::on || sizeof(BSDF) == sizeof(Bsdf), "the warp plane's values go to a plain Bsdf's Sample_f (no DIS build reads them)");
     uint32_t nee_flags = 0;
     if (EXT && lt.type == kLightInfinite) {
         float light_pdf = 0, scattering_pdf = 0;
@@ -898,7 +933,7 @@
     } else {
         float light_pdf = 0, scattering_pdf = 0;
         F3 wi = F3{0, 0, 0}, Li = F3{0, 0, 0};
-        const LightSample ps = EXT ? shape_sample(S, lt, is, ul0, ul1, &light_pdf) : sphere_sample(*lsp, is, ul0, ul1, &light_pdf);
+        const LightSample ps = EXT ? shape_sample(S, lt, is, ul0, ul1, &light_pdf, warp_cone(warp)) : sphere_sample(*lsp, is, ul0, ul1, &light_pdf, warp_cone(warp));
         if (light_pdf == 0 || length_sq(ps.p - is.p) == 0) {
             light_pdf = 0;
         } else {
@@ -916,7 +951,7 @@
                 nee_flags |= NEE_HAS_SHADOW;
             }
         }
-        F3 f2 = bsdf_sample_f(bsdf, is.wo, &wi, us0, us1, &scattering_pdf);
+        F3 f2 = bsdf_sample_f(bsdf, is.wo, &wi, us0, us1, &scattering_pdf, false, nullptr, nullptr, warp_mis(warp));
         f2 = f2 * absdot(wi, is.sn);
         if (!is_black(f2) && scattering_pdf > 0) {
             const F3 m_o = offset_ray_origin(is.p, is.perr, is.n, wi);
diff --git a/pbrt-v3-iile_amd/csrc/device/dscene.h b/pbrt-v3-iile_amd/csrc/device/dscene.h
--- a/pbrt-v3-iile_amd/csrc/device/dscene.h
+++ b/pbrt-v3-iile_amd/csrc/device/dscene.h
@@ -189,6 +189,9 @@
     S->stab_shade = nullptr;
     S->stab_slots = S->stab_spp = S->stab_spp_magic = S->stab_spp_shift = 0;
 }
+inline __host__ __device__ const float4 *warp_plane(const DScene &S) {
+    return S.stab_shade + size_t(S.max_depth) * size_t(S.stab_slots) * 2;
+}
 
 enum { NEE_HAS_SHADOW = 1, NEE_HAS_MIS = 2 };
 
diff --git a/pbrt-v3-iile_amd/csrc/device/kernels.h b/pbrt-v3-iile_amd/csrc/device/kernels.h
--- a/pbrt-v3-iile_amd/csrc/device/kernels.h
+++ b/pbrt-v3-iile_amd/csrc/device/kernels.h
@@ -82,6 +82,7 @@
     bool count_stats;
     int trav_blocks_per_cu = 0;
     bool camera_moves = false;
+    bool warp_table = false;
 };
 
 int api_fail(int code, const std::string &msg);
@@ -100,6 +101,9 @@
 void launch_sample_table(const DScene &S, float2 *cam, float2 *lens, float4 *shade, const LaunchCfg &cfg);
 void launch_sample_table_time(const DScene &S, float *time, const LaunchCfg &cfg);
 void launch_sample_table_read(const DScene &S, int n, const int *px, const int *py, const int *k, const int *bounce, float *out, const LaunchCfg &cfg);
+void launch_sample_warp(const DScene &S, const float4 *shade, float4 *warp, const LaunchCfg &cfg);
+void launch_sample_warp_read(const DScene &S, int n, const int *px, const int *py, const int *k, const int *bounce, float *out, const LaunchCfg &cfg);
+void launch_warp_probe(int n, const float *rec8, float *out8, const LaunchCfg &cfg);
 void launch_miss(const DScene &S, const PassBuffers &B, int bounce, uint32_t max_rays, const LaunchCfg &cfg);
 void launch_mis_lit(const DScene &S, const PassBuffers &B, int bounce, uint32_t max_rays, const LaunchCfg &cfg);
 void launch_direct_generate(const DScene &S, const PassDesc &P, const PassBuffers &B, const LaunchCfg &cfg);
diff --git a/pbrt-v3-iile_amd/csrc/device/kernels_shade.hip b/pbrt-v3-iile_amd/csrc/device/kernels_shade.hip
--- a/pbrt-v3-iile_amd/csrc/device/kernels_shade.hip
+++ b/pbrt-v3-iile_amd/csrc/device/kernels_shade.hip
@@ -114,6 +114,40 @@
     reinterpret_cast<float4 *>(out)[2 * size_t(i)] = a;
     reinterpret_cast<float4 *>(out)[2 * size_t(i) + 1] = b;
 }
+DEV void warp_record(const float4 &ra, const float4 &rb, float4 *wa, float4 *wb) {
+    const F3 mis = cosine_sample_hemisphere(ra.w, rb.x);
+    const F3 cont = cosine_sample_hemisphere(rb.y, rb.z);
+    float sin_phi, cos_phi;
+    sincos_f(sphere_cone_phi(ra.z), &sin_phi, &cos_phi);
+    *wa = make_float4(mis.x, mis.y, mis.z, cont.x);
+    *wb = make_float4(cont.y, cont.z, sin_phi, cos_phi);
+}
+__global__ __launch_bounds__(256) void k_sample_warp(DScene S, const float4 *shade, float4 *warp) {
+    const uint32_t slot = blockIdx.x * blockDim.x + threadIdx.x;
+    if (slot >= S.stab_slots) return;
+    const size_t at = (size_t(blockIdx.y) * S.stab_slots + slot) * 2;
+    float4 wa, wb;
+    warp_record(shade[at], shade[at + 1], &wa, &wb);
+    warp[at] = wa;
+    warp[at + 1] = wb;
+}
+__global__ void k_sample_warp_read(DScene S, int n, const int *px, const int *py, const int *k, const int *bounce, float *out) {
+    const int i = blockIdx.x * blockDim.x + threadIdx.x;
+    if (i >= n) return;
+    const float4 *rec = warp_plane(S) + (size_t(bounce[i]) * S.stab_slots + sample_slot(S, px[i], py[i], uint32_t(k[i]))) * 2;
+    reinterpret_cast<float4 *>(out)[2 * size_t(i)] = rec[0];
+    reinterpret_cast<float4 *>(out)[2 * size_t(i) + 1] = rec[1];
+}
+__global__ void k_warp_probe(int n, const float *rec8, float *out8) {
+    const int i = blockIdx.x * blockDim.x + threadIdx.x;
+    if (i >= n) return;
+    const float *r = rec8 + 8 * size_t(i);
+    const F3 mis = cosine_sample_hemisphere(r[3], r[4]), cont = cosine_sample_hemisphere(r[5], r[6]);
+    float s, c;
+    sincos_f(sphere_cone_phi(r[2]), &s, &c);
+    float *o = out8 + 8 * size_t(i);
+    o[0] = mis.x, o[1] = mis.y, o[2] = mis.z, o[3] = cont.x, o[4] = cont.y, o[5] = cont.z, o[6] = s, o[7] = c;
+}
 #endif
 
 #ifndef IILE_SHADE_WAVES
@@ -129,11 +163,15 @@
 #ifndef IILE_SHADE_TAB_REREAD
 #define IILE_SHADE_TAB_REREAD 0
 #endif
-template <bool COUNT, bool EXT, bool TEX, bool TAB = false, bool DIS = false, bool MOT = false>
+#ifndef IILE_SHADE_WARP_REREAD
+#define IILE_SHADE_WARP_REREAD 1
+#endif
+template <bool COUNT, bool EXT, bool TEX, bool TAB = false, bool DIS = false, bool MOT = false, bool WARP = false>
 __global__ __launch_bounds__(kBlock, shade_waves(TEX, DIS)) void k_shade(DScene S, PassDesc P, PassBuffers B, int bounce, uint32_t plane) {
     static_assert(!(TAB && COUNT), "the instrumented build keeps the digit chains");
     static_assert(!DIS || (EXT && TEX && !COUNT), "the Disney builds are textured ones");
     static_assert(!MOT || (TEX && (DIS || COUNT)), "the moving camera's builds are the instrumented one and the Disney builds");
+    static_assert(!WARP || (TAB && !DIS), "the warp plane belongs to the sample table; the Disney builds do not read it");
     constexpr bool DZ = DIS || COUNT;
     typename std::conditional<TAB, const uint16_t *, lds_u16 *>::type s_perms;
     if constexpr (TAB) {
@@ -197,6 +235,8 @@
         int dim = 0;
         bool tab_wave = false;
         float4 rec_a = make_float4(0, 0, 0, 0), rec_b = make_float4(0, 0, 0, 0);
+        float4 warp_a = make_float4(0, 0, 0, 0), warp_b = make_float4(0, 0, 0, 0);
+        auto warp_rec = [&]() { return warp_plane(S) + (size_t(bounce) * S.stab_slots + hidx) * 2; };
         auto chain_index = [&]() { return TAB ? slot_halton_index(S, hidx) : hidx; };
         Isect is;
         typename bsdf_of<DZ>::type bsdf;
@@ -252,6 +292,7 @@
                             rec_a = rec[0];
                             rec_b = rec[1];
                             u_nee[0] = rec_a.y, u_nee[1] = rec_a.z, u_nee[2] = rec_a.w, u_nee[3] = rec_b.x;
+                            if (WARP && !IILE_SHADE_WARP_REREAD) warp_a = warp_rec()[0], warp_b = warp_rec()[1];
                         } else {
                             sample_dimensions_n<4>(S, s_perms, dim_u + 1, false, dim + 1, chain_index(), u_nee);
                         }
@@ -353,8 +394,17 @@
                             const DLight &lt = EXT ? S.lights[li] : lt_u;
                             const DSphere &lsp = EXT ? S.spheres[lt.sphere] : lsp_u;
                             dim += 4;
-                            nee_flags = estimate_direct_request<EXT, COUNT>(S, lt, &lsp, is, bsdf, u_nee[0], u_nee[1], u_nee[2], u_nee[3], so, sd,
-                                                                            A, mo, md, Bc, &n_pdf_tests, &n_pdf_hits);
+                            if constexpr (WARP) {
+                                if (IILE_SHADE_WARP_REREAD && tab_wave) warp_a = warp_rec()[0], warp_b = warp_rec()[1];
+                                DirectWarp dw;
+                                dw.mis = LambertWarp{tab_wave && n_nonspec(bsdf) == 1 && bsdf.has_lambert, F3{warp_a.x, warp_a.y, warp_a.z}};
+                                dw.cone = ConeWarp{tab_wave, warp_b.z, warp_b.w};
+                                nee_flags = estimate_direct_request<EXT, COUNT>(S, lt, &lsp, is, bsdf, u_nee[0], u_nee[1], u_nee[2], u_nee[3], so, sd,
+                                                                                A, mo, md, Bc, &n_pdf_tests, &n_pdf_hits, dw);
+                            } else {
+                                nee_flags = estimate_direct_request<EXT, COUNT>(S, lt, &lsp, is, bsdf, u_nee[0], u_nee[1], u_nee[2], u_nee[3], so, sd,
+                                                                                A, mo, md, Bc, &n_pdf_tests, &n_pdf_hits);
+                            }
                             stamps.mark(3);
                             nee_light = uint32_t(li);
                             emit_nee = COUNT || nee_flags != 0;
@@ -389,8 +439,20 @@
         if (P.skip_last_bounce == 2 && bounce + 1 >= S.max_depth) surface = false;
         if (surface) {
             float u_bsdf[2], ur_tab = 0;
+            LambertWarp cont_warp{false, F3{0, 0, 0}};
             if (TAB && tab_wave) {
                 const int off = dim - (5 + 7 * bounce);
+                if constexpr (WARP) {
+                    cont_warp.use = off == 5 && (EXT ? bsdf.n_lobes : n_nonspec(bsdf)) == 1 && bsdf.has_lambert;
+                    if (IILE_SHADE_WARP_REREAD) {
+                        if (__ballot(cont_warp.use) != 0) {
+                            const float *wf = reinterpret_cast<const float *>(warp_rec()) + 3;
+                            cont_warp.w = F3{wf[0], wf[1], wf[2]};
+                        }
+                    } else {
+                        cont_warp.w = F3{warp_a.w, warp_b.x, warp_b.y};
+                    }
+                }
                 if (IILE_SHADE_TAB_REREAD) {
                     const float *rf = reinterpret_cast<const float *>(S.stab_shade + (size_t(bounce) * S.stab_slots + hidx) * 2) + off;
                     u_bsdf[0] = rf[0], u_bsdf[1] = rf[1];
@@ -407,7 +469,11 @@
             float pdf = 0;
             F3 wi = F3{0, 0, 0};
             bool sampled_specular = false, sampled_transmission = false;
-            const F3 f = bsdf_sample_f(bsdf, -ray_d, &wi, u0, u1, &pdf, EXT, &sampled_specular, &sampled_transmission);
+            F3 f;
+            if constexpr (WARP)
+                f = bsdf_sample_f(bsdf, -ray_d, &wi, u0, u1, &pdf, EXT, &sampled_specular, &sampled_transmission, cont_warp);
+            else
+                f = bsdf_sample_f(bsdf, -ray_d, &wi, u0, u1, &pdf, EXT, &sampled_specular, &sampled_transmission);
             float eta_scale = 1.f;
             if (EXT && S.has_glass && bounce > 0) eta_scale = B.eta_scale[pid];
             if (!(is_black(f) || pdf == 0.f)) {
@@ -495,8 +561,12 @@
     } else if (S.stab_shade && !cfg.count_stats) {
         if (S.textured_materials)
             hipLaunchKernelGGL((k_shade<false, true, true, true>), grid, dim3(kBlock), 0, cfg.stream, S, P, B, bounce, B.queue_cap);
+        else if (S.extended_features && cfg.warp_table)
+            hipLaunchKernelGGL((k_shade<false, true, false, true, false, false, true>), grid, dim3(kBlock), 0, cfg.stream, S, P, B, bounce, B.queue_cap);
         else if (S.extended_features)
             hipLaunchKernelGGL((k_shade<false, true, false, true>), grid, dim3(kBlock), 0, cfg.stream, S, P, B, bounce, B.queue_cap);
+        else if (cfg.warp_table)
+            hipLaunchKernelGGL((k_shade<false, false, false, true, false, false, true>), grid, dim3(kBlock), 0, cfg.stream, S, P, B, bounce, B.queue_cap);
         else
             hipLaunchKernelGGL((k_shade<false, false, false, true>), grid, dim3(kBlock), 0, cfg.stream, S, P, B, bounce, B.queue_cap);
     } else if (cfg.count_stats)
@@ -518,6 +588,15 @@
 void launch_sample_table_read(const DScene &S, int n, const int *px, const int *py, const int *k, const int *bounce, float *out, const LaunchCfg &cfg) {
     hipLaunchKernelGGL(k_sample_table_read, dim3((n + 127) / 128), dim3(128), 0, cfg.stream, S, n, px, py, k, bounce, out);
 }
+void launch_sample_warp(const DScene &S, const float4 *shade, float4 *warp, const LaunchCfg &cfg) {
+    hipLaunchKernelGGL(k_sample_warp, dim3((S.stab_slots + 255) / 256, S.max_depth), dim3(256), 0, cfg.stream, S, shade, warp);
+}
+void launch_sample_warp_read(const DScene &S, int n, const int *px, const int *py, const int *k, const int *bounce, float *out, const LaunchCfg &cfg) {
+    hipLaunchKernelGGL(k_sample_warp_read, dim3((n + 127) / 128), dim3(128), 0, cfg.stream, S, n, px, py, k, bounce, out);
+}
+void launch_warp_probe(int n, const float *rec8, float *out8, const LaunchCfg &cfg) {
+    hipLaunchKernelGGL(k_warp_probe, dim3((n + 127) / 128), dim3(128), 0, cfg.stream, n, rec8, out8);
+}
 void launch_light_distributions(const DScene &S, const float *samples, float *out, const LaunchCfg &cfg) {
     const int n = S.light_nv[0] * S.light_nv[1] * S.light_nv[2];
     for (int l0 = 0; l0 < S.n_lights; l0 += 32768) {
```

After: 12070. No clear change (-0.1%).
